# jematy/SAHS-Deformable-Nerf

Hardware: AMD Instinct MI355X
Metric: rendered rays/sec (coarse64+fine128, 8x256 MLP) (higher is better)
Workload: dtype f32

## Files before the change

include/sahs_nerf.h:

```cpp
#ifndef SAHS_NERF_H
#define SAHS_NERF_H
#include <stddef.h>
#include <stdint.h>
#ifdef __cplusplus
extern "C" {
#endif

#define SAHS_ABI_VERSION 1
#define SAHS_F32 0
#define SAHS_BF16 1
#define SAHS_BF16X3 3

int sahs_abi_version(void);
const char *sahs_last_error(void);

long sahs_param_count(void);
long sahs_packed_words(int precision);
long sahs_frame_words(void);

int sahs_pack_weights(const float *flat_params, void *packed, int precision, void *stream);

int sahs_fold_conditioning(const float *flat_params, const float *audio, const float *pose, int pose_ld, float *frame,
                           void *stream);

int sahs_get_ray_bundle(int H, int W, float fx, float fy, float cx, float cy, const float *c2w, int ld, float *ro, float *rd,
                        void *stream);

int sahs_ray_uniforms(uint64_t seed, int stream_id, long ray0, long N, int S, float *out, void *stream);

int sahs_stratified_depths(long N, int S, const float *rays, int ray_stride, int lindisp, const float *t_rand, float *z,
                           void *stream);

int sahs_field_forward(const void *packed, const float *frame, int level, long N, int S, const float *rays, int ray_stride,
                       const float *z, float *raw, float *dbg, int precision, void *stream);

int sahs_composite_forward(long N, int S, const float *raw, const float *z, const float *rays, int ray_stride,
                           const float *noise, const float *bg, int white_background, float *rgb, float *disp, float *acc,
                           float *weights, float *depth, void *stream);

int sahs_resample(long N, int S, int nf, const float *z, const float *weights, const float *u, float *z_samples,
                  float *z_out, int64_t *inds, void *stream);

int sahs_sample_pdf(long N, int nb, int ns, const float *bins, const float *weights, const float *u, float *samples,
                    int64_t *inds, void *stream);

int sahs_render_rays(const void *packed, const float *frame, int precision, long N, const float *rays, int ray_stride, int Sc,
                     int nf, int lindisp, int white_background, const float *bg, const float *t_rand, const float *noise_c,
                     const float *u, const float *noise_f, float *z_c, float *z_f, float *raw, float *weights, float *rgb_c,
                     float *disp_c, float *acc_c, float *rgb_f, float *disp_f, float *acc_f, float *w_bg, float *depth_f,
                     void *stream);

long sahs_act_words_per_sample(void);
long sahs_field_backward_workspace_words(long P);
int sahs_field_forward_save(const void *packed, const float *frame, int level, long N, int S, const float *rays, int ray_stride,
                            const float *z, float *raw, float *act_out, void *stream);
int sahs_field_backward(const float *flat_params, const float *frame, int level, long P, const float *act_in, const float *d_raw,
                        float *grad_flat, float *grad_cond, float *workspace, void *stream);
int sahs_backward_gemm_precision(int precision);
int sahs_composite_backward(long N, int S, const float *raw, const float *z, const float *rays, int ray_stride, const float *noise,
                            const float *bg, int white_background, const float *d_rgb, const float *d_disp, const float *d_acc,
                            const float *d_depth, const float *d_wlast, const float *d_weights, float *d_raw, void *stream);
#define SAHS_LOSS_STATS_WORDS 64
int sahs_stage1_loss_forward(long N, const float *map_coarse, const float *map_fine, const float *target, int target_ld, const float *mask,
                             const float *class_weights, float *stats, void *stream);
int sahs_composite_backward_loss(long N, int S, const float *raw, const float *z, const float *rays, int ray_stride, const float *noise,
                                 const float *bg, int white_background, const float *d_rgb, const float *d_disp, const float *d_acc,
                                 const float *d_depth, const float *d_wlast, const float *loss_map, const float *loss_target, int target_ld,
                                 const float *loss_mask, const float *loss_stats, const float *loss_gscale, float *d_raw, void *stream);
int sahs_conditioning_backward(const float *flat_params, const float *audio, const float *grad_cond, float *grad_flat,
                               float *grad_audio, void *stream);

#define SAHS_MODEL_AUDIO 0
#define SAHS_MODEL_NERFACE 1
#define SAHS_MODEL_NERFACE_STATIC 2
long sahs_model_param_count(int model);
long sahs_model_packed_words(int model, int precision);
long sahs_model_frame_words(int model);
int sahs_model_pack_weights(int model, const float *flat_params, void *packed, int precision, void *stream);
int sahs_model_fold_conditioning(int model, const float *flat_params, const float *driving, const float *pose, int pose_ld, float *frame,
                                 void *stream);
int sahs_model_field_forward(int model, const void *packed, const float *frame, int level, long N, int S, const float *rays,
                             int ray_stride, const float *z, float *raw, float *dbg, int precision, void *stream);
int sahs_model_render_rays(int model, const void *packed, const float *frame, int precision, long N, const float *rays, int ray_stride,
                           int Sc, int nf, int lindisp, int white_background, const float *bg, const float *t_rand, const float *noise_c,
                           const float *u, const float *noise_f, float *z_c, float *z_f, float *raw, float *weights, float *rgb_c,
                           float *disp_c, float *acc_c, float *rgb_f, float *disp_f, float *acc_f, float *w_bg, float *depth_f,
                           void *stream);

long sahs_model_act_words_per_sample(int model);
long sahs_model_field_backward_workspace_words(int model, long P);
int sahs_model_field_forward_save(int model, const void *packed, const float *frame, int level, long N, int S, const float *rays,
                                  int ray_stride, const float *z, float *raw, float *act_out, void *stream);
int sahs_model_field_backward(int model, const float *flat_params, const float *frame, int level, long P, const float *act_in,
                              const float *d_raw, float *grad_flat, float *grad_cond, float *workspace, void *stream);

long sahs_model_executed_macs_per_sample(int model, int precision);
long sahs_model_executed_macs_part(int model, int precision, int part);

#define SAHS_ROW_COLUMNS 36
#define SAHS_ROW_RGB_C 0
#define SAHS_ROW_DISP_C 15
#define SAHS_ROW_ACC_C 16
#define SAHS_ROW_RGB_F 17
#define SAHS_ROW_DISP_F 32
#define SAHS_ROW_ACC_F 33
#define SAHS_ROW_W_BG 34
#define SAHS_ROW_DEPTH_F 35
int sahs_composite_forward_rows(long N, int S, const float *raw, const float *z, const float *rays, int ray_stride, const float *noise,
                                const float *bg, int white_background, float *weights, float *rows, int row_ld, int fine_pass, void *stream);
int sahs_resample_merge(long N, int S, int nf, const float *z, const float *weights, const float *u, float *z_samples, float *z_out,
                        int32_t *src, void *stream);

int sahs_model_field_forward_split(int model, const void *packed, const float *frame, int precision, int level, int mode, long N, int S, const float *rays,
                                   int ray_stride, const float *z, float *raw, float *xw, int xw_row, int xw_col0, const int32_t *src,
                                   void *stream);

long sahs_model_act_words_part(int model, int part);
int sahs_model_field_forward_split_save(int model, const void *packed, const float *frame, int level, int mode, long N, int S, const float *rays,
                                        int ray_stride, const float *z, float *raw, float *xw, int xw_row, int xw_col0, const int32_t *src,
                                        float *act_out, void *stream);
int sahs_model_field_backward_split(int model, const float *flat_params, const float *frame, int level, int part, long P, const float *act_in,
                                    const float *d_raw, const float *xw_grad_in, float *xw_grad_out, float *grad_flat, float *grad_cond,
                                    float *workspace, void *stream);
int sahs_route_xw_grad(long N, int Sc, int nf, const int32_t *src, const float *g_fine, float *g_coarse, float *g_new, void *stream);

int sahs_bf16_exact_leaky(int enable);

long sahs_model_bits_words_part(int model, int part);
int sahs_model_field_forward_split_save_bits(int model, const void *packed, const float *frame, int level, int mode, long N, int S, const float *rays,
                                             int ray_stride, const float *z, float *raw, float *xw, int xw_row, int xw_col0, const int32_t *src,
                                             float *act_out, uint32_t *bits_out, void *stream);
int sahs_model_field_forward_save_bits(int model, const void *packed, const float *frame, int level, long N, int S, const float *rays,
                                       int ray_stride, const float *z, float *raw, float *act_out, uint32_t *bits_out, void *stream);
int sahs_model_field_forward_split_save_bits_x3(int model, const void *packed, const float *frame, int level, int mode, long N, int S, const float *rays,
                                                int ray_stride, const float *z, float *raw, float *xw, int xw_row, int xw_col0, const int32_t *src,
                                                float *act_out, uint32_t *bits_out, void *stream);
int sahs_model_field_forward_save_bits_x3(int model, const void *packed, const float *frame, int level, long N, int S, const float *rays,
                                          int ray_stride, const float *z, float *raw, float *act_out, uint32_t *bits_out, void *stream);
long sahs_model_field_backward_fused_workspace_words(int model, int part, long P);
int sahs_model_field_backward_fused(int model, const float *flat_params, const float *frame, int level, int part, long P, const float *act_in,
                                    const uint32_t *bits_in, const float *d_raw, const float *xw_grad_in, float *xw_grad_out, float *grad_flat,
                                    float *grad_cond, float *workspace, void *stream);

int sahs_model_render_rays_rows(int model, const void *packed, const float *frame, int precision, long N, const float *rays,
                                int ray_stride, int Sc, int nf, int lindisp, int white_background, const float *bg, const float *t_rand,
                                const float *noise_c, const float *u, const float *noise_f, float *z_c, float *z_f, float *raw,
                                float *weights, float *rows, int row_ld, float *xw, int32_t *src, float *z_new, void *stream);

size_t sahs_model_render_sparse_workspace_bytes(int model, long samples);
int sahs_model_render_rays_rows_sparse(int model, const void *packed, const float *frame, int precision, long N, const float *rays,
                                       int ray_stride, int Sc, int nf, int lindisp, int white_background, const float *bg, const float *t_rand,
                                       const float *noise_c, const float *u, const float *noise_f, float *z_c, float *z_f, float *raw,
                                       float *weights, float *rows, int row_ld, float *xw, int32_t *src, float *z_new, void *ws, size_t ws_bytes,
                                       void *stream);

int sahs_adam_step(float *params, const float *grad, float *exp_avg, float *exp_avg_sq, long n, float lr, float beta1, float beta2,
                   float eps, long step, float grad_scale, void *stream);

long sahs_spade_modulate_workspace_words(long planes);
int sahs_spade_modulate(long planes, long hw, const float *x, const float *gamma, const float *beta, float eps, float slope, float *out,
                        float *stats, void *stream);

int sahs_probe_arm(int capacity);
int sahs_probe_disarm(void);
int sahs_probe_count(void);
int sahs_probe_dropped(void);
int sahs_probe_read(int i, int *kind, long *samples, float *ms);

#ifdef __cplusplus
}
#endif
#endif
```

sahs-deformable-nerf_amd/_lib.py:

```python
import ctypes
import os

_HERE = os.path.dirname(os.path.abspath(__file__))
LIB_PATH = os.environ.get("SAHS_NERF_LIB") or os.path.join(_HERE, "libsahs_nerf.so")
SAHS_F32, SAHS_BF16, SAHS_BF16X3 = 0, 1, 3

_P = ctypes.c_void_p
_I = ctypes.c_int
_L = ctypes.c_long
_F = ctypes.c_float

SIGNATURES = {
    "sahs_abi_version": (_I, []),
    "sahs_last_error": (ctypes.c_char_p, []),
    "sahs_param_count": (_L, []),
    "sahs_packed_words": (_L, [_I]),
    "sahs_frame_words": (_L, []),
    "sahs_pack_weights": (_I, [_P, _P, _I, _P]),
    "sahs_fold_conditioning": (_I, [_P, _P, _P, _I, _P, _P]),
    "sahs_get_ray_bundle": (_I, [_I, _I, _F, _F, _F, _F, _P, _I, _P, _P, _P]),
    "sahs_ray_uniforms": (_I, [ctypes.c_uint64, _I, _L, _L, _I, _P, _P]),
    "sahs_stratified_depths": (_I, [_L, _I, _P, _I, _I, _P, _P, _P]),
    "sahs_field_forward": (_I, [_P, _P, _I, _L, _I, _P, _I, _P, _P, _P, _I, _P]),
    "sahs_composite_forward": (_I, [_L, _I, _P, _P, _P, _I, _P, _P, _I, _P, _P, _P, _P, _P, _P]),
    "sahs_resample": (_I, [_L, _I, _I, _P, _P, _P, _P, _P, _P, _P]),
    "sahs_sample_pdf": (_I, [_L, _I, _I, _P, _P, _P, _P, _P, _P]),
    "sahs_render_rays": (_I, [_P, _P, _I, _L, _P, _I, _I, _I, _I, _I] + [_P] * 18),
    "sahs_act_words_per_sample": (_L, []),
    "sahs_field_backward_workspace_words": (_L, [_L]),
    "sahs_field_forward_save": (_I, [_P, _P, _I, _L, _I, _P, _I, _P, _P, _P, _P]),
    "sahs_field_backward": (_I, [_P, _P, _I, _L, _P, _P, _P, _P, _P, _P]),
    "sahs_composite_backward": (_I, [_L, _I, _P, _P, _P, _I, _P, _P, _I, _P, _P, _P, _P, _P, _P, _P, _P]),
    "sahs_conditioning_backward": (_I, [_P, _P, _P, _P, _P, _P]),
    "sahs_model_param_count": (_L, [_I]),
    "sahs_model_packed_words": (_L, [_I, _I]),
    "sahs_model_frame_words": (_L, [_I]),
    "sahs_model_pack_weights": (_I, [_I, _P, _P, _I, _P]),
    "sahs_model_fold_conditioning": (_I, [_I, _P, _P, _P, _I, _P, _P]),
    "sahs_model_field_forward": (_I, [_I, _P, _P, _I, _L, _I, _P, _I, _P, _P, _P, _I, _P]),
    "sahs_model_render_rays": (_I, [_I, _P, _P, _I, _L, _P, _I, _I, _I, _I, _I] + [_P] * 18),
    "sahs_composite_forward_rows": (_I, [_L, _I, _P, _P, _P, _I, _P, _P, _I, _P, _P, _I, _I, _P]),
    "sahs_model_executed_macs_per_sample": (_L, [_I, _I]),
    "sahs_model_executed_macs_part": (_L, [_I, _I, _I]),
    "sahs_model_render_rays_rows": (_I, [_I, _P, _P, _I, _L, _P, _I, _I, _I, _I, _I] + [_P] * 10 + [_I, _P, _P, _P, _P]),
    "sahs_model_render_sparse_workspace_bytes": (ctypes.c_size_t, [_I, _L]),
    "sahs_model_render_rays_rows_sparse": (_I, [_I, _P, _P, _I, _L, _P, _I, _I, _I, _I, _I] + [_P] * 10 + [_I, _P, _P, _P, _P, ctypes.c_size_t, _P]),
    "sahs_resample_merge": (_I, [_L, _I, _I, _P, _P, _P, _P, _P, _P, _P]),
    "sahs_model_act_words_part": (_L, [_I, _I]),
    "sahs_model_field_forward_split_save": (_I, [_I, _P, _P, _I, _I, _L, _I, _P, _I, _P, _P, _P, _I, _I, _P, _P, _P]),
    "sahs_model_field_backward_split": (_I, [_I, _P, _P, _I, _I, _L, _P, _P, _P, _P, _P, _P, _P, _P]),
    "sahs_route_xw_grad": (_I, [_L, _I, _I, _P, _P, _P, _P, _P]),
    "sahs_bf16_exact_leaky": (_I, [_I]),
    "sahs_model_bits_words_part": (_L, [_I, _I]),
    "sahs_model_field_forward_split_save_bits": (_I, [_I, _P, _P, _I, _I, _L, _I, _P, _I, _P, _P, _P, _I, _I, _P, _P, _P, _P]),
    "sahs_model_field_forward_save_bits": (_I, [_I, _P, _P, _I, _L, _I, _P, _I, _P, _P, _P, _P, _P]),
    "sahs_model_field_forward_split_save_bits_x3": (_I, [_I, _P, _P, _I, _I, _L, _I, _P, _I, _P, _P, _P, _I, _I, _P, _P, _P, _P]),
    "sahs_model_field_forward_save_bits_x3": (_I, [_I, _P, _P, _I, _L, _I, _P, _I, _P, _P, _P, _P, _P]),
    "sahs_model_field_backward_fused_workspace_words": (_L, [_I, _I, _L]),
    "sahs_model_field_backward_fused": (_I, [_I, _P, _P, _I, _I, _L, _P, _P, _P, _P, _P, _P, _P, _P, _P]),
    "sahs_stage1_loss_forward": (_I, [_L, _P, _P, _P, _I, _P, _P, _P, _P]),
    "sahs_composite_backward_loss": (_I, [_L, _I, _P, _P, _P, _I, _P, _P, _I] + [_P] * 5 + [_P, _P, _I, _P, _P, _P, _P, _P]),
    "sahs_model_field_forward_split": (_I, [_I, _P, _P, _I, _I, _I, _L, _I, _P, _I, _P, _P, _P, _I, _I, _P, _P]),
    "sahs_model_act_words_per_sample": (_L, [_I]),
    "sahs_model_field_backward_workspace_words": (_L, [_I, _L]),
    "sahs_model_field_forward_save": (_I, [_I, _P, _P, _I, _L, _I, _P, _I, _P, _P, _P, _P]),
    "sahs_model_field_backward": (_I, [_I, _P, _P, _I, _L, _P, _P, _P, _P, _P, _P]),
    "sahs_backward_gemm_precision": (_I, [_I]),
    "sahs_adam_step": (_I, [_P, _P, _P, _P, _L, _F, _F, _F, _F, _L, _F, _P]),
    "sahs_spade_modulate_workspace_words": (_L, [_L]),
    "sahs_spade_modulate": (_I, [_L, _L, _P, _P, _P, _F, _F, _P, _P, _P]),
    "sahs_probe_arm": (_I, [_I]),
    "sahs_probe_disarm": (_I, []),
    "sahs_probe_count": (_I, []),
    "sahs_probe_dropped": (_I, []),
    "sahs_probe_read": (_I, [_I, ctypes.POINTER(_I), ctypes.POINTER(_L), ctypes.POINTER(_F)]),
}

_lib = None


class SahsError(RuntimeError):
    pass


def lib():
    global _lib
    if _lib is None:
        if not os.path.exists(LIB_PATH):
            raise SahsError("%s not found: the HIP extension is not built (run `python sahs-deformable-nerf_amd/build.py`); "
                            "there is no CPU fallback" % LIB_PATH)
        L = ctypes.CDLL(LIB_PATH)
        for name, (res, args) in SIGNATURES.items():
            fn = getattr(L, name)
            fn.restype, fn.argtypes = res, args
        if L.sahs_abi_version() != 1:
            raise SahsError("libsahs_nerf.so ABI version %d, expected 1" % L.sahs_abi_version())
        _lib = L
    return _lib


def check(code, what):
    if code != 0:
        raise SahsError("%s failed (%d): %s" % (what, code, lib().sahs_last_error().decode()))
```

sahs-deformable-nerf_amd/build.py:

```python
import os
import re
import subprocess
import sys

HERE = os.path.dirname(os.path.abspath(__file__))
CSRC = os.path.join(HERE, "csrc")
LIB = os.path.join(HERE, "libsahs_nerf.so")
SOURCES = ["capi.hip", "pack.hip", "render_ops.hip", "spade_ops.hip", "optim.hip", "field_f32.hip", "field_bf16w.hip", "field_bf16x3.hip", "field_bwd.hip", "field_bwd_gemm.hip", "field_bwd_chain.hip", "field_bwd_chain_f32.hip", "train_bwd.hip"]
MODEL_SOURCES = ["pack.hip", "field_f32.hip", "field_bwd.hip", "field_bwd_chain.hip", "field_bwd_chain_f32.hip"]
X3_SOURCES = ["field_bf16x3.hip"]
MODEL1_SOURCES = ["field_bf16w.hip"]
FIELD_FLAGS = ["-fno-honor-nans", "-mno-amdgpu-ieee"]
NO_SCRATCH = {"gemm_dma_kernel": 0, "_ZN4sahs24field_forward_f32_kernelILb0E": 0, "field_forward_bf16w_kernel": 0,
              "field_radiance_bf16x3_kernel": 0, "field_deform_bf16x3_kernel": 0, "gemm_tn_split_kernel": 0, "gemm_tn_jobs_kernel": 0,
              "field_backward_chain_rad_kernel": 0, "field_backward_chain_def_kernel": 0, "_ZN4sahs24field_forward_f32_kernelILb1E": 96,
              "gemm_tn_jobs_f32_kernel": 0, "gemm_tn_jobs256_f32_kernel": 0, "adam_step_kernel": 0,
              "field_backward_chain_rad_f32_kernel": 0, "field_backward_chain_def_f32_kernel": 0,
              "_ZN7sahs_nf3bwc31field_backward_chain_rad_kernel": 0, "_ZN7sahs_nf3bwc31field_backward_chain_def_kernel": 0,
              "_ZN7sahs_ns3bwc31field_backward_chain_rad_kernel": 0, "_ZN7sahs_nf3bwf35field_backward_chain_rad_f32_kernel": 0,
              "_ZN7sahs_nf3bwf35field_backward_chain_def_f32_kernel": 0, "_ZN7sahs_ns3bwf35field_backward_chain_rad_f32_kernel": 0}
HAND_SCHEDULED = [("field_bf16w.hip", 0, "field_forward_bf16w_kernel"), ("field_bf16w.hip", 1, "field_forward_bf16w_kernel"),
                  ("field_bf16w.hip", 2, "field_forward_bf16w_kernel"), ("field_bf16x3.hip", 0, "field_radiance_bf16x3_kernel"),
                  ("field_bf16x3.hip", 0, "field_deform_bf16x3_kernel"), ("field_bf16x3.hip", 1, "field_deform_bf16x3_kernel"),
                  ("field_bf16x3.hip", 1, "field_radiance_bf16x3_kernel"), ("field_bf16x3.hip", 2, "field_radiance_bf16x3_kernel"),
                  ("field_bwd_chain.hip", 0, "field_backward_chain_rad_kernel"), ("field_bwd_chain.hip", 0, "field_backward_chain_def_kernel"),
                  ("field_bwd_chain.hip", 1, "field_backward_chain_rad_kernel"), ("field_bwd_chain.hip", 1, "field_backward_chain_def_kernel"),
                  ("field_bwd_chain.hip", 2, "field_backward_chain_rad_kernel")]
PER_FILE_FLAGS = {"field_bwd_gemm.hip": ["-fno-slp-vectorize"], "field_bwd.hip": ["-fno-slp-vectorize"],
                  "field_bf16w.hip": ["-mllvm", "-amdgpu-mfma-vgpr-form=1"], "field_bf16x3.hip": ["-mllvm", "-amdgpu-mfma-vgpr-form=1"],
                  "field_bwd_chain.hip": ["-mllvm", "-amdgpu-mfma-vgpr-form=1"]}
FLAGS = ["--offload-arch=gfx950", "-O3", "-std=c++20", "-fPIC", "-ffp-contract=off", "-fno-math-errno", "-Wall", "-Wno-unused-function"]


def _stale():
    if not os.path.exists(LIB):
        return True
    t = os.path.getmtime(LIB)
    deps = [os.path.join(CSRC, f) for f in os.listdir(CSRC)] + [os.path.join(HERE, "..", "include", "sahs_nerf.h")]
    return any(os.path.getmtime(d) > t for d in deps)


def _resource_usage(remarks):
    out, cur = {}, None
    keys = {"TotalSGPRs": "sgpr", "VGPRs": "vgpr", "AGPRs": "agpr", "ScratchSize [bytes/lane]": "scratch", "Occupancy [waves/SIMD]": "occ",
            "LDS Size [bytes/block]": "lds"}
    for line in remarks.splitlines():
        if "remark:" not in line:
            continue
        body = line.split("remark:", 1)[1].replace("[-Rpass-analysis=kernel-resource-usage]", "").strip()
        if body.startswith("Function Name:"):
            cur = body.split(":", 1)[1].strip()
            out[cur] = dict(sgpr=0, vgpr=0, agpr=0, scratch=0, occ=0, lds=0)
        elif cur is not None and ":" in body:
            k, v = body.rsplit(":", 1)
            if k.strip() in keys:
                out[cur][keys[k.strip()]] = int(v)
    return out


def _compile_cmd(hipcc, src, model, defines):
    base = os.path.basename(src)
    extra = (FIELD_FLAGS if base.startswith("field_") else []) + (["-DSAHS_MODEL=%d" % model] if model else []) + \
            ([] if "SAHS_NOTHING" in defines else PER_FILE_FLAGS.get(src, []))
    return [hipcc] + FLAGS + extra + ["-D" + d for d in defines]


def build(force=False, verbose=False, defines=(), out=None, check_inflight=True):
    global LIB
    if out is None and defines:
        raise RuntimeError("libsahs_nerf.so is built without extra defines (SAHS_DIAG variants go to their own file: out=...)")
    if out is not None:
        LIB, force = out, True
    if not (force or _stale()):
        return LIB
    hipcc = os.environ.get("HIPCC", "/opt/rocm/bin/hipcc")
    objs = []
    bdir = os.path.join(HERE, "build")
    os.makedirs(bdir, exist_ok=True)
    tag = os.path.basename(LIB)
    procs = []
    for src, model in [(s, 0) for s in SOURCES] + [(s, m) for m in (1, 2) for s in MODEL_SOURCES] + [(s, m) for m in (1, 2) for s in MODEL1_SOURCES] + [(s, m) for m in (1, 2) for s in X3_SOURCES]:
        obj = os.path.join(bdir, (tag + "." if out else "") + os.path.basename(src).replace(".hip", ".m%d.o" % model if model else ".o"))
        objs.append(obj)
        cmd = _compile_cmd(hipcc, src, model, defines) + ["-Rpass-analysis=kernel-resource-usage", "-c", os.path.join(CSRC, src), "-o", obj]
        if verbose:
            print(" ".join(cmd))
        procs.append((src, subprocess.Popen(cmd, stderr=subprocess.PIPE, text=True)))
    isa = []
    if check_inflight:
        for src, model, pat in HAND_SCHEDULED:
            path = os.path.join(bdir, "%s.%s.m%d.s" % (tag, src.replace(".hip", ""), model))
            cmd = _compile_cmd(hipcc, src, model, defines) + ["--cuda-device-only", "-S", os.path.join(CSRC, src), "-o", path]
            isa.append((src, model, pat, path, subprocess.Popen(cmd, stderr=subprocess.DEVNULL)))
    usage = {}
    for src, p in procs:
        err = p.communicate()[1]
        diag = [l for l in err.splitlines() if "[-Rpass-analysis=kernel-resource-usage]" not in l and not l.lstrip().startswith(("|", "^")) and
                not (l[:1] == " " and l.strip()[:1].isdigit() and "|" in l)]
        if diag and (verbose or p.returncode != 0):
            print("\n".join(diag), file=sys.stderr)
        if p.returncode != 0:
            raise RuntimeError("hipcc failed on " + src)
        usage.update(_resource_usage(err))
    with open(os.path.join(bdir, tag + ".resource_usage.txt"), "w") as f:
        for k in sorted(usage):
            f.write("%-110s vgpr %3d agpr %3d sgpr %3d scratch %4d lds %6d occupancy %d\n" % (
                k, usage[k]["vgpr"], usage[k]["agpr"], usage[k]["sgpr"], usage[k]["scratch"], usage[k]["lds"], usage[k]["occ"]))
    bad = ["%s: %d bytes/lane of scratch" % (k, v["scratch"]) for k, v in usage.items() for name, cap in NO_SCRATCH.items()
           if name in k and v["scratch"] > cap]
    if bad and not defines:
        raise RuntimeError("kernels that rely on counted waits must not use scratch:\n  " + "\n  ".join(bad))
    if isa:
        sys.path.insert(0, os.path.join(HERE, "..", "tools"))
        import check_lds_inflight as chk
        report = []
        for src, model, pat, path, p in isa:
            if p.wait() != 0:
                raise RuntimeError("hipcc -S failed on %s (SAHS_MODEL=%d)" % (src, model))
            text = open(path).read()
            total, viol, dist = chk.check(text, pat)
            for n in re.findall(r"^(\S*%s\S*):" % re.escape(pat), text, re.M):
                want, meta = usage.get(n), re.search(r"\.amdhsa_kernel %s\b.*?\.end_amdhsa_kernel" % re.escape(n), text, re.S)
                nxt = re.search(r"\.amdhsa_next_free_vgpr (\d+)", meta.group(0)) if meta else None
                if want is not None and nxt is not None:
                    expect = want["vgpr"] if not want["agpr"] else (want["vgpr"] + 3) // 4 * 4 + want["agpr"]
                    if int(nxt.group(1)) != expect:
                        raise RuntimeError("in-flight check: the ISA of %s is not the object's (next_free_vgpr %s, object vgpr %d agpr %d)"
                                           % (n, nxt.group(1), want["vgpr"], want["agpr"]))
            report.append("%s (SAHS_MODEL=%d) %s: %d hand-issued ds_read_b128, %d violations, longest in-flight window %d instructions"
                          % (src, model, pat, total, len(viol), max(dist) if dist else 0))
            if viol or total == 0:
                raise RuntimeError("hand-issued LDS reads touched in flight (tools/check_lds_inflight.py) in %s SAHS_MODEL=%d:\n  %s"
                                   % (src, model, "\n  ".join("%s | %s" % (r, w) for _, r, w in viol[:8]) or "no reads found"))
        with open(os.path.join(bdir, tag + ".lds_inflight.txt"), "w") as f:
            f.write("\n".join(report) + "\n")
        if verbose:
            print("\n".join(report))
    cmd = [hipcc, "--offload-arch=gfx950", "-shared", "-fPIC", "-Wl,-z,defs", "-o", LIB] + objs
    subprocess.check_call(cmd)
    return LIB


if __name__ == "__main__":
    print(build(force="--force" in sys.argv, verbose=True))
```

sahs-deformable-nerf_amd/csrc/capi.hip:

```cpp
#include <hip/hip_runtime.h>
#include <cmath>
#include <cstdarg>
#include <cstdio>
#include <cstdlib>
#include <cstring>
#include <atomic>
#include <vector>
#include "../../include/sahs_nerf.h"
#include "sahs_common.hpp"
#include "sahs_launchers.hpp"

static thread_local char g_err[512] = "";

__attribute__((format(printf, 2, 3))) static int fail(int code, const char *fmt, ...)
{
    va_list ap;
    va_start(ap, fmt);
    vsnprintf(g_err, sizeof(g_err), fmt, ap);
    va_end(ap);
    return code;
}
static int hip_fail(const char *what, int e)
{
    snprintf(g_err, sizeof(g_err), "%s: HIP error %d (%s)", what, e, hipGetErrorString((hipError_t)e));
    return 100 + e;
}
#define REQUIRE(cond, name) do { if (!(cond)) return fail(1, "%s: invalid argument (capi.hip:%d)", name, __LINE__); } while (0)
#define ALIGNED16(p) ((reinterpret_cast<uintptr_t>(p) & 15u) == 0)

static int num_cus()
{
    static std::atomic<int> cache[sahs_once::MAX_DEVICES];
    int dev = 0;
    if (hipGetDevice(&dev) != hipSuccess || dev < 0 || dev >= sahs_once::MAX_DEVICES) return 256;
    int n = cache[dev].load(std::memory_order_relaxed);
    if (n == 0) {
        int v = 0;
        n = (hipDeviceGetAttribute(&v, hipDeviceAttributeMultiprocessorCount, dev) == hipSuccess && v > 0) ? v : 256;
        cache[dev].store(n, std::memory_order_relaxed);
    }
    return n;
}

struct Probe {
    bool armed = false;
    int cap = 0, n = 0, dropped = 0;
    std::vector<hipEvent_t> ev;
    std::vector<int> kind;
    std::vector<long> samples;
};
static thread_local Probe g_probe;
static inline int probe_kind(int model, int precision, int level, int part) { return model << 16 | level << 12 | part << 8 | precision; }
template <class F> static inline int probed(int kind, long samples, hipStream_t st, F &&launch)
{
    Probe &p = g_probe;
    if (!p.armed) return launch();
    if (p.n >= p.cap) { ++p.dropped; return launch(); }
    (void)hipEventRecord(p.ev[2 * p.n], st);
    const int e = launch();
    (void)hipEventRecord(p.ev[2 * p.n + 1], st);
    p.kind[p.n] = kind;
    p.samples[p.n] = samples;
    ++p.n;
    return e;
}


extern "C" {

int sahs_abi_version(void) { return SAHS_ABI_VERSION; }

int sahs_probe_arm(int capacity)
{
    Probe &p = g_probe;
    REQUIRE(capacity >= 1 && capacity <= 65536, "sahs_probe_arm(1 <= capacity <= 65536)");
    while ((int)p.ev.size() < 2 * capacity) {
        hipEvent_t e;
        const hipError_t r = hipEventCreate(&e);
        if (r != hipSuccess) return hip_fail("sahs_probe_arm", (int)r);
        p.ev.push_back(e);
    }
    p.kind.assign(capacity, 0);
    p.samples.assign(capacity, 0);
    p.cap = capacity;
    p.n = p.dropped = 0;
    p.armed = true;
    return 0;
}
int sahs_probe_disarm(void) { g_probe.armed = false; return 0; }
int sahs_probe_count(void) { return g_probe.n; }
int sahs_probe_dropped(void) { return g_probe.dropped; }
int sahs_probe_read(int i, int *kind, long *samples, float *ms)
{
    Probe &p = g_probe;
    REQUIRE(i >= 0 && i < p.n && kind && samples && ms, "sahs_probe_read");
    hipError_t r = hipEventSynchronize(p.ev[2 * i + 1]);
    if (r == hipSuccess) r = hipEventElapsedTime(ms, p.ev[2 * i], p.ev[2 * i + 1]);
    if (r != hipSuccess) return hip_fail("sahs_probe_read", (int)r);
    *kind = p.kind[i];
    *samples = p.samples[i];
    return 0;
}
const char *sahs_last_error(void) { return g_err; }

int sahs_get_ray_bundle(int H, int W, float fx, float fy, float cx, float cy, const float *c2w, int ld, float *ro, float *rd, void *stream)
{
    REQUIRE(H > 0 && W > 0 && c2w && ro && rd && ld >= 4, "sahs_get_ray_bundle");
    int e = sahs_ray_bundle_launch(H, W, fx, fy, cx, cy, c2w, ld, ro, rd, (hipStream_t)stream);
    return e ? hip_fail("sahs_get_ray_bundle", e) : 0;
}

int sahs_ray_uniforms(uint64_t seed, int stream_id, long ray0, long N, int S, float *out, void *stream)
{
    if (N == 0) return 0;
    REQUIRE(out && N >= 0 && S >= 1 && ray0 >= 0, "sahs_ray_uniforms");
    int e = sahs_ray_uniforms_launch(seed, stream_id, ray0, N, S, out, (hipStream_t)stream);
    return e ? hip_fail("sahs_ray_uniforms", e) : 0;
}

int sahs_stratified_depths(long N, int S, const float *rays, int ray_stride, int lindisp, const float *t_rand, float *z, void *stream)
{
    if (N == 0) return 0;
    REQUIRE(N >= 0 && S >= 1 && rays && z && ray_stride >= 8, "sahs_stratified_depths");
    int e = sahs_stratified_depths_launch(N, S, rays, ray_stride, lindisp, t_rand, z, (hipStream_t)stream);
    return e ? hip_fail("sahs_stratified_depths", e) : 0;
}

int sahs_composite_forward(long N, int S, const float *raw, const float *z, const float *rays, int ray_stride, const float *noise,
                           const float *bg, int white_background, float *rgb, float *disp, float *acc, float *weights, float *depth,
                           void *stream)
{
    if (N == 0) return 0;
    REQUIRE(raw && z && rays && rgb && disp && acc && weights && depth && ray_stride >= 6, "sahs_composite_forward");
    REQUIRE(N >= 0 && S >= 1 && S <= 256 && ALIGNED16(raw), "sahs_composite_forward(shape: 1 <= S <= 256)");
    int e = sahs_composite_forward_launch(N, S, raw, z, rays, ray_stride, noise, bg, white_background, rgb, disp, acc, weights, depth,
                                          nullptr, 15, 1, (hipStream_t)stream);
    return e ? hip_fail("sahs_composite_forward", e) : 0;
}

int sahs_resample(long N, int S, int nf, const float *z, const float *weights, const float *u, float *z_samples, float *z_out,
                  int64_t *inds, void *stream)
{
    if (N == 0) return 0;
    REQUIRE(z && weights && z_out, "sahs_resample");
    REQUIRE(N >= 0 && S >= 3 && S <= 256 && nf >= 1 && nf <= 256, "sahs_resample(shape: 3 <= S <= 256, 1 <= nf <= 256)");
    int e = sahs_resample_launch(N, S, nf, 1, z, weights, u, z_samples, z_out, (long long *)inds, nullptr, (hipStream_t)stream);
    return e ? hip_fail("sahs_resample", e) : 0;
}

int sahs_resample_merge(long N, int S, int nf, const float *z, const float *weights, const float *u, float *z_samples, float *z_out,
                        int32_t *src, void *stream)
{
    if (N == 0) return 0;
    REQUIRE(z && weights && z_out && z_samples && src, "sahs_resample_merge");
    REQUIRE(N >= 0 && S >= 3 && S <= 256 && nf >= 1 && nf <= 256, "sahs_resample_merge(shape: 3 <= S <= 256, 1 <= nf <= 256)");
    int e = sahs_resample_launch(N, S, nf, 1, z, weights, u, z_samples, z_out, nullptr, src, (hipStream_t)stream);
    return e ? hip_fail("sahs_resample_merge", e) : 0;
}

int sahs_sample_pdf(long N, int nb, int ns, const float *bins, const float *weights, const float *u, float *samples, int64_t *inds,
                    void *stream)
{
    if (N == 0) return 0;
    REQUIRE(bins && weights && samples, "sahs_sample_pdf");
    REQUIRE(N >= 0 && nb >= 2 && nb < 256 && ns >= 1 && ns <= 256, "sahs_sample_pdf(shape: 2 <= nb < 256, 1 <= ns <= 256)");
    int e = sahs_resample_launch(N, nb + 1, ns, 0, bins, weights, u, samples, nullptr, (long long *)inds, nullptr, (hipStream_t)stream);
    return e ? hip_fail("sahs_sample_pdf", e) : 0;
}

int sahs_composite_backward(long N, int S, const float *raw, const float *z, const float *rays, int ray_stride, const float *noise,
                            const float *bg, int white_background, const float *d_rgb, const float *d_disp, const float *d_acc,
                            const float *d_depth, const float *d_wlast, const float *d_weights, float *d_raw, void *stream)
{
    REQUIRE(raw && z && rays && d_raw && ray_stride >= 6 && ALIGNED16(raw) && ALIGNED16(d_raw), "sahs_composite_backward");
    REQUIRE(N >= 0 && S >= 1 && S <= 256, "sahs_composite_backward(shape: 1 <= S <= 256)");
    if (N == 0) return 0;
    int e = sahs_composite_backward_launch(N, S, raw, z, rays, ray_stride, noise, bg, white_background, d_rgb, d_disp, d_acc, d_depth, d_wlast,
                                           d_weights, d_raw, nullptr, nullptr, 0, nullptr, nullptr, nullptr, (hipStream_t)stream);
    return e ? hip_fail("sahs_composite_backward", e) : 0;
}

int sahs_stage1_loss_forward(long N, const float *map_coarse, const float *map_fine, const float *target, int target_ld, const float *mask,
                             const float *class_weights, float *stats, void *stream)
{
    REQUIRE((map_coarse || map_fine) && target && mask && class_weights && stats && target_ld >= 3 && N >= 1, "sahs_stage1_loss_forward");
    int e = sahs_stage1_loss_forward_launch(N, map_coarse, map_fine, target, target_ld, mask, class_weights, stats, (hipStream_t)stream);
    return e ? hip_fail("sahs_stage1_loss_forward", e) : 0;
}

int sahs_composite_backward_loss(long N, int S, const float *raw, const float *z, const float *rays, int ray_stride, const float *noise,
                                 const float *bg, int white_background, const float *d_rgb, const float *d_disp, const float *d_acc,
                                 const float *d_depth, const float *d_wlast, const float *loss_map, const float *loss_target, int target_ld,
                                 const float *loss_mask, const float *loss_stats, const float *loss_gscale, float *d_raw, void *stream)
{
    REQUIRE(raw && z && rays && d_raw && ray_stride >= 6 && ALIGNED16(raw) && ALIGNED16(d_raw), "sahs_composite_backward_loss");
    REQUIRE(loss_map && loss_target && loss_mask && loss_stats && target_ld >= 3, "sahs_composite_backward_loss(loss operands)");
    REQUIRE(N >= 0 && S >= 1 && S <= 256, "sahs_composite_backward_loss(shape: 1 <= S <= 256)");
    if (N == 0) return 0;
    int e = sahs_composite_backward_launch(N, S, raw, z, rays, ray_stride, noise, bg, white_background, d_rgb, d_disp, d_acc, d_depth, d_wlast,
                                           nullptr, d_raw, loss_map, loss_target, target_ld, loss_mask, loss_stats, loss_gscale,
                                           (hipStream_t)stream);
    return e ? hip_fail("sahs_composite_backward_loss", e) : 0;
}

int sahs_conditioning_backward(const float *flat_params, const float *audio, const float *grad_cond, float *grad_flat, float *grad_audio,
                               void *stream)
{
    REQUIRE(flat_params && audio && grad_cond && grad_flat, "sahs_conditioning_backward");
    int e = sahs_conditioning_backward_launch(flat_params, audio, grad_cond, grad_flat, grad_audio, (hipStream_t)stream);
    return e ? hip_fail("sahs_conditioning_backward", e) : 0;
}

int sahs_route_xw_grad(long N, int Sc, int nf, const int32_t *src, const float *g_fine, float *g_coarse, float *g_new, void *stream)
{
    if (N == 0) return 0;
    REQUIRE(src && g_fine && g_coarse && g_new && N >= 0 && Sc >= 1 && nf >= 1 && ALIGNED16(g_fine) && ALIGNED16(g_coarse) && ALIGNED16(g_new),
            "sahs_route_xw_grad");
    int e = sahs_route_xw_grad_launch(N, Sc, nf, src, g_fine, g_coarse, g_new, (hipStream_t)stream);
    return e ? hip_fail("sahs_route_xw_grad", e) : 0;
}

static double decimal_double(float x)
{
    char buf[32];
    for (int digits = 1; digits <= 9; ++digits) {
        snprintf(buf, sizeof(buf), "%.*g", digits, (double)x);
        if (strtof(buf, nullptr) == x) return strtod(buf, nullptr);
    }
    return (double)x;
}

int sahs_adam_step(float *params, const float *grad, float *exp_avg, float *exp_avg_sq, long n, float lr, float beta1, float beta2, float eps,
                   long step, float grad_scale, void *stream)
{
    if (n == 0) return 0;
    REQUIRE(params && grad && exp_avg && exp_avg_sq && n > 0 && step >= 1, "sahs_adam_step");
    REQUIRE(std::isfinite(lr) && lr > 0.0f && std::isfinite(eps) && eps > 0.0f && std::isfinite(grad_scale), "sahs_adam_step(lr > 0, eps > 0, finite)");
    REQUIRE(beta1 >= 0.0f && beta1 < 1.0f && beta2 >= 0.0f && beta2 < 1.0f, "sahs_adam_step(0 <= beta < 1)");
    const uintptr_t p = reinterpret_cast<uintptr_t>(params), g = reinterpret_cast<uintptr_t>(grad), m = reinterpret_cast<uintptr_t>(exp_avg),
                    v = reinterpret_cast<uintptr_t>(exp_avg_sq), bytes = (uintptr_t)n * sizeof(float);
    REQUIRE(((p | g | m | v) & 3u) == 0, "sahs_adam_step(4-byte aligned buffers)");
    auto overlap = [bytes](uintptr_t a, uintptr_t b) { return a < b + bytes && b < a + bytes; };
    REQUIRE(!overlap(p, m) && !overlap(p, v) && !overlap(m, v), "sahs_adam_step(params, exp_avg, exp_avg_sq must not overlap)");
    const double b1 = decimal_double(beta1), b2 = decimal_double(beta2);
    const double bc1 = 1.0 - std::pow(b1, (double)step), bc2 = 1.0 - std::pow(b2, (double)step);
    int e = sahs_adam_step_launch(params, grad, exp_avg, exp_avg_sq, n, (float)(1.0 - b1), (float)b2, (float)(1.0 - b2),
                                  (float)(decimal_double(lr) / bc1), (float)std::sqrt(bc2), (float)decimal_double(eps), grad_scale,
                                  (hipStream_t)stream);
    return e ? hip_fail("sahs_adam_step", e) : 0;
}

long sahs_spade_modulate_workspace_words(long planes) { return planes > 0 ? sahs_spade_stats_words(planes) : 0; }

int sahs_spade_modulate(long planes, long hw, const float *x, const float *gamma, const float *beta, float eps, float slope, float *out,
                        float *stats, void *stream)
{
    if (planes == 0 || hw == 0) return 0;
    REQUIRE(planes > 0 && planes <= 2147483647L && hw > 0 && x && gamma && beta && out && stats && eps > 0.0f, "sahs_spade_modulate");
    int e = sahs_spade_modulate_launch(planes, hw, x, gamma, beta, eps, slope, out, stats, (hipStream_t)stream);
    return e ? hip_fail("sahs_spade_modulate", e) : 0;
}

int sahs_composite_forward_rows(long N, int S, const float *raw, const float *z, const float *rays, int ray_stride, const float *noise,
                                const float *bg, int white_background, float *weights, float *rows, int row_ld, int fine_pass, void *stream)
{
    if (N == 0) return 0;
    REQUIRE(raw && z && rays && weights && rows && ray_stride >= 6 && row_ld >= SAHS_ROW_COLUMNS, "sahs_composite_forward_rows");
    REQUIRE(N >= 0 && S >= 1 && S <= 256 && ALIGNED16(raw), "sahs_composite_forward_rows(shape: 1 <= S <= 256)");
    int e = fine_pass ? sahs_composite_forward_launch(N, S, raw, z, rays, ray_stride, noise, bg, white_background, rows + SAHS_ROW_RGB_F,
                                                      rows + SAHS_ROW_DISP_F, rows + SAHS_ROW_ACC_F, weights, rows + SAHS_ROW_DEPTH_F,
                                                      rows + SAHS_ROW_W_BG, row_ld, row_ld, (hipStream_t)stream)
                      : sahs_composite_forward_launch(N, S, raw, z, rays, ray_stride, noise, bg, white_background, rows + SAHS_ROW_RGB_C,
                                                      rows + SAHS_ROW_DISP_C, rows + SAHS_ROW_ACC_C, weights, nullptr, nullptr, row_ld,
                                                      row_ld, (hipStream_t)stream);
    return e ? hip_fail("sahs_composite_forward_rows", e) : 0;
}

enum Pack { PK_NONE, PK_F32, PK_BF16, PK_X3 };
typedef int (*pack_fn)(const float *, float *, hipStream_t);
struct ModelFns {
    bool deformation_nets;
    long (*param_count)(void);
    long (*frame_words)(void);
    long (*act_words)(void);
    long (*packed_words[4])(void);
    pack_fn pack[4];
    long (*executed_macs)(int, int);
    int (*act_part_words)(int);
    int (*act_part_col0)(int);
    int (*bits_part_words)(int);
    int (*fold)(const float *, const float *, const float *, int, float *, hipStream_t);
    int (*bwd_gemm_precision_state)(int);
    int (*bf16w_exact_leaky_state)(int);
    decltype(&sahs_field_forward_f32_launch) f32;
    decltype(&sahs_field_forward_f32_split_launch) f32_split;
    decltype(&sahs_field_forward_f32_split_bits_launch) f32_split_bits;
    decltype(&sahs_field_forward_f32_sparse_launch) f32_sparse;
    decltype(&sahs_field_f32_sparse_ws_bytes) f32_sparse_ws_bytes;
    long (*bwd_ws_words)(long);
    decltype(&sahs_field_backward_launch) bwd;
    decltype(&sahs_field_backward_split_launch) bwd_split;
    long (*fused_ws_words)(int, long);
    decltype(&sahs_field_backward_fused_launch) bwd_fused;
    decltype(&sahs_field_forward_bf16w_launch) bf16w;
    decltype(&sahs_field_forward_bf16w_split_launch) bf16w_split;
    decltype(&sahs_field_deform_bf16x3_launch) deform_x3;
    decltype(&sahs_field_deform_bf16x3_save_launch) deform_x3_save;
    decltype(&sahs_field_radiance_bf16x3_launch) radiance_x3;
    decltype(&sahs_field_radiance_bf16x3_save_launch) radiance_x3_save;
    decltype(&sahs_field_forward_bf16x3_launch) x3;
    decltype(&sahs_field_forward_bf16x3_save_launch) x3_save;
};
#define SAHS_MODEL_ROW(sfx, deform)                                                                                                    \
    deform, sahs_layout_param_count##sfx, sahs_layout_frame_words##sfx, sahs_layout_act_words##sfx,                                 \
        {nullptr, sahs_layout_packed_words_f32##sfx, sahs_layout_packed_words_bf16##sfx, sahs_layout_packed_words_bf16x3##sfx},      \
        {nullptr, sahs_pack_weights_f32_launch##sfx, sahs_pack_weights_bf16_launch##sfx, sahs_pack_weights_bf16x3_launch##sfx},      \
        sahs_layout_executed_macs##sfx, sahs_layout_act_part_words##sfx, sahs_layout_act_part_col0##sfx, sahs_layout_bits_part_words##sfx, \
        sahs_fold_conditioning_launch##sfx, sahs_bwd_gemm_precision_state##sfx, sahs_bf16w_exact_leaky_state##sfx,                  \
        sahs_field_forward_f32_launch##sfx, sahs_field_forward_f32_split_launch##sfx, sahs_field_forward_f32_split_bits_launch##sfx, \
        sahs_field_forward_f32_sparse_launch##sfx, sahs_field_f32_sparse_ws_bytes##sfx,                                              \
        sahs_field_backward_ws_words##sfx, sahs_field_backward_launch##sfx, sahs_field_backward_split_launch##sfx,                  \
        sahs_field_backward_fused_ws_words##sfx, sahs_field_backward_fused_launch##sfx
static const ModelFns kModels[3] = {
    {SAHS_MODEL_ROW(, true), sahs_field_forward_bf16w_launch, sahs_field_forward_bf16w_split_launch, sahs_field_deform_bf16x3_launch,
     sahs_field_deform_bf16x3_save_launch, sahs_field_radiance_bf16x3_launch, sahs_field_radiance_bf16x3_save_launch, nullptr, nullptr},
    {SAHS_MODEL_ROW(_nf, true), nullptr, sahs_field_forward_bf16w_split_launch_nf, sahs_field_deform_bf16x3_launch_nf,
     sahs_field_deform_bf16x3_save_launch_nf, sahs_field_radiance_bf16x3_launch_nf, sahs_field_radiance_bf16x3_save_launch_nf, nullptr, nullptr},
    {SAHS_MODEL_ROW(_ns, false), sahs_field_forward_bf16w_launch_ns, nullptr, nullptr, nullptr, nullptr, nullptr,
     sahs_field_forward_bf16x3_launch_ns, sahs_field_forward_bf16x3_save_launch_ns},
};
#undef SAHS_MODEL_ROW

enum Kernel { K_NONE, K_F32, K_BF16, K_X3 };
struct Pipe {
    Pack seg[3];
    Kernel whole;
    Kernel split;
    Kernel chain;
    int def_prec, def_x, rad_prec, rad_x;
};
static const Pipe kPipes[3][4] = {
    {
        {{PK_F32}, K_F32, K_F32, K_NONE, SAHS_F32, 1, SAHS_F32, 1},
        {{PK_BF16}, K_BF16, K_BF16, K_NONE, SAHS_BF16, 1, SAHS_BF16, 1},
        {{}, K_NONE, K_NONE, K_NONE, SAHS_BF16, 1, SAHS_BF16, 1},
        {{PK_X3, PK_F32}, K_NONE, K_NONE, K_X3, SAHS_BF16, 3, SAHS_BF16, 3},
    },
    {
        {{PK_F32}, K_F32, K_F32, K_NONE, SAHS_F32, 1, SAHS_F32, 1},
        {{PK_BF16, PK_F32, PK_X3}, K_NONE, K_NONE, K_BF16, SAHS_BF16, 3, SAHS_BF16, 1},
        {{}, K_NONE, K_NONE, K_NONE, SAHS_BF16, 1, SAHS_BF16, 1},
        {{PK_X3, PK_F32}, K_NONE, K_NONE, K_X3, SAHS_BF16, 3, SAHS_BF16, 3},
    },
    {
        {{PK_F32}, K_F32, K_NONE, K_NONE, SAHS_F32, 1, SAHS_F32, 1},
        {{PK_BF16}, K_BF16, K_NONE, K_NONE, SAHS_BF16, 1, SAHS_BF16, 1},
        {{}, K_NONE, K_NONE, K_NONE, SAHS_BF16, 1, SAHS_BF16, 1},
        {{PK_X3}, K_X3, K_NONE, K_NONE, SAHS_BF16, 3, SAHS_BF16, 3},
    },
};
static const Pipe *pipe_of(int model, int precision) { return precision >= 0 && precision <= 3 ? &kPipes[model][precision] : nullptr; }
static long packed_layout(int model, const Pipe *p, long off[4])
{
    long end = -1;
    for (int i = 0; p && i < 3 && p->seg[i] != PK_NONE; ++i) {
        off[p->seg[i]] = end < 0 ? 0 : (end + 3) / 4 * 4;
        end = off[p->seg[i]] + kModels[model].packed_words[p->seg[i]]();
    }
    return end;
}
static bool x3_deform_on_f32()
{
    static const bool v = getenv("SAHS_X3_DEFORM") != nullptr && strcmp(getenv("SAHS_X3_DEFORM"), "f32") == 0;
    return v;
}
static long act_col0(int model, int part) { return kModels[model].act_part_col0(part == 3 ? 0 : part); }
#define REQUIRE_MODEL(m, name) do { if ((m) < 0 || (m) > 2) return fail(3, "%s: unknown model %d", name, (int)(m)); } while (0)

long sahs_param_count(void) { return sahs_model_param_count(SAHS_MODEL_AUDIO); }
long sahs_packed_words(int precision) { return sahs_model_packed_words(SAHS_MODEL_AUDIO, precision); }
long sahs_frame_words(void) { return sahs_model_frame_words(SAHS_MODEL_AUDIO); }
long sahs_act_words_per_sample(void) { return sahs_model_act_words_per_sample(SAHS_MODEL_AUDIO); }
long sahs_field_backward_workspace_words(long P) { return sahs_model_field_backward_workspace_words(SAHS_MODEL_AUDIO, P); }

long sahs_model_param_count(int model) { return (model < 0 || model > 2) ? -1 : kModels[model].param_count(); }
long sahs_model_frame_words(int model) { return (model < 0 || model > 2) ? -1 : kModels[model].frame_words(); }
long sahs_model_act_words_per_sample(int model) { return (model < 0 || model > 2) ? -1 : kModels[model].act_words(); }
long sahs_model_field_backward_workspace_words(int model, long P) { return (model < 0 || model > 2) ? -1 : kModels[model].bwd_ws_words(P); }
long sahs_model_packed_words(int model, int precision)
{
    long off[4];
    return (model < 0 || model > 2) ? -1 : packed_layout(model, pipe_of(model, precision), off);
}
long sahs_model_executed_macs_part(int model, int precision, int part)
{
    if (model < 0 || model > 2 || precision < SAHS_F32 || precision > SAHS_BF16X3 || part < 0 || part > 2) return -1;
    const ModelFns &m = kModels[model];
    const Pipe &p = kPipes[model][precision];
    const long def = p.chain != K_NONE && x3_deform_on_f32() ? m.executed_macs(SAHS_F32, 1) : p.def_x * m.executed_macs(p.def_prec, 1);
    const long rad = p.rad_x * m.executed_macs(p.rad_prec, 2);
    return (part != 2 ? def : 0) + (part != 1 ? rad : 0);
}
long sahs_model_executed_macs_per_sample(int model, int precision) { return sahs_model_executed_macs_part(model, precision, 0); }
long sahs_model_act_words_part(int model, int part)
{
    return (model < 0 || model > 2 || part < 0 || part > 3) ? -1 : kModels[model].act_part_words(part == 3 ? 0 : part);
}
long sahs_model_bits_words_part(int model, int part)
{
    return (model < 0 || model > 2 || part < 0 || part > 3) ? 0 : kModels[model].bits_part_words(part == 3 ? 0 : part);
}
long sahs_model_field_backward_fused_workspace_words(int model, int part, long P)
{
    return (model < 0 || model > 2 || part < 1 || part > 3 || P < 0) ? -1 : kModels[model].fused_ws_words(part, P);
}

int sahs_backward_gemm_precision(int precision)
{
    if (precision < 0) return kModels[SAHS_MODEL_AUDIO].bwd_gemm_precision_state(-1) ? SAHS_BF16X3 : SAHS_F32;
    if (precision != SAHS_F32 && precision != SAHS_BF16X3) return -1;
    for (const ModelFns &m : kModels) m.bwd_gemm_precision_state(precision == SAHS_BF16X3 ? 3 : 0);
    return precision;
}

int sahs_bf16_exact_leaky(int enable)
{
    if (enable < 0) return kModels[SAHS_MODEL_AUDIO].bf16w_exact_leaky_state(-1);
    int r = 0;
    for (int i = 2; i >= 0; --i) r = kModels[i].bf16w_exact_leaky_state(enable);
    return r;
}

static int pack_weights(const char *who, int model, const float *flat_params, void *packed, int precision, void *stream)
{
    REQUIRE(flat_params && packed && ALIGNED16(packed), who);
    long off[4];
    if (packed_layout(model, pipe_of(model, precision), off) < 0) return fail(2, "%s: precision %d is not built for this model", who, precision);
    int e = 0;
    for (Pack s : kPipes[model][precision].seg)
        if (s != PK_NONE && !e) e = kModels[model].pack[s](flat_params, (float *)packed + off[s], (hipStream_t)stream);
    return e ? hip_fail(who, e) : 0;
}
int sahs_pack_weights(const float *flat_params, void *packed, int precision, void *stream)
{
    return pack_weights("sahs_pack_weights", SAHS_MODEL_AUDIO, flat_params, packed, precision, stream);
}
int sahs_model_pack_weights(int model, const float *flat_params, void *packed, int precision, void *stream)
{
    REQUIRE_MODEL(model, "sahs_model_pack_weights");
    return pack_weights("sahs_model_pack_weights", model, flat_params, packed, precision, stream);
}

static int fold_conditioning(const char *who, int model, const float *flat_params, const float *driving, const float *pose, int pose_ld,
                             float *frame, void *stream)
{
    REQUIRE(flat_params && driving && pose && frame && pose_ld >= 4 && ALIGNED16(frame), who);
    int e = kModels[model].fold(flat_params, driving, pose, pose_ld, frame, (hipStream_t)stream);
    return e ? hip_fail(who, e) : 0;
}
int sahs_fold_conditioning(const float *flat_params, const float *audio, const float *pose, int pose_ld, float *frame, void *stream)
{
    return fold_conditioning("sahs_fold_conditioning", SAHS_MODEL_AUDIO, flat_params, audio, pose, pose_ld, frame, stream);
}
int sahs_model_fold_conditioning(int model, const float *flat_params, const float *driving, const float *pose, int pose_ld, float *frame,
                                 void *stream)
{
    REQUIRE_MODEL(model, "sahs_model_fold_conditioning");
    return fold_conditioning("sahs_model_fold_conditioning", model, flat_params, driving, pose, pose_ld, frame, stream);
}

static int field_forward(const char *who, int model, const void *packed, const float *frame, int level, long N, int S, const float *rays,
                         int ray_stride, const float *z, float *raw, float *dbg, int precision, void *stream)
{
    if (N == 0) return 0;
    REQUIRE(packed && frame && rays && z && raw, who);
    REQUIRE((level == 0 || level == 1) && N >= 0 && S >= 1 && ray_stride >= 8, who);
    REQUIRE(ALIGNED16(packed) && ALIGNED16(frame) && ALIGNED16(raw) && (!dbg || ALIGNED16(dbg)), who);
    const Pipe *p = pipe_of(model, precision);
    long off[4];
    if (packed_layout(model, p, off) < 0) return fail(2, "%s: precision %d is not built for this model", who, precision);
    if (p->whole == K_NONE)
        return fail(2, "%s: precision %d of this model runs through sahs_model_field_forward_split / sahs_model_render_rays_rows (it needs the "
                       "xw workspace)", who, precision);
    const ModelFns &m = kModels[model];
    const float *pk = (const float *)packed;
    hipStream_t st = (hipStream_t)stream;
    int e = probed(probe_kind(model, precision, level, 0), N * S, st, [&] {
        if (p->whole == K_F32) return m.f32(pk, frame, level, N * S, S, rays, ray_stride, z, raw, dbg, nullptr, num_cus(), st);
        if (p->whole == K_BF16) return m.bf16w(pk, frame, level, N * S, S, rays, ray_stride, z, raw, dbg, num_cus(), st);
        return m.x3(pk, frame, level, N * S, S, rays, ray_stride, z, raw, num_cus(), st);
    });
    return e ? hip_fail(who, e) : 0;
}
int sahs_field_forward(const void *packed, const float *frame, int level, long N, int S, const float *rays, int ray_stride,
                       const float *z, float *raw, float *dbg, int precision, void *stream)
{
    return field_forward("sahs_field_forward", SAHS_MODEL_AUDIO, packed, frame, level, N, S, rays, ray_stride, z, raw, dbg, precision, stream);
}
int sahs_model_field_forward(int model, const void *packed, const float *frame, int level, long N, int S, const float *rays, int ray_stride,
                             const float *z, float *raw, float *dbg, int precision, void *stream)
{
    REQUIRE_MODEL(model, "sahs_model_field_forward");
    return field_forward("sahs_model_field_forward", model, packed, frame, level, N, S, rays, ray_stride, z, raw, dbg, precision, stream);
}

static int render_rays_chain(const char *who, int model, const void *packed, const float *frame, int precision, long N,
                             const float *rays, int ray_stride, int Sc, int nf, int lindisp, int white_background, const float *bg,
                             const float *t_rand, const float *noise_c, const float *u, const float *noise_f, float *z_c, float *z_f,
                             float *raw, float *weights, float *rgb_c, float *disp_c, float *acc_c, float *rgb_f, float *disp_f,
                             float *acc_f, float *w_bg, float *depth_f, void *stream, int rgb_ld = 15, int sc_ld = 1)
{
    if (N == 0) return 0;
    REQUIRE(packed && frame && rays && z_c && raw && weights && rgb_c && disp_c && acc_c && w_bg && depth_f, who);
    REQUIRE(nf == 0 || (z_f && rgb_f && disp_f && acc_f), who);
    hipStream_t st = (hipStream_t)stream;
    int e;
    if ((e = sahs_stratified_depths(N, Sc, rays, ray_stride, lindisp, t_rand, z_c, stream))) return e;
    if ((e = field_forward(who, model, packed, frame, 0, N, Sc, rays, ray_stride, z_c, raw, nullptr, precision, stream))) return e;
    REQUIRE(Sc <= 256, who);
    e = sahs_composite_forward_launch(N, Sc, raw, z_c, rays, ray_stride, noise_c, bg, white_background, rgb_c, disp_c, acc_c, weights,
                                      nf == 0 ? depth_f : nullptr, nf == 0 ? w_bg : nullptr, rgb_ld, sc_ld, st);
    if (e) return hip_fail(who, e);
    if (nf > 0) {
        const int Sf = Sc + nf;
        REQUIRE(Sf <= 256, who);
        if ((e = sahs_resample(N, Sc, nf, z_c, weights, u, nullptr, z_f, nullptr, stream))) return e;
        if ((e = field_forward(who, model, packed, frame, 1, N, Sf, rays, ray_stride, z_f, raw, nullptr, precision, stream))) return e;
        e = sahs_composite_forward_launch(N, Sf, raw, z_f, rays, ray_stride, noise_f, bg, white_background, rgb_f, disp_f, acc_f,
                                          weights, depth_f, w_bg, rgb_ld, sc_ld, st);
        if (e) return hip_fail(who, e);
    }
    return 0;
}

int sahs_render_rays(const void *packed, const float *frame, int precision, long N, const float *rays, int ray_stride, int Sc, int nf,
                     int lindisp, int white_background, const float *bg, const float *t_rand, const float *noise_c, const float *u,
                     const float *noise_f, float *z_c, float *z_f, float *raw, float *weights, float *rgb_c, float *disp_c,
                     float *acc_c, float *rgb_f, float *disp_f, float *acc_f, float *w_bg, float *depth_f, void *stream)
{
    return render_rays_chain("sahs_render_rays", SAHS_MODEL_AUDIO, packed, frame, precision, N, rays, ray_stride, Sc, nf, lindisp,
                             white_background, bg, t_rand, noise_c, u, noise_f, z_c, z_f, raw, weights, rgb_c, disp_c, acc_c, rgb_f, disp_f,
                             acc_f, w_bg, depth_f, stream);
}
int sahs_model_render_rays(int model, const void *packed, const float *frame, int precision, long N, const float *rays, int ray_stride,
                           int Sc, int nf, int lindisp, int white_background, const float *bg, const float *t_rand, const float *noise_c,
                           const float *u, const float *noise_f, float *z_c, float *z_f, float *raw, float *weights, float *rgb_c,
                           float *disp_c, float *acc_c, float *rgb_f, float *disp_f, float *acc_f, float *w_bg, float *depth_f, void *stream)
{
    REQUIRE_MODEL(model, "sahs_model_render_rays");
    return render_rays_chain("sahs_model_render_rays", model, packed, frame, precision, N, rays, ray_stride, Sc, nf, lindisp, white_background,
                             bg, t_rand, noise_c, u, noise_f, z_c, z_f, raw, weights, rgb_c, disp_c, acc_c, rgb_f, disp_f, acc_f, w_bg, depth_f,
                             stream);
}

int sahs_model_field_forward_split(int model, const void *packed, const float *frame, int precision, int level, int mode, long N, int S,
                                   const float *rays, int ray_stride, const float *z, float *raw, float *xw, int xw_row, int xw_col0,
                                   const int32_t *src, void *stream)
{
    const char *who = "sahs_model_field_forward_split";
    REQUIRE_MODEL(model, who);
    if (N == 0) return 0;
    const ModelFns &m = kModels[model];
    if (!m.deformation_nets) return fail(4, "%s: this model has no deformation nets", who);
    REQUIRE(packed && frame && rays && xw && (level == 0 || level == 1) && N >= 0 && S >= 1 && ray_stride >= 8 && mode >= 0 && mode <= 2, who);
    const Pipe *p = pipe_of(model, precision);
    const bool chain = p && p->chain != K_NONE;
    REQUIRE((mode == 1 || raw) && (mode == 2 || z) && (mode != 2 || src || chain), who);
    REQUIRE(xw_col0 >= 0 && xw_row >= xw_col0 + (mode == 2 ? 0 : S) && ALIGNED16(xw) && ALIGNED16(packed) && ALIGNED16(frame) && (!raw || ALIGNED16(raw)),
            who);
    const float *pk = (const float *)packed;
    const long P = N * S;
    hipStream_t st = (hipStream_t)stream;
    int e = 0;
    if (chain) {
        REQUIRE(mode != 0 || xw_col0 == 0, who);
        long off[4];
        packed_layout(model, p, off);
        if (mode != 2 && !x3_deform_on_f32())
            e = probed(probe_kind(model, SAHS_BF16X3, level, 1), P, st, [&] {
                return m.deform_x3(pk + off[PK_X3], frame, level, P, S, rays, ray_stride, z, xw, xw_row, xw_col0, num_cus(), st);
            });
        else if (mode != 2)
            e = probed(probe_kind(model, SAHS_F32, level, 1), P, st, [&] {
                return m.f32_split(pk + off[PK_F32], frame, level, 1, P, S, rays, ray_stride, z, nullptr, xw, xw_row, xw_col0, nullptr, nullptr,
                                   num_cus(), st);
            });
        if (!e && mode != 1)
            e = probed(probe_kind(model, precision, level, 2), P, st, [&] {
                const int *sp = mode == 2 ? src : nullptr;
                return p->chain == K_BF16
                           ? m.bf16w_split(pk + off[PK_BF16], frame, level, 2, P, S, rays, ray_stride, nullptr, raw, xw, xw_row, 0, sp, num_cus(), st)
                           : m.radiance_x3(pk + off[PK_X3], frame, level, P, S, rays, ray_stride, raw, xw, xw_row, sp, num_cus(), st);
            });
        return e ? hip_fail(who, e) : 0;
    }
    if (!p || p->split == K_NONE) return fail(4, "%s: precision %d is not built for this model", who, precision);
    e = probed(probe_kind(model, precision, level, mode), P, st, [&] {
        return p->split == K_BF16
                   ? m.bf16w_split(pk, frame, level, mode, P, S, rays, ray_stride, z, raw, xw, xw_row, xw_col0, src, num_cus(), st)
                   : m.f32_split(pk, frame, level, mode, P, S, rays, ray_stride, z, raw, xw, xw_row, xw_col0, src, nullptr, num_cus(), st);
    });
    return e ? hip_fail(who, e) : 0;
}


struct SaveForm {
    const char *who;
    bool split, x3, bits;
};
static int field_forward_save(const SaveForm &f, int model, const void *packed, const float *frame, int level, int mode, long N, int S,
                              const float *rays, int ray_stride, const float *z, float *raw, float *xw, int xw_row, int xw_col0,
                              const int32_t *src, float *act_out, uint32_t *bits_out, void *stream)
{
    const char *who = f.who;
    REQUIRE_MODEL(model, who);
    const ModelFns &m = kModels[model];
    if (f.split && !f.bits && N == 0) return 0;
    if (f.split && !m.deformation_nets)
        return fail(4, "%s: this model has no deformation nets (its saving forward: sahs_model_field_forward_save%s)", who,
                    f.x3 ? "_bits_x3" : (f.bits ? "_bits" : ""));
    if (!f.split && f.x3 && !m.x3_save)
        return fail(4, "%s: this model saves through the split chain on this pipe (sahs_model_field_forward_split_save_bits_x3)", who);
    if (f.split && N == 0) return 0;
    REQUIRE(packed && frame && rays && act_out && (!f.bits || bits_out) && (f.split ? xw != nullptr : z && raw), who);
    REQUIRE((level == 0 || level == 1) && N >= 0 && S >= 1 && ray_stride >= 8, who);
    if (f.split) {
        REQUIRE(f.x3 ? (mode == 1 || mode == 2) : (mode >= 0 && mode <= 2), who);
        REQUIRE((mode == 1 || raw) && (mode == 2 || z) && (mode != 2 || src), who);
        REQUIRE(xw_col0 >= 0 && xw_row >= xw_col0 + (mode == 2 ? 0 : S) && ALIGNED16(xw), who);
    }
    REQUIRE(ALIGNED16(packed) && ALIGNED16(frame) && (!raw || ALIGNED16(raw)) && ALIGNED16(act_out) && (!f.bits || ALIGNED16(bits_out)), who);
    const long P = N * S;
    REQUIRE(!f.bits || P <= 4000000L, who);
    if (!f.split && f.bits && P == 0) return 0;
    const float *pk = (const float *)packed;
    float *base = act_out - act_col0(model, mode) * P;
    hipStream_t st = (hipStream_t)stream;
    int e;
    if (f.x3)
        e = probed(probe_kind(model, SAHS_BF16X3, level, mode), P, st, [&] {
            if (!f.split) return m.x3_save(pk, frame, level, P, S, rays, ray_stride, z, raw, act_out, bits_out, num_cus(), st);
            if (mode == 1) return m.deform_x3_save(pk, frame, level, P, S, rays, ray_stride, z, xw, xw_row, xw_col0, base, bits_out, num_cus(), st);
            return m.radiance_x3_save(pk, frame, level, P, S, rays, ray_stride, raw, xw, xw_row, src, base, bits_out, num_cus(), st);
        });
    else if (f.bits)
        e = m.f32_split_bits(pk, frame, level, mode, P, S, rays, ray_stride, z, raw, xw, xw_row, xw_col0, src, base, bits_out, num_cus(), st);
    else if (f.split)
        e = m.f32_split(pk, frame, level, mode, P, S, rays, ray_stride, z, raw, xw, xw_row, xw_col0, src, base, num_cus(), st);
    else
        e = m.f32(pk, frame, level, P, S, rays, ray_stride, z, raw, nullptr, act_out, num_cus(), st);
    return e ? hip_fail(who, e) : 0;
}

int sahs_field_forward_save(const void *packed, const float *frame, int level, long N, int S, const float *rays, int ray_stride,
                            const float *z, float *raw, float *act_out, void *stream)
{
    return field_forward_save({"sahs_field_forward_save", false, false, false}, SAHS_MODEL_AUDIO, packed, frame, level, 0, N, S, rays,
                              ray_stride, z, raw, nullptr, 0, 0, nullptr, act_out, nullptr, stream);
}
int sahs_model_field_forward_save(int model, const void *packed, const float *frame, int level, long N, int S, const float *rays,
                                  int ray_stride, const float *z, float *raw, float *act_out, void *stream)
{
    return field_forward_save({"sahs_model_field_forward_save", false, false, false}, model, packed, frame, level, 0, N, S, rays, ray_stride,
                              z, raw, nullptr, 0, 0, nullptr, act_out, nullptr, stream);
}
int sahs_model_field_forward_save_bits(int model, const void *packed, const float *frame, int level, long N, int S, const float *rays, int ray_stride,
                                       const float *z, float *raw, float *act_out, uint32_t *bits_out, void *stream)
{
    return field_forward_save({"sahs_model_field_forward_save_bits", false, false, true}, model, packed, frame, level, 0, N, S, rays,
                              ray_stride, z, raw, nullptr, 0, 0, nullptr, act_out, bits_out, stream);
}
int sahs_model_field_forward_save_bits_x3(int model, const void *packed, const float *frame, int level, long N, int S, const float *rays, int ray_stride,
                                          const float *z, float *raw, float *act_out, uint32_t *bits_out, void *stream)
{
    return field_forward_save({"sahs_model_field_forward_save_bits_x3", false, true, true}, model, packed, frame, level, 0, N, S, rays,
                              ray_stride, z, raw, nullptr, 0, 0, nullptr, act_out, bits_out, stream);
}
int sahs_model_field_forward_split_save(int model, const void *packed, const float *frame, int level, int mode, long N, int S, const float *rays,
                                        int ray_stride, const float *z, float *raw, float *xw, int xw_row, int xw_col0, const int32_t *src,
                                        float *act_out, void *stream)
{
    return field_forward_save({"sahs_model_field_forward_split_save", true, false, false}, model, packed, frame, level, mode, N, S, rays,
                              ray_stride, z, raw, xw, xw_row, xw_col0, src, act_out, nullptr, stream);
}
int sahs_model_field_forward_split_save_bits(int model, const void *packed, const float *frame, int level, int mode, long N, int S, const float *rays,
                                             int ray_stride, const float *z, float *raw, float *xw, int xw_row, int xw_col0, const int32_t *src,
                                             float *act_out, uint32_t *bits_out, void *stream)
{
    return field_forward_save({"sahs_model_field_forward_split_save_bits", true, false, true}, model, packed, frame, level, mode, N, S, rays,
                              ray_stride, z, raw, xw, xw_row, xw_col0, src, act_out, bits_out, stream);
}
int sahs_model_field_forward_split_save_bits_x3(int model, const void *packed, const float *frame, int level, int mode, long N, int S, const float *rays,
                                                int ray_stride, const float *z, float *raw, float *xw, int xw_row, int xw_col0, const int32_t *src,
                                                float *act_out, uint32_t *bits_out, void *stream)
{
    return field_forward_save({"sahs_model_field_forward_split_save_bits_x3", true, true, true}, model, packed, frame, level, mode, N, S, rays,
                              ray_stride, z, raw, xw, xw_row, xw_col0, src, act_out, bits_out, stream);
}

static int field_backward(const char *who, int model, const float *flat_params, const float *frame, int level, long P, const float *act_in,
                          const float *d_raw, float *grad_flat, float *grad_cond, float *workspace, void *stream)
{
    REQUIRE(flat_params && frame && act_in && d_raw && grad_flat && grad_cond && workspace, who);
    REQUIRE((level == 0 || level == 1) && P >= 0 && P <= 4000000L, who);
    int e = kModels[model].bwd(flat_params, frame, level, P, act_in, d_raw, grad_flat, grad_cond, workspace, (hipStream_t)stream);
    return e ? hip_fail(who, e) : 0;
}
int sahs_field_backward(const float *flat_params, const float *frame, int level, long P, const float *act_in, const float *d_raw,
                        float *grad_flat, float *grad_cond, float *workspace, void *stream)
{
    return field_backward("sahs_field_backward", SAHS_MODEL_AUDIO, flat_params, frame, level, P, act_in, d_raw, grad_flat, grad_cond,
                          workspace, stream);
}
int sahs_model_field_backward(int model, const float *flat_params, const float *frame, int level, long P, const float *act_in,
                              const float *d_raw, float *grad_flat, float *grad_cond, float *workspace, void *stream)
{
    REQUIRE_MODEL(model, "sahs_model_field_backward");
    return field_backward("sahs_model_field_backward", model, flat_params, frame, level, P, act_in, d_raw, grad_flat, grad_cond, workspace,
                          stream);
}

int sahs_model_field_backward_split(int model, const float *flat_params, const float *frame, int level, int part, long P, const float *act_in,
                                    const float *d_raw, const float *xw_grad_in, float *xw_grad_out, float *grad_flat, float *grad_cond,
                                    float *workspace, void *stream)
{
    const char *who = "sahs_model_field_backward_split";
    REQUIRE_MODEL(model, who);
    if (part == 0) part = 3;
    REQUIRE(flat_params && frame && act_in && grad_flat && grad_cond && workspace && part >= 1 && part <= 3, who);
    REQUIRE((level == 0 || level == 1) && P >= 0 && P <= 4000000L, who);
    REQUIRE(((part & 2) ? d_raw != nullptr : xw_grad_in != nullptr) && (part != 2 || xw_grad_out != nullptr), who);
    const ModelFns &m = kModels[model];
    if (!m.deformation_nets && part != 3) return fail(4, "%s: this model has no deformation nets", who);
    int e = m.bwd_split(flat_params, frame, level, part, P, act_in - act_col0(model, part) * P, d_raw, xw_grad_in, xw_grad_out, grad_flat,
                        grad_cond, workspace, (hipStream_t)stream);
    return e ? hip_fail(who, e) : 0;
}

int sahs_model_field_backward_fused(int model, const float *flat_params, const float *frame, int level, int part, long P, const float *act_in,
                                    const uint32_t *bits_in, const float *d_raw, const float *xw_grad_in, float *xw_grad_out, float *grad_flat,
                                    float *grad_cond, float *workspace, void *stream)
{
    const char *who = "sahs_model_field_backward_fused";
    REQUIRE_MODEL(model, who);
    const ModelFns &m = kModels[model];
    if (!m.deformation_nets && part != 3) return fail(4, "%s: this model has no deformation nets", who);
    REQUIRE(flat_params && frame && act_in && bits_in && grad_flat && grad_cond && workspace && part >= 1 && part <= 3, who);
    REQUIRE((level == 0 || level == 1) && P >= 0 && P <= 4000000L, who);
    REQUIRE(((part & 2) ? d_raw != nullptr : xw_grad_in != nullptr) && (part != 2 || xw_grad_out != nullptr), who);
    REQUIRE(ALIGNED16(act_in) && ALIGNED16(bits_in) && ALIGNED16(workspace) && (!d_raw || ALIGNED16(d_raw)) && (!xw_grad_in || ALIGNED16(xw_grad_in)) &&
            (!xw_grad_out || ALIGNED16(xw_grad_out)), who);
    if (P == 0) return 0;
    int e = m.bwd_fused(flat_params, frame, level, part, P, act_in - act_col0(model, part) * P, bits_in, d_raw, xw_grad_in, xw_grad_out,
                        grad_flat, grad_cond, workspace, num_cus(), (hipStream_t)stream);
    return e ? hip_fail(who, e) : 0;
}

int sahs_model_render_rays_rows(int model, const void *packed, const float *frame, int precision, long N, const float *rays,
                                int ray_stride, int Sc, int nf, int lindisp, int white_background, const float *bg, const float *t_rand,
                                const float *noise_c, const float *u, const float *noise_f, float *z_c, float *z_f, float *raw,
                                float *weights, float *rows, int row_ld, float *xw, int32_t *src, float *z_new, void *stream)
{
    const char *who = "sahs_model_render_rays_rows";
    REQUIRE_MODEL(model, who);
    if (N == 0) return 0;
    REQUIRE(rows && row_ld >= SAHS_ROW_COLUMNS, who);
    const Pipe *p = pipe_of(model, precision);
    const bool deform = kModels[model].deformation_nets;
    if (deform && p && p->chain != K_NONE)
        REQUIRE(xw && src && z_new && nf > 0, who);
    if (xw && src && z_new && nf > 0 && deform && p && (p->split != K_NONE || p->chain != K_NONE)) {
        REQUIRE(packed && frame && rays && z_c && z_f && raw && weights && Sc + nf <= 256, who);
        const int Sf = Sc + nf;
        hipStream_t st = (hipStream_t)stream;
        int e;
        if ((e = sahs_stratified_depths(N, Sc, rays, ray_stride, lindisp, t_rand, z_c, stream))) return e;
        if ((e = sahs_model_field_forward_split(model, packed, frame, precision, 0, 0, N, Sc, rays, ray_stride, z_c, raw, xw, Sf, 0, nullptr, stream))) return e;
        e = sahs_composite_forward_launch(N, Sc, raw, z_c, rays, ray_stride, noise_c, bg, white_background, rows + SAHS_ROW_RGB_C, rows + SAHS_ROW_DISP_C,
                                          rows + SAHS_ROW_ACC_C, weights, nullptr, nullptr, row_ld, row_ld, st);
        if (e) return hip_fail(who, e);
        if ((e = sahs_resample_merge(N, Sc, nf, z_c, weights, u, z_new, z_f, src, stream))) return e;
        if ((e = sahs_model_field_forward_split(model, packed, frame, precision, 1, 1, N, nf, rays, ray_stride, z_new, nullptr, xw, Sf, Sc, nullptr, stream))) return e;
        if ((e = sahs_model_field_forward_split(model, packed, frame, precision, 1, 2, N, Sf, rays, ray_stride, nullptr, raw, xw, Sf, 0, src, stream))) return e;
        e = sahs_composite_forward_launch(N, Sf, raw, z_f, rays, ray_stride, noise_f, bg, white_background, rows + SAHS_ROW_RGB_F, rows + SAHS_ROW_DISP_F,
                                          rows + SAHS_ROW_ACC_F, weights, rows + SAHS_ROW_DEPTH_F, rows + SAHS_ROW_W_BG, row_ld, row_ld, st);
        return e ? hip_fail(who, e) : 0;
    }
    return render_rays_chain(who, model, packed, frame, precision, N, rays, ray_stride, Sc, nf, lindisp, white_background, bg, t_rand, noise_c,
                             u, noise_f, z_c, z_f, raw, weights, rows + SAHS_ROW_RGB_C, rows + SAHS_ROW_DISP_C, rows + SAHS_ROW_ACC_C,
                             rows + SAHS_ROW_RGB_F, rows + SAHS_ROW_DISP_F, rows + SAHS_ROW_ACC_F, rows + SAHS_ROW_W_BG, rows + SAHS_ROW_DEPTH_F,
                             stream, row_ld, row_ld);
}

static long sparse_capacity(int model, size_t ws_bytes)
{
    const ModelFns &m = kModels[model];
    const long head = m.f32_sparse_ws_bytes(0), rec = m.f32_sparse_ws_bytes(1) - head;
    if ((long)ws_bytes < head) return 0;
    long cap = ((long)ws_bytes - head) / rec / 128 * 128;
    return cap > (1L << 30) ? (1L << 30) : cap;
}
static int field_forward_sparse(const char *who, int model, const float *pk, const float *frame, int level, int stage, int part, long N, int S,
                                const float *rays, int ray_stride, const float *z, float *raw, float *xw, int xw_row, const int32_t *src,
                                const float *noise, int has_bg, void *ws, long cap, hipStream_t st)
{
    const ModelFns &m = kModels[model];
    const long per = cap / S;
    if (per < 1) return fail(5, "%s: the sparse-branch workspace holds %ld records, one ray has %d samples", who, cap, S);
    const long nslab = (N + per - 1) / per, step = (N + nslab - 1) / nslab;
    int e = probed(probe_kind(model, SAHS_F32, level, part), N * S, st, [&] {
        for (long r0 = 0; r0 < N; r0 += step) {
            const long n = N - r0 < step ? N - r0 : step, s0 = r0 * S;
            hipError_t he = hipMemsetAsync(ws, 0, 8, st);
            if (he != hipSuccess) return (int)he;
            int le = m.f32_sparse(pk, frame, level, stage, n * S, S, rays + r0 * ray_stride, ray_stride, z ? z + s0 : nullptr, raw + s0 * 16,
                                  xw ? xw + r0 * xw_row * 8 : nullptr, xw_row, 0, src ? src + s0 : nullptr, noise ? noise + s0 : nullptr, has_bg, ws,
                                  cap, num_cus(), st);
            if (le) return le;
            le = m.f32_sparse(pk, frame, level, 2, n * S, S, rays + r0 * ray_stride, ray_stride, nullptr, raw + s0 * 16, nullptr, 0, 0, nullptr, nullptr,
                              has_bg, ws, cap, num_cus(), st);
            if (le) return le;
        }
        return 0;
    });
    if (e == -4) return fail(5, "%s: the sparse-branch launcher refused its record workspace (%ld slots for slabs of %ld samples)", who, cap, step * S);
    if (e < 0) return fail(4, "%s: the sparse-branch launcher has no stage %d for this model", who, stage);
    return e ? hip_fail(who, e) : 0;
}

size_t sahs_model_render_sparse_workspace_bytes(int model, long samples)
{
    if (model < 0 || model > 2 || samples < 0 || samples > (1L << 30)) return 0;
    return (size_t)kModels[model].f32_sparse_ws_bytes((samples + 127) / 128 * 128);
}

int sahs_model_render_rays_rows_sparse(int model, const void *packed, const float *frame, int precision, long N, const float *rays,
                                       int ray_stride, int Sc, int nf, int lindisp, int white_background, const float *bg, const float *t_rand,
                                       const float *noise_c, const float *u, const float *noise_f, float *z_c, float *z_f, float *raw,
                                       float *weights, float *rows, int row_ld, float *xw, int32_t *src, float *z_new, void *ws, size_t ws_bytes,
                                       void *stream)
{
    const char *who = "sahs_model_render_rays_rows_sparse";
    REQUIRE_MODEL(model, who);
    if (precision != SAHS_F32)
        return sahs_model_render_rays_rows(model, packed, frame, precision, N, rays, ray_stride, Sc, nf, lindisp, white_background, bg, t_rand, noise_c,
                                           u, noise_f, z_c, z_f, raw, weights, rows, row_ld, xw, src, z_new, stream);
    if (N == 0) return 0;
    REQUIRE(rows && row_ld >= SAHS_ROW_COLUMNS, who);
    REQUIRE(packed && frame && rays && z_c && raw && weights && N >= 0 && Sc >= 1 && nf >= 0 && Sc + nf <= 256 && ray_stride >= 8, who);
    REQUIRE(nf == 0 || z_f, who);
    REQUIRE(ws && ALIGNED16(ws) && ALIGNED16(packed) && ALIGNED16(frame) && ALIGNED16(raw) && (!xw || ALIGNED16(xw)), who);
    const long cap = sparse_capacity(model, ws_bytes);
    if (cap < 128)
        return fail(5, "%s: a sparse-branch workspace of %zu bytes holds less than one tile of 128 records (sahs_model_render_sparse_workspace_bytes)",
                    who, ws_bytes);
    const bool shared = xw && src && z_new && nf > 0 && kModels[model].deformation_nets;
    const float *pk = (const float *)packed;
    const int Sf = Sc + nf, has_bg = bg != nullptr;
    hipStream_t st = (hipStream_t)stream;
    int e;
    if ((e = sahs_stratified_depths(N, Sc, rays, ray_stride, lindisp, t_rand, z_c, stream))) return e;
    if ((e = field_forward_sparse(who, model, pk, frame, 0, 0, 0, N, Sc, rays, ray_stride, z_c, raw, shared ? xw : nullptr, Sf, nullptr, noise_c, has_bg, ws,
                                  cap, st)))
        return e;
    e = sahs_composite_forward_launch(N, Sc, raw, z_c, rays, ray_stride, noise_c, bg, white_background, rows + SAHS_ROW_RGB_C, rows + SAHS_ROW_DISP_C,
                                      rows + SAHS_ROW_ACC_C, weights, nf == 0 ? rows + SAHS_ROW_DEPTH_F : nullptr, nf == 0 ? rows + SAHS_ROW_W_BG : nullptr,
                                      row_ld, row_ld, st);
    if (e) return hip_fail(who, e);
    if (nf == 0) return 0;
    if (shared) {
        if ((e = sahs_resample_merge(N, Sc, nf, z_c, weights, u, z_new, z_f, src, stream))) return e;
        if ((e = sahs_model_field_forward_split(model, packed, frame, precision, 1, 1, N, nf, rays, ray_stride, z_new, nullptr, xw, Sf, Sc, nullptr, stream))) return e;
        if ((e = field_forward_sparse(who, model, pk, frame, 1, 1, 2, N, Sf, rays, ray_stride, nullptr, raw, xw, Sf, src, noise_f, has_bg, ws, cap, st))) return e;
    } else {
        if ((e = sahs_resample(N, Sc, nf, z_c, weights, u, nullptr, z_f, nullptr, stream))) return e;
        if ((e = field_forward_sparse(who, model, pk, frame, 1, 0, 0, N, Sf, rays, ray_stride, z_f, raw, nullptr, 0, nullptr, noise_f, has_bg, ws, cap, st))) return e;
    }
    e = sahs_composite_forward_launch(N, Sf, raw, z_f, rays, ray_stride, noise_f, bg, white_background, rows + SAHS_ROW_RGB_F, rows + SAHS_ROW_DISP_F,
                                      rows + SAHS_ROW_ACC_F, weights, rows + SAHS_ROW_DEPTH_F, rows + SAHS_ROW_W_BG, row_ld, row_ld, st);
    return e ? hip_fail(who, e) : 0;
}

}
```

sahs-deformable-nerf_amd/csrc/field_f32.hip:

```cpp
#include <hip/hip_runtime.h>
#include "sahs_common.hpp"
#include "sahs_launchers.hpp"
#include "sahs_layout.hpp"
#include "f32_pipe.hpp"

namespace SAHS_NS {


struct RevArg { float p, lo; };
__device__ __forceinline__ RevArg rev_arg(float x)
{
    const float C_HI = 0.15915494f;
    const float C_LO = 6.4206382e-09f;
    RevArg r;
    r.p = x * C_HI;
    r.lo = fmaf(x, C_LO, fmaf(x, C_HI, -r.p));
    return r;
}
__device__ __forceinline__ float sin_octave(RevArg u, float scale, int fn)
{
    const float P = u.p * scale, Lo = u.lo * scale;
    const float f = (P - rintf(P)) + Lo;
    const float qf = rintf(4.0f * f);
    const float th = fmaf(qf, -0.25f, f) * 6.2831855f;
    const float z = th * th;
    const float sp = fmaf(th * z, fmaf(fmaf(-1.9515295891e-4f, z, 8.3321608736e-3f), z, -1.6666654611e-1f), th);
    const float cp = fmaf(z * z, fmaf(fmaf(2.443315711809948e-5f, z, -1.388731625493765e-3f), z, 4.166664568298827e-2f), fmaf(z, -0.5f, 1.0f));
    const int m = ((int)qf + fn) & 3;
    const float v = (m & 1) ? cp : sp;
    return (m & 2) ? -v : v;
}

template <int D, int L, int NB, int INC = 1>
__device__ __forceinline__ void pe_blocks(const float *v, int q, f32x4 *out)
{
    constexpr int D0 = INC ? D : 0;
    constexpr int W = D0 + 2 * D * L;
    const float v0 = v[0], v1 = v[D > 1 ? 1 : 0], v2 = v[D > 2 ? 2 : 0];
    const RevArg u0 = rev_arg(v0), u1 = rev_arg(v1), u2 = rev_arg(v2);
#pragma unroll
    for (int b = 0; b < NB; ++b)
#pragma unroll
        for (int r = 0; r < 4; ++r) {
            const int f = 16 * b + 4 * q + r;
            float val = 0.0f;
            if (f < D0) {
                val = (f == 0) ? v0 : ((f == 1) ? v1 : v2);
            } else if (f < W) {
                const int g = f - D0;
                const int k = g / (2 * D), rem = g % (2 * D);
                const int fn = rem / D, ax = rem % D;
                RevArg a;
                a.p = (ax == 0) ? u0.p : ((ax == 1) ? u1.p : u2.p);
                a.lo = (ax == 0) ? u0.lo : ((ax == 1) ? u1.lo : u2.lo);
                val = sin_octave(a, (float)(1 << k), fn);
            }
            out[b][r] = val;
        }
}

__device__ __forceinline__ void grid_blocks(const float *__restrict__ grid, float x, float y, float z, int q, f32x4 *out)
{
    const float R1 = (float)(G_RES - 1);
    const float ix = ((x + 1.0f) / 2.0f) * R1, iy = ((y + 1.0f) / 2.0f) * R1, iz = ((z + 1.0f) / 2.0f) * R1;
    const float fx = floorf(ix), fy = floorf(iy), fz = floorf(iz);
    const float x1 = fx + 1.0f, y1 = fy + 1.0f, z1 = fz + 1.0f;
    const float wx[2] = {x1 - ix, ix - fx}, wy[2] = {y1 - iy, iy - fy}, wz[2] = {z1 - iz, iz - fz};
    const bool ok = fx >= -1.0f && fx <= (float)G_RES && fy >= -1.0f && fy <= (float)G_RES && fz >= -1.0f && fz <= (float)G_RES;
    const int xi = ok ? (int)fx : -2, yi = ok ? (int)fy : -2, zi = ok ? (int)fz : -2;
    out[0] = f32x4{0.0f, 0.0f, 0.0f, 0.0f};
    out[1] = f32x4{0.0f, 0.0f, 0.0f, 0.0f};
#pragma unroll
    for (int n = 0; n < 8; ++n) {
        const int cx = xi + (n & 1), cy = yi + ((n >> 1) & 1), cz = zi + (n >> 2);
        const bool inb = cx >= 0 && cx < G_RES && cy >= 0 && cy < G_RES && cz >= 0 && cz < G_RES;
        const float wt = (wx[n & 1] * wy[(n >> 1) & 1]) * wz[n >> 2];
        const long vox = inb ? (((long)cz * G_RES + cy) * G_RES + cx) : 0;
        const f32x4 *g = reinterpret_cast<const f32x4 *>(grid + vox * D_GRID) + q;
        const f32x4 g0 = g[0], g1 = g[4];
        const float we = inb ? wt : 0.0f;
#pragma unroll
        for (int r = 0; r < 4; ++r) { out[0][r] = out[0][r] + g0[r] * we; out[1][r] = out[1][r] + g1[r] * we; }
    }
}

#define CHF(id) (kProg.layer[id].G * kProg.layer[id].KB * 256)

enum { FIELD_ALL = 0, FIELD_DEFORM = 1, FIELD_RADIANCE = 2, FIELD_ALL_TRUNK = 3, FIELD_RADIANCE_TRUNK = 4, FIELD_BRANCH = 5 };
struct SparseArgs {
    const float *noise;
    unsigned int *count;
    f32x4 *hdr;
    f32x4 *feat;
    unsigned int cap;
    int has_bg;
};
constexpr long SPARSE_HEAD_BYTES = 256, SPARSE_RECORD_BYTES = 16 + 16 * 16 * 4;
#if defined(SAHS_DIAG) && defined(SAHS_F32_ENC2)
constexpr bool DIAG_ENC2 = true;
#else
constexpr bool DIAG_ENC2 = false;
#endif
#if defined(SAHS_DIAG) && defined(SAHS_F32_NOENC)
constexpr bool DIAG_NOENC = true;
#else
constexpr bool DIAG_NOENC = false;
#endif
#if defined(SAHS_DIAG) && defined(SAHS_F32_NOLOADS_TRUNK)
constexpr bool DIAG_NOLOADS_TRUNK = true;
#else
constexpr bool DIAG_NOLOADS_TRUNK = false;
#endif
#if defined(SAHS_DIAG) && defined(SAHS_F32_NOLOADS_BRANCH)
constexpr bool DIAG_NOLOADS_BRANCH = true;
#else
constexpr bool DIAG_NOLOADS_BRANCH = false;
#endif
#if defined(SAHS_DIAG) && defined(SAHS_F32_NOAPPEND)
constexpr bool DIAG_NOAPPEND = true;
#else
constexpr bool DIAG_NOAPPEND = false;
#endif
template <int NB>
__device__ __forceinline__ void diag_blocks(const float *v, int q, f32x4 *out)
{
#pragma unroll
    for (int b = 0; b < NB; ++b) out[b] = f32x4{v[0], v[1], v[0] * (float)(q + b), v[1] + (float)b};
}
template <bool SAVE, int MODE>
__global__ void __launch_bounds__(F32_THREADS, 2)
field_forward_f32_kernel(const float *__restrict__ packed, const float *__restrict__ frame, int level, long P, int S,
                         const float *__restrict__ rays, int ray_stride, const float *__restrict__ zvals,
                         float *__restrict__ raw, float *__restrict__ dbg, float *__restrict__ actbuf,
                         float *__restrict__ xw, int xw_row, int xw_col0, const int *__restrict__ src, uint32_t *__restrict__ bits, SparseArgs sp)
{
#if SAHS_MODEL == 2
    static_assert(MODE == FIELD_ALL || MODE == FIELD_ALL_TRUNK || MODE == FIELD_BRANCH, "this model has no deformation nets to split off");
#endif
    constexpr bool TRUNK = MODE == FIELD_ALL_TRUNK || MODE == FIELD_RADIANCE_TRUNK;
    constexpr bool BRANCH = MODE == FIELD_BRANCH;
    constexpr bool XW_IN = MODE == FIELD_RADIANCE || MODE == FIELD_RADIANCE_TRUNK;
    static_assert(!(SAVE && (TRUNK || BRANCH)), "the sparse branches are an inference path");
    extern __shared__ __attribute__((aligned(16))) float lds[];
    Ctx cx;
    cx.stream = packed + PACK_STREAM_OFF + (long)level * STREAM_FLOATS;
    cx.lds = lds;
    cx.buf = 1;
    cx.lane = threadIdx.x & 63;
    cx.q = cx.lane >> 4;
    cx.wave = __builtin_amdgcn_readfirstlane(threadIdx.x >> 6);
    constexpr const Layer *Ly = kProg.layer;
    constexpr int L_START = BRANCH ? L_D0B : (XW_IN ? L_T0 : L_FIRST);
    cx.wrap_to = (uint32_t)Ly[L_START].stream_off;
    cx.wrap_at = (MODE == FIELD_DEFORM) ? (uint32_t)Ly[L_T0].stream_off : (TRUNK ? (uint32_t)Ly[L_D0B].stream_off : (uint32_t)STREAM_FLOATS);
    cx.off = cx.wrap_to;
    const float *grid = packed + PACK_GRID_OFF;

    {
        const float *bsrc = frame + FRAME_BIAS_OFF + level * BIAS_FLOATS;
        for (int i = threadIdx.x; i < BIAS_FLOATS; i += F32_THREADS) lds[LDS_BIAS_OFF + i] = bsrc[i];
        cx.begin_chunk(CHF(L_START));
#pragma unroll
        for (int pc = 0; pc < (CHF(L_START) + PIECE_FLOATS - 1) / PIECE_FLOATS; ++pc) cx.issue_piece(pc);
        cx.end_chunk();
    }

    if constexpr (BRANCH) {
        const unsigned int n = *sp.count;
        P = n < sp.cap ? n : sp.cap;
    }
    const long ntiles = (P + F32_PTS_PER_WG - 1) / F32_PTS_PER_WG;
    constexpr bool XW_AHEAD = MODE == FIELD_RADIANCE_TRUNK && !DIAG_NOLOADS_TRUNK;
    f32x4 nx_a = f32x4{0.0f, 0.0f, 0.0f, 0.0f};
    float nx_w1 = 0.0f;
    int nx_src = 0;
    for (long tile = blockIdx.x; tile < ntiles; tile += gridDim.x) {
        cx.refresh();
        int q_tile = cx.q;
        if constexpr (TRUNK) { asm volatile("" : "+s"(cx.off)); asm volatile("" : "+v"(q_tile)); }
        const int q = q_tile;
        const long p_raw = tile * F32_PTS_PER_WG + cx.wave * F32_PTS_PER_WAVE + (cx.lane & 15);
        const long p = p_raw < P ? p_raw : P - 1;
        float *stash = lds + LDS_STASH_OFF + (cx.wave * F32_PTS_PER_WAVE + (cx.lane & 15)) * STASH_FLOATS;
        const bool dump = MODE == FIELD_ALL && dbg != nullptr && q == 0 && p_raw < P;
        float *dsl = dbg + p * DBG_STRIDE;
        const bool sv_on = SAVE && p_raw < P;
        long Psv = P;
        if constexpr (SAVE) asm volatile("" : "+s"(Psv));
#define SVP(c, w) (actbuf + (long)(c) * Psv + p * (long)(w) + 4 * q)
#define SV(c, w) SVP(c, w)
        const bool sb_on = sv_on && bits != nullptr;
        uint32_t *const bits_r = bits + (MODE == FIELD_ALL ? (long)sbits::BD_WORDS * Psv : 0L);
        const uint32_t sb_lane = (uint32_t)(p * 4 + q);
#define SBD(b, w) (sb_on ? bits + (long)(b) * Psv + sb_lane * (uint32_t)((w) >= 128 ? (w) / 128 : 1) : nullptr)
#define SBR(b, w) (sb_on ? bits_r + (long)(b) * Psv + sb_lane * (uint32_t)((w) >= 128 ? (w) / 128 : 1) : nullptr)
        float x[3] = {0.0f, 0.0f, 0.0f};
        long smp = p;
        if constexpr ((TRUNK && DIAG_NOLOADS_TRUNK) || (BRANCH && DIAG_NOLOADS_BRANCH)) {
            const float t = (float)(p & 1023) * (1.0f / 1024.0f);
            x[0] = t - 0.5f; x[1] = 0.25f - t; x[2] = 0.8f - t;
            if (q == 0 && (XW_IN || BRANCH)) { stash[0] = x[0]; stash[1] = x[1]; stash[2] = x[2]; stash[3] = t; stash[4] = -t; }
        } else if constexpr (BRANCH) {
            const f32x4 a = sp.hdr[p];
            smp = __float_as_int(a[3]);
            if (q == 0) { stash[0] = a[0]; stash[1] = a[1]; stash[2] = a[2]; }
        } else if constexpr (!XW_IN) {
            const float *rp = rays + (p / S) * ray_stride;
            const float z = zvals[p];
#pragma unroll
            for (int i = 0; i < 3; ++i) x[i] = rp[i] + rp[3 + i] * z;
        } else if constexpr (XW_AHEAD) {
            if (q == 0) {
                if (tile == (long)blockIdx.x) {
                    const float *row = xw + ((p / S) * (long)xw_row + src[p]) * 8;
                    nx_a = *reinterpret_cast<const f32x4 *>(row);
                    nx_w1 = row[4];
                }
                stash[0] = nx_a[0]; stash[1] = nx_a[1]; stash[2] = nx_a[2]; stash[3] = nx_a[3]; stash[4] = nx_w1;
            }
        } else if (q == 0) {
            const float *row = xw + ((p / S) * (long)xw_row + src[p]) * 8;
            const f32x4 a = *reinterpret_cast<const f32x4 *>(row);
            stash[0] = a[0]; stash[1] = a[1]; stash[2] = a[2]; stash[3] = a[3]; stash[4] = row[4];
            if (sv_on) { float *d = SVP(act::XW, 16); d[0] = a[0]; d[1] = a[1]; d[2] = a[2]; }
        }
        const bool has_next = XW_AHEAD && tile + gridDim.x < ntiles;
        const long pn_raw = p_raw + (long)gridDim.x * F32_PTS_PER_WG;
        const long p_next = pn_raw < P ? pn_raw : P - 1;
        if constexpr (XW_AHEAD) {
            if (has_next && q == 0) nx_src = src[p_next];
        }
        if constexpr (!XW_IN && !BRANCH) {
#if SAHS_MODEL == 2
        if (q == 0) {
            stash[0] = x[0]; stash[1] = x[1]; stash[2] = x[2]; stash[3] = 0.0f; stash[4] = 0.0f;
            if (sv_on) { float *d = SVP(act::XW, 16); d[0] = x[0]; d[1] = x[1]; d[2] = x[2]; }
        }
#else
        f32x4 pe_x[KB_XYZ];
        {
            if constexpr (TRUNK && DIAG_NOENC) diag_blocks<KB_XYZ>(x, q, pe_x);
            else pe_blocks<3, L_XYZ, KB_XYZ>(x, q, pe_x);
            if (sv_on) {
#pragma unroll
                for (int b = 0; b < KB_XYZ; ++b) *reinterpret_cast<f32x4 *>(SVP(act::E, 16 * KB_XYZ) + 16 * b) = pe_x[b];
            }
        }
        {
            f32x4 h[8], hn[8];
            dense_sv<SAVE, KB_XYZ, 0, 8, CHF(L_W1)>(cx, pe_x, nullptr, h, Ly[L_W0].bias_off, false, 0.0f, SV(act::WH, 128), SBD(sbits::BD_WH + 4 * (0), 128));
            constexpr int W_ROLLED = (CHF(L_W4B) == CHF(L_W2)) ? 3 : 2;
#pragma unroll 1
            for (int l = 0; l < W_ROLLED; ++l) {
                dense_sv<SAVE, 8, 0, 8, CHF(L_W2)>(cx, h, nullptr, hn, Ly[L_W1].bias_off + 128 * l, false, 0.0f, SV(act::WH + 128 * (l + 1), 128), SBD(sbits::BD_WH + 4 * ((l + 1)), 128));
#pragma unroll
                for (int i = 0; i < 8; ++i) h[i] = hn[i];
            }
            if (W_ROLLED == 2) {
                dense_sv<SAVE, 8, 0, 8, CHF(L_W4B)>(cx, h, nullptr, hn, Ly[L_W3].bias_off, false, 0.0f, SV(act::WH + 128 * 3, 128), SBD(sbits::BD_WH + 4 * (3), 128));
#pragma unroll
                for (int i = 0; i < 8; ++i) h[i] = hn[i];
            }
            dense<KB_XYZ, 0, 8, CHF(L_W4A)>(cx, pe_x, nullptr, hn, Ly[L_W4B].bias_off, false, 1.0f);
            dense_sv<SAVE, 8, 0, 8, CHF(L_W5)>(cx, h, nullptr, hn, 0, true, 0.0f, SV(act::WH + 4 * 128, 128), SBD(sbits::BD_WH + 4 * (4), 128));
            dense_sv<SAVE, 8, 0, 8, CHF(L_WF)>(cx, hn, nullptr, h, Ly[L_W5].bias_off, false, 0.0f, SV(act::WH + 5 * 128, 128), SBD(sbits::BD_WH + 4 * (5), 128));
            f32x4 o[1];
            dense<8, 0, 1, CHF(L_H0)>(cx, h, nullptr, o, Ly[L_WF].bias_off, false, 1.0f);
            if (q == 0) {
#pragma unroll
                for (int i = 0; i < 3; ++i) {
                    const float dxv = tanhf(o[0][i]);
                    stash[i] = x[i] + dxv;
                    if (sv_on) { SVP(act::DX, 16)[i] = dxv; SVP(act::XW, 16)[i] = x[i] + dxv; }
                }
            }
        }
        {
            f32x4 h[4], hn[4];
            dense_sv<SAVE, KB_XYZ, 0, 4, CHF(L_H1)>(cx, pe_x, nullptr, h, Ly[L_H0].bias_off, false, 0.0f, SV(act::HH, 64), SBD(sbits::BD_HH + 4 * (0), 64));
            constexpr int H_ROLLED = (CHF(L_H4B) == CHF(L_H2)) ? 3 : 2;
#pragma unroll 1
            for (int l = 0; l < H_ROLLED; ++l) {
                dense_sv<SAVE, 4, 0, 4, CHF(L_H2)>(cx, h, nullptr, hn, Ly[L_H1].bias_off + 64 * l, false, 0.0f, SV(act::HH + 64 * (l + 1), 64), SBD(sbits::BD_HH + 4 * ((l + 1)), 64));
#pragma unroll
                for (int i = 0; i < 4; ++i) h[i] = hn[i];
            }
            if (H_ROLLED == 2) {
                dense_sv<SAVE, 4, 0, 4, CHF(L_H4B)>(cx, h, nullptr, hn, Ly[L_H3].bias_off, false, 0.0f, SV(act::HH + 64 * 3, 64), SBD(sbits::BD_HH + 4 * (3), 64));
#pragma unroll
                for (int i = 0; i < 4; ++i) h[i] = hn[i];
            }
            dense<KB_XYZ, 0, 4, CHF(L_H4A)>(cx, pe_x, nullptr, hn, Ly[L_H4B].bias_off, false, 1.0f);
            dense_sv<SAVE, 4, 0, 4, CHF(L_H5)>(cx, h, nullptr, hn, 0, true, 0.0f, SV(act::HH + 4 * 64, 64), SBD(sbits::BD_HH + 4 * (4), 64));
            dense_sv<SAVE, 4, 0, 4, CHF(L_HF)>(cx, hn, nullptr, h, Ly[L_H5].bias_off, false, 0.0f, SV(act::HH + 5 * 64, 64), SBD(sbits::BD_HH + 4 * (5), 64));
            f32x4 o[1];
            dense<4, 0, 1, (MODE == FIELD_DEFORM ? CHF(L_FIRST) : CHF(L_T0))>(cx, h, nullptr, o, Ly[L_HF].bias_off, false, 1.0f);
            if (q == 0) {
                stash[3] = o[0][0]; stash[4] = (AMB_DIM > 1) ? o[0][1] : 0.0f;
                if (sv_on) { SVP(act::AW, 16)[0] = o[0][0]; SVP(act::AW, 16)[1] = stash[4]; }
            }
        }
#endif
        if (xw != nullptr && q == 0 && p_raw < P) {
            float *row = xw + ((p / S) * (long)xw_row + xw_col0 + (p % S)) * 8;
            *reinterpret_cast<f32x4 *>(row) = f32x4{stash[0], stash[1], stash[2], stash[3]};
            row[4] = stash[4];
        }
        }
        if constexpr (MODE == FIELD_DEFORM) continue;
        __builtin_amdgcn_wave_barrier();
        if (dump) { dsl[0] = stash[0] - x[0]; dsl[1] = stash[1] - x[1]; dsl[2] = stash[2] - x[2]; dsl[3] = stash[3]; dsl[4] = stash[4]; }

        f32x4 fin[1];
        f32x4 feat[16];
        if constexpr (BRANCH && DIAG_NOLOADS_BRANCH) {
            fin[0] = f32x4{x[0], x[1], x[2], x[0]};
#pragma unroll
            for (int b = 0; b < 16; ++b) feat[b] = f32x4{x[0] * (float)b, x[1], x[2] + (float)q, x[0]};
        } else if constexpr (BRANCH) {
            fin[0] = *reinterpret_cast<const f32x4 *>(raw + smp * D_RAW + 4 * q);
            const f32x4 *rec = sp.feat + (p >> 4) * (16 * 64) + q * 16 + (p & 15);
#pragma unroll
            for (int b = 0; b < 16; ++b) feat[b] = rec[b * 64];
        } else {
            f32x4 h[16];
            if constexpr (TRUNK) {
                constexpr bool ENC_ONCE = MODE == FIELD_RADIANCE_TRUNK && !DIAG_ENC2;
                f32x4 in_tr[KB_XYZ + KB_AMB];
                auto build_enc = [&]() {
                    const float xw[3] = {stash[0], stash[1], stash[2]}, amb[2] = {stash[3], stash[4]};
                    if constexpr (DIAG_NOENC) {
                        diag_blocks<KB_XYZ>(xw, q, in_tr);
                        diag_blocks<KB_AMB>(amb, q, in_tr + KB_XYZ);
                    } else {
                        pe_blocks<3, L_XYZ, KB_XYZ>(xw, q, in_tr);
#if SAHS_MODEL != 2
                        pe_blocks<AMB_DIM, L_AMB, KB_AMB, AMB_INC>(amb, q, in_tr + KB_XYZ);
#else
                        (void)amb;
#endif
                    }
                };
                build_enc();
                dense<KB_XYZ, KB_AMB, 16, CHF(L_T1)>(cx, in_tr, in_tr + KB_XYZ, h, Ly[L_T0].bias_off, false, 0.01f);
                dense<16, 0, 16, CHF(L_T2)>(cx, h, nullptr, feat, Ly[L_T1].bias_off, false, 0.01f);
#pragma unroll
                for (int i = 0; i < 16; ++i) h[i] = feat[i];
                dense<16, 0, 16, CHF(L_T3B)>(cx, h, nullptr, feat, Ly[L_T2].bias_off, false, 0.01f);
#pragma unroll
                for (int i = 0; i < 16; ++i) h[i] = feat[i];
                if constexpr (XW_AHEAD) {
                    if (has_next && q == 0) {
                        const float *row = xw + ((p_next / S) * (long)xw_row + nx_src) * 8;
                        nx_a = *reinterpret_cast<const f32x4 *>(row);
                        nx_w1 = row[4];
                    }
                }
                if constexpr (!ENC_ONCE) build_enc();
                dense<KB_XYZ, KB_AMB, 16, CHF(L_T3A)>(cx, in_tr, in_tr + KB_XYZ, feat, Ly[L_T3B].bias_off, false, 1.0f);
            } else {
            {
                f32x4 in_tr[KB_XYZ + KB_AMB];
                const float xw[3] = {stash[0], stash[1], stash[2]}, amb[2] = {stash[3], stash[4]};
                pe_blocks<3, L_XYZ, KB_XYZ>(xw, q, in_tr);
#if SAHS_MODEL != 2
                pe_blocks<AMB_DIM, L_AMB, KB_AMB, AMB_INC>(amb, q, in_tr + KB_XYZ);
#else
                (void)amb;
#endif
                if (sv_on) {
#pragma unroll
                    for (int b = 0; b < KB_XYZ + KB_AMB; ++b)
                        *reinterpret_cast<f32x4 *>(b < KB_XYZ ? SVP(act::PEX, 16 * KB_XYZ) + 16 * b : SVP(act::PEW, 16 * KB_AMB) + 16 * (b - KB_XYZ)) = in_tr[b];
                }
                dense_sv<SAVE, KB_XYZ, KB_AMB, 16, CHF(L_T1)>(cx, in_tr, in_tr + KB_XYZ, h, Ly[L_T0].bias_off, false, 0.01f, SV(act::T, 256), SBR(sbits::BR_T + 8 * (0), 256));
            }
            if (dump) dsl[5] = h[0][0];
            dense_sv<SAVE, 16, 0, 16, CHF(L_T2)>(cx, h, nullptr, feat, Ly[L_T1].bias_off, false, 0.01f, SV(act::T + 256, 256), SBR(sbits::BR_T + 8 * (1), 256));
            if (dump) dsl[6] = feat[0][0];
#pragma unroll
            for (int i = 0; i < 16; ++i) h[i] = feat[i];
            dense_sv<SAVE, 16, 0, 16, CHF(L_T3B)>(cx, h, nullptr, feat, Ly[L_T2].bias_off, false, 0.01f, SV(act::T + 512, 256), SBR(sbits::BR_T + 8 * (2), 256));
            if (dump) dsl[7] = feat[0][0];
#pragma unroll
            for (int i = 0; i < 16; ++i) h[i] = feat[i];
            {
                f32x4 in_tr[KB_XYZ + KB_AMB];
                const float xw[3] = {stash[0], stash[1], stash[2]}, amb[2] = {stash[3], stash[4]};
                pe_blocks<3, L_XYZ, KB_XYZ>(xw, q, in_tr);
#if SAHS_MODEL != 2
                pe_blocks<AMB_DIM, L_AMB, KB_AMB, AMB_INC>(amb, q, in_tr + KB_XYZ);
#else
                (void)amb;
#endif
                dense<KB_XYZ, KB_AMB, 16, CHF(L_T3A)>(cx, in_tr, in_tr + KB_XYZ, feat, Ly[L_T3B].bias_off, false, 1.0f);
            }
            }
#if SAHS_MODEL == 0
            dense_sv<SAVE, 16, 0, 16, CHF(L_T4)>(cx, h, nullptr, feat, 0, true, 0.01f, SV(act::T + 768, 256), SBR(sbits::BR_T + 8 * (3), 256));
#else
            dense_sv<SAVE, 16, 0, 16, CHF(L_FEAT)>(cx, h, nullptr, feat, 0, true, 0.01f, SV(act::T + 768, 256), SBR(sbits::BR_T + 8 * (3), 256));
#endif
            if (dump) dsl[8] = feat[0][0];
#pragma unroll
            for (int i = 0; i < 16; ++i) h[i] = feat[i];
#if SAHS_MODEL == 0
#pragma unroll 1
            for (int l = 4; l <= 7; ++l) {
                dense_sv<SAVE, 16, 0, 16, CHF(L_T5)>(cx, h, nullptr, feat, Ly[L_T4].bias_off + 256 * (l - 4), false, 0.01f, SV(act::T + 256 * l, 256), SBR(sbits::BR_T + 8 * (l), 256));
                if (dump) dsl[5 + l] = feat[0][0];
#pragma unroll
                for (int i = 0; i < 16; ++i) h[i] = feat[i];
            }
#endif
            dense_sv<SAVE, 16, 0, 16, CHF(L_ALPHA)>(cx, h, nullptr, feat, Ly[L_FEAT].bias_off, false, 1.0f, SV(act::FEAT, 256));
            if (dump) dsl[13] = feat[0][0];
        }
        if constexpr (!BRANCH) dense<16, 0, 1, (TRUNK ? CHF(L_START) : CHF(L_D0B))>(cx, feat, nullptr, fin, Ly[L_ALPHA].bias_off, false, 1.0f);
        if constexpr (TRUNK) {
            if (p_raw < P) *reinterpret_cast<f32x4 *>(raw + p * D_RAW + 4 * q) = fin[0];
            const long ray = p / S;
            const bool last = (p - ray * S) == S - 1;
            const float sg = fin[0][3] + (sp.noise != nullptr ? sp.noise[p] : 0.0f);
            const bool live = q == 3 && p_raw < P && (last ? sp.has_bg == 0 : sg > 0.0f);
            const uint32_t mask = (uint32_t)(__ballot(live) >> 48);
            if (!DIAG_NOAPPEND && mask != 0u) {
                uint32_t base = 0u;
                if (cx.lane == 0) base = atomicAdd(sp.count, (unsigned int)__popc(mask));
                base = (uint32_t)__builtin_amdgcn_readfirstlane((int)base);
                const int j = cx.lane & 15;
                const uint32_t slot = base + (uint32_t)__popc(mask & ((1u << j) - 1u));
                if (((mask >> j) & 1u) && slot < sp.cap) {
                    f32x4 *rec = sp.feat + (long)(slot >> 4) * (16 * 64) + q * 16 + (slot & 15u);
#pragma unroll
                    for (int b = 0; b < 16; ++b) rec[b * 64] = feat[b];
                    if (q == 0) sp.hdr[slot] = f32x4{stash[0], stash[1], stash[2], __int_as_float((int)p)};
                }
            }
            continue;
        }
        if (dbg != nullptr && p_raw < P) *reinterpret_cast<f32x4 *>(dsl + 24 + 4 * q) = fin[0];
        {
            f32x4 in_d[4];
            {
                if constexpr (BRANCH && DIAG_NOLOADS_BRANCH) {
                    pe_blocks<3, 4, 2>(x, q, in_d);
                    diag_blocks<2>(x, q, in_d + 2);
                } else if constexpr (BRANCH && DIAG_NOENC) {
                    const float *rp = rays + (smp / S) * ray_stride;
                    const float rd[3] = {rp[3], rp[4], rp[5]};
                    diag_blocks<2>(rd, q, in_d);
                    grid_blocks(grid, stash[0], stash[1], stash[2], q, in_d + 2);
                } else {
                const float *rp = rays + (smp / S) * ray_stride;
                const float rd[3] = {rp[3], rp[4], rp[5]};
                pe_blocks<3, 4, 2>(rd, q, in_d);
                grid_blocks(grid, stash[0], stash[1], stash[2], q, in_d + 2);
                }
                if (sv_on) {
#pragma unroll
                    for (int b = 0; b < 4; ++b) *reinterpret_cast<f32x4 *>(b < 2 ? SVP(act::DIR, 32) + 16 * b : SVP(act::GRID, 32) + 16 * (b - 2)) = in_d[b];
                }
            }
            if (dbg != nullptr && p_raw < P) {
                float *d = dbg + P * DBG_STRIDE + p * 32;
                *reinterpret_cast<f32x4 *>(d + 4 * q) = in_d[2];
                *reinterpret_cast<f32x4 *>(d + 16 + 4 * q) = in_d[3];
            }
            f32x4 c[8], cn[8];
            dense<2, 2, 8, CHF(L_D0A)>(cx, in_d, in_d + 2, c, Ly[L_D0B].bias_off, false, 1.0f);
            dense_sv<SAVE, 16, 0, 8, CHF(L_D1)>(cx, feat, nullptr, c, 0, true, 0.01f, SV(act::C, 128), SBR(sbits::BR_C + 4 * (0), 128));
            if (dump) dsl[14] = c[0][0];
#pragma unroll 1
            for (int l = 0; l < 2; ++l) {
                dense_sv<SAVE, 8, 0, 8, CHF(L_D2)>(cx, c, nullptr, cn, Ly[L_D1].bias_off + 128 * l, false, 0.01f, SV(act::C + 128 * (l + 1), 128), SBR(sbits::BR_C + 4 * ((l + 1)), 128));
#pragma unroll
                for (int i = 0; i < 8; ++i) c[i] = cn[i];
            }
            dense_sv<SAVE, 8, 0, 8, CHF(L_RGB)>(cx, c, nullptr, cn, Ly[L_D3].bias_off, false, 0.01f, SV(act::C + 384, 128), SBR(sbits::BR_C + 4 * (3), 128));
            if (dump) dsl[15] = cn[0][0];
            dense<8, 0, 1, CHF(L_S0)>(cx, cn, nullptr, fin, 0, true, 1.0f);
            if (dbg != nullptr && p_raw < P) *reinterpret_cast<f32x4 *>(dsl + 40 + 4 * q) = fin[0];
        }
        {
            f32x4 s[8], sn[8];
            dense_sv<SAVE, 16, 0, 8, CHF(L_S1)>(cx, feat, nullptr, s, Ly[L_S0].bias_off, false, 0.01f, SV(act::S, 128), SBR(sbits::BR_S + 4 * (0), 128));
            if (dump) dsl[16] = s[0][0];
#pragma unroll 1
            for (int l = 0; l < 2; ++l) {
                dense_sv<SAVE, 8, 0, 8, CHF(L_S2)>(cx, s, nullptr, sn, Ly[L_S1].bias_off + 128 * l, false, 0.01f, SV(act::S + 128 * (l + 1), 128), SBR(sbits::BR_S + 4 * ((l + 1)), 128));
#pragma unroll
                for (int i = 0; i < 8; ++i) s[i] = sn[i];
            }
            dense_sv<SAVE, 8, 0, 8, CHF(L_SEG)>(cx, s, nullptr, sn, Ly[L_S3].bias_off, false, 0.01f, SV(act::S + 384, 128), SBR(sbits::BR_S + 4 * (3), 128));
            if (dump) dsl[17] = sn[0][0];
            dense<8, 0, 1, CHF(L_START)>(cx, sn, nullptr, fin, 0, true, 1.0f);
        }
        if (p_raw < P) *reinterpret_cast<f32x4 *>(raw + smp * D_RAW + 4 * q) = fin[0];
    }
}

}

using namespace SAHS_NS;

template <bool SAVE, int MODE>
static int launch_field(const float *packed, const float *frame, int level, long P, int S, const float *rays, int ray_stride, const float *zvals,
                        float *raw, float *dbg, float *actbuf, float *xw, int xw_row, int xw_col0, const int *src, int num_cu, hipStream_t stream,
                        uint32_t *bits = nullptr, SparseArgs sp = SparseArgs{})
{
    const long ntiles = (P + F32_PTS_PER_WG - 1) / F32_PTS_PER_WG;
    const int grid = (int)(ntiles < num_cu ? ntiles : num_cu);
    const size_t lds_bytes = (size_t)LDS_TOTAL_FLOATS * sizeof(float);
    static sahs_once::Flags attr_set;
    hipError_t ae = sahs_once::per_device(attr_set, [&]() {
        return hipFuncSetAttribute(reinterpret_cast<const void *>(field_forward_f32_kernel<SAVE, MODE>), hipFuncAttributeMaxDynamicSharedMemorySize,
                                   (int)lds_bytes);
    });
    if (ae != hipSuccess) return (int)ae;
    field_forward_f32_kernel<SAVE, MODE><<<grid, F32_THREADS, lds_bytes, stream>>>(packed, frame, level, P, S, rays, ray_stride, zvals, raw, dbg, actbuf,
                                                                                   xw, xw_row, xw_col0, src, bits, sp);
    return (int)hipGetLastError();
}

extern "C" int SAHS_SYM(sahs_field_forward_f32_launch)(const float *packed, const float *frame, int level, long P, int S, const float *rays,
                                             int ray_stride, const float *zvals, float *raw, float *dbg, float *actbuf, int num_cu,
                                             hipStream_t stream)
{
    if (P <= 0) return 0;
    if (actbuf != nullptr)
        return launch_field<true, FIELD_ALL>(packed, frame, level, P, S, rays, ray_stride, zvals, raw, dbg, actbuf, nullptr, 0, 0, nullptr, num_cu, stream);
    return launch_field<false, FIELD_ALL>(packed, frame, level, P, S, rays, ray_stride, zvals, raw, dbg, nullptr, nullptr, 0, 0, nullptr, num_cu, stream);
}

extern "C" int SAHS_SYM(sahs_field_forward_f32_split_launch)(const float *packed, const float *frame, int level, int mode, long P, int S,
                                                   const float *rays, int ray_stride, const float *zvals, float *raw, float *xw, int xw_row,
                                                   int xw_col0, const int *src, float *actbuf, int num_cu, hipStream_t stream)
{
    return SAHS_SYM(sahs_field_forward_f32_split_bits_launch)(packed, frame, level, mode, P, S, rays, ray_stride, zvals, raw, xw, xw_row, xw_col0, src, actbuf,
                                                              nullptr, num_cu, stream);
}
extern "C" int SAHS_SYM(sahs_field_forward_f32_split_bits_launch)(const float *packed, const float *frame, int level, int mode, long P, int S,
                                                   const float *rays, int ray_stride, const float *zvals, float *raw, float *xw, int xw_row,
                                                   int xw_col0, const int *src, float *actbuf, uint32_t *bits, int num_cu, hipStream_t stream)
{
    if (P <= 0) return 0;
#if SAHS_MODEL == 2
    if (mode != FIELD_ALL || actbuf == nullptr) return -3;
    return launch_field<true, FIELD_ALL>(packed, frame, level, P, S, rays, ray_stride, zvals, raw, nullptr, actbuf, xw, xw_row, xw_col0, nullptr, num_cu, stream, bits);
#else
    if (actbuf != nullptr) {
        if (mode == FIELD_ALL)
            return launch_field<true, FIELD_ALL>(packed, frame, level, P, S, rays, ray_stride, zvals, raw, nullptr, actbuf, xw, xw_row, xw_col0, nullptr, num_cu, stream, bits);
        if (mode == FIELD_DEFORM)
            return launch_field<true, FIELD_DEFORM>(packed, frame, level, P, S, rays, ray_stride, zvals, nullptr, nullptr, actbuf, xw, xw_row, xw_col0, nullptr, num_cu, stream, bits);
        if (mode == FIELD_RADIANCE)
            return launch_field<true, FIELD_RADIANCE>(packed, frame, level, P, S, rays, ray_stride, nullptr, raw, nullptr, actbuf, xw, xw_row, 0, src, num_cu, stream, bits);
        return -2;
    }
    if (mode == FIELD_ALL)
        return launch_field<false, FIELD_ALL>(packed, frame, level, P, S, rays, ray_stride, zvals, raw, nullptr, nullptr, xw, xw_row, xw_col0, nullptr, num_cu, stream);
    if (mode == FIELD_DEFORM)
        return launch_field<false, FIELD_DEFORM>(packed, frame, level, P, S, rays, ray_stride, zvals, nullptr, nullptr, nullptr, xw, xw_row, xw_col0, nullptr, num_cu, stream);
    if (mode == FIELD_RADIANCE)
        return launch_field<false, FIELD_RADIANCE>(packed, frame, level, P, S, rays, ray_stride, nullptr, raw, nullptr, nullptr, xw, xw_row, 0, src, num_cu, stream);
    return -2;
#endif
}

extern "C" long SAHS_SYM(sahs_field_f32_sparse_ws_bytes)(long cap) { return SPARSE_HEAD_BYTES + cap * SPARSE_RECORD_BYTES; }
extern "C" int SAHS_SYM(sahs_field_forward_f32_sparse_launch)(const float *packed, const float *frame, int level, int stage, long P, int S,
                                                    const float *rays, int ray_stride, const float *zvals, float *raw, float *xw, int xw_row,
                                                    int xw_col0, const int *src, const float *noise, int has_bg, void *ws, long cap, int num_cu,
                                                    hipStream_t stream)
{
    if (P <= 0) return 0;
    if (ws == nullptr || cap < P || cap % F32_PTS_PER_WG != 0 || cap > (1L << 30)) return -4;
    char *base = static_cast<char *>(ws);
    SparseArgs sp{noise, reinterpret_cast<unsigned int *>(base), reinterpret_cast<f32x4 *>(base + SPARSE_HEAD_BYTES),
                  reinterpret_cast<f32x4 *>(base + SPARSE_HEAD_BYTES + cap * 16), (unsigned int)cap, has_bg};
    if (stage == 0)
        return launch_field<false, FIELD_ALL_TRUNK>(packed, frame, level, P, S, rays, ray_stride, zvals, raw, nullptr, nullptr, xw, xw_row, xw_col0, nullptr, num_cu, stream, nullptr, sp);
    if (stage == 2)
        return launch_field<false, FIELD_BRANCH>(packed, frame, level, P, S, rays, ray_stride, nullptr, raw, nullptr, nullptr, nullptr, 0, 0, nullptr, num_cu, stream, nullptr, sp);
#if SAHS_MODEL != 2
    if (stage == 1)
        return launch_field<false, FIELD_RADIANCE_TRUNK>(packed, frame, level, P, S, rays, ray_stride, nullptr, raw, nullptr, nullptr, xw, xw_row, 0, src, num_cu, stream, nullptr, sp);
#endif
    return -2;
}

extern "C" int SAHS_SYM(sahs_layout_act_part_words)(int part) { return part == 1 ? act::XW + 16 : (part == 2 ? act::STRIDE - act::XW : act::STRIDE); }
extern "C" int SAHS_SYM(sahs_layout_act_part_col0)(int part) { return part == 2 ? act::XW : 0; }
extern "C" int SAHS_SYM(sahs_layout_bits_part_words)(int part) { return part == 1 ? sbits::BD_WORDS : (part == 2 ? sbits::BR_WORDS : sbits::BD_WORDS + sbits::BR_WORDS); }
```

sahs-deformable-nerf_amd/csrc/sahs_launchers.hpp:

```cpp
#pragma once
#include <hip/hip_runtime.h>
#include <cstdint>

extern "C" {
int sahs_ray_bundle_launch(int H, int W, float fx, float fy, float cx, float cy, const float *c2w, int ld, float *ro, float *rd,
                           hipStream_t stream);
int sahs_stratified_depths_launch(long N, int S, const float *rays, int ray_stride, int lindisp, const float *t_rand, float *z,
                                  hipStream_t stream);
int sahs_composite_forward_launch(long N, int S, const float *raw, const float *z, const float *rays, int ray_stride, const float *noise,
                                  const float *bg, int white_bkgd, float *rgb_map, float *disp, float *acc_map, float *weights,
                                  float *depth, float *w_last, int rgb_ld, int sc_ld, hipStream_t stream);
int sahs_route_xw_grad_launch(long N, int Sc, int nf, const int *src, const float *g_fine, float *g_coarse, float *g_new, hipStream_t stream);
int sahs_resample_launch(long N, int S, int nf, int from_z, const float *z, const float *weights, const float *u, float *z_samples,
                         float *z_out, long long *inds, int *src, hipStream_t stream);
int sahs_ray_uniforms_launch(unsigned long long seed, int stream_id, long ray0, long N, int S, float *out, hipStream_t stream);
long sahs_spade_stats_words(long planes);
int sahs_spade_modulate_launch(long planes, long hw, const float *x, const float *gamma, const float *beta, float eps, float slope, float *out,
                               float *stats, hipStream_t stream);
int sahs_adam_step_launch(float *params, const float *grad, float *exp_avg, float *exp_avg_sq, long n, float w1, float beta2, float w2,
                          float step_size, float bc2_sqrt, float eps, float grad_scale, hipStream_t stream);
int sahs_composite_backward_launch(long N, int S, const float *raw, const float *z, const float *rays, int ray_stride, const float *noise,
                                   const float *bg, int white_bkgd, const float *d_rgb, const float *d_disp, const float *d_acc,
                                   const float *d_depth, const float *d_wlast, const float *d_weights, float *d_raw, const float *loss_map,
                                   const float *loss_target, int target_ld, const float *loss_mask, const float *loss_stats,
                                   const float *loss_gscale, hipStream_t stream);
int sahs_stage1_loss_forward_launch(long N, const float *map_c, const float *map_f, const float *target, int target_ld, const float *mask,
                                    const float *class_w, float *stats, hipStream_t stream);
int sahs_conditioning_backward_launch(const float *flat, const float *audio, const float *grad_cond, float *grad_flat, float *grad_audio,
                                      hipStream_t stream);

#define SAHS_DECLARE_MODEL(sfx)                                                                                                          \
                                                                                                                           \
    long sahs_layout_param_count##sfx(void);                                                                                            \
    long sahs_layout_packed_words_f32##sfx(void);                                                                                       \
    long sahs_layout_packed_words_bf16##sfx(void);                                                                                      \
    long sahs_layout_packed_words_bf16x3##sfx(void);                                                                                    \
    long sahs_layout_frame_words##sfx(void);                                                                                            \
    long sahs_layout_act_words##sfx(void);                                                                                              \
    long sahs_layout_executed_macs##sfx(int precision, int part);                                                                       \
    int sahs_pack_weights_f32_launch##sfx(const float *flat, float *packed, hipStream_t stream);                                       \
    int sahs_pack_weights_bf16_launch##sfx(const float *flat, float *packed, hipStream_t stream);                                      \
    int sahs_pack_weights_bf16x3_launch##sfx(const float *flat, float *packed, hipStream_t stream);                                    \
    int sahs_fold_conditioning_launch##sfx(const float *flat, const float *audio, const float *pose, int pose_ld, float *frame,        \
                                           hipStream_t stream);                                                                         \
                                                                                                                      \
    int sahs_layout_act_part_words##sfx(int part);                                                                                      \
    int sahs_layout_act_part_col0##sfx(int part);                                                                                       \
    int sahs_layout_bits_part_words##sfx(int part);                                                                                     \
    int sahs_field_forward_f32_launch##sfx(const float *packed, const float *frame, int level, long P, int S, const float *rays,       \
                                           int ray_stride, const float *zvals, float *raw, float *dbg, float *actbuf, int num_cu,       \
                                           hipStream_t stream);                                                                         \
    int sahs_field_forward_f32_split_launch##sfx(const float *packed, const float *frame, int level, int mode, long P, int S,          \
                                                 const float *rays, int ray_stride, const float *zvals, float *raw, float *xw,          \
                                                 int xw_row, int xw_col0, const int *src, float *actbuf, int num_cu,                    \
                                                 hipStream_t stream);                                                                   \
    int sahs_field_forward_f32_split_bits_launch##sfx(const float *packed, const float *frame, int level, int mode, long P, int S,     \
                                                      const float *rays, int ray_stride, const float *zvals, float *raw, float *xw,     \
                                                      int xw_row, int xw_col0, const int *src, float *actbuf, uint32_t *bits,           \
                                                      int num_cu, hipStream_t stream);                                                  \
    long sahs_field_f32_sparse_ws_bytes##sfx(long cap);                                                                                 \
    int sahs_field_forward_f32_sparse_launch##sfx(const float *packed, const float *frame, int level, int stage, long P, int S,        \
                                                  const float *rays, int ray_stride, const float *zvals, float *raw, float *xw,         \
                                                  int xw_row, int xw_col0, const int *src, const float *noise, int has_bg, void *ws,    \
                                                  long cap, int num_cu, hipStream_t stream);                                            \
                                                                                                                    \
    int sahs_bf16w_exact_leaky_state##sfx(int set);                                                                                     \
    int sahs_field_forward_bf16w_launch##sfx(const float *packed, const float *frame, int level, long P, int S, const float *rays,     \
                                             int ray_stride, const float *zvals, float *raw, float *dbg, int num_cu, hipStream_t stream); \
    int sahs_field_forward_bf16w_split_launch##sfx(const float *packed, const float *frame, int level, int mode, long P, int S,        \
                                                   const float *rays, int ray_stride, const float *zvals, float *raw, float *xw,        \
                                                   int xw_row, int xw_col0, const int *src, int num_cu, hipStream_t stream);            \
                                                                                                                   \
    int sahs_field_deform_bf16x3_launch##sfx(const float *packed, const float *frame, int level, long P, int S, const float *rays,     \
                                             int ray_stride, const float *zvals, float *xw, int xw_row, int xw_col0, int num_cu,        \
                                             hipStream_t stream);                                                                       \
    int sahs_field_deform_bf16x3_save_launch##sfx(const float *packed, const float *frame, int level, long P, int S,                  \
                                                  const float *rays, int ray_stride, const float *zvals, float *xw, int xw_row,         \
                                                  int xw_col0, float *actbuf, uint32_t *bits, int num_cu, hipStream_t stream);          \
    int sahs_field_radiance_bf16x3_launch##sfx(const float *packed, const float *frame, int level, long P, int S, const float *rays,   \
                                               int ray_stride, float *raw, const float *xw, int xw_row, const int *src, int num_cu,     \
                                               hipStream_t stream);                                                                     \
    int sahs_field_radiance_bf16x3_save_launch##sfx(const float *packed, const float *frame, int level, long P, int S,                \
                                                    const float *rays, int ray_stride, float *raw, const float *xw, int xw_row,         \
                                                    const int *src, float *actbuf, uint32_t *bits, int num_cu, hipStream_t stream);     \
    int sahs_field_forward_bf16x3_launch##sfx(const float *packed, const float *frame, int level, long P, int S, const float *rays,    \
                                              int ray_stride, const float *zvals, float *raw, int num_cu, hipStream_t stream);          \
    int sahs_field_forward_bf16x3_save_launch##sfx(const float *packed, const float *frame, int level, long P, int S,                  \
                                                   const float *rays, int ray_stride, const float *zvals, float *raw, float *actbuf,    \
                                                   uint32_t *bits, int num_cu, hipStream_t stream);                                     \
                                                                                                                      \
    int sahs_bwd_gemm_precision_state##sfx(int set);                                                                                    \
    long sahs_field_backward_ws_words##sfx(long P);                                                                                     \
    int sahs_field_backward_launch##sfx(const float *flat, const float *frame, int level, long P, const float *actbuf,                  \
                                        const float *d_raw, float *grad_flat, float *grad_cond, float *ws, hipStream_t stream);         \
    int sahs_field_backward_split_launch##sfx(const float *flat, const float *frame, int level, int part, long P, const float *actbuf,  \
                                              const float *d_raw, const float *xwg_in, float *xwg_out, float *grad_flat,                \
                                              float *grad_cond, float *ws, hipStream_t stream);                                         \
    long sahs_field_backward_fused_ws_words##sfx(int part, long P);                                                                     \
    int sahs_field_backward_fused_launch##sfx(const float *flat, const float *frame, int level, int part, long P, const float *actbuf,  \
                                              const uint32_t *bits, const float *d_raw, const float *xwg_in, float *xwg_out,            \
                                              float *grad_flat, float *grad_cond, float *ws, int num_cu, hipStream_t stream);           \
                                                  \
    long sahs_bwd_chain_stream_hw##sfx(int part);                                                                                       \
    int sahs_bwd_chain_pack_launch##sfx(const float *flat, void *stream_out, int level, int part, hipStream_t stream);                 \
    int sahs_bwd_chain_rad_launch##sfx(const void *bstream, long P, const float *d_raw, const uint32_t *bits, float *dact,             \
                                       float *dgridf, float *din_a, float *din_b, int num_cu, hipStream_t stream);                      \
    int sahs_bwd_chain_def_launch##sfx(const void *bstream, long P, const float *xwg, const float *actbuf, const uint32_t *bits,       \
                                       float *dact, float *g3, float *dw4, int num_cu, hipStream_t stream);                             \
                                                                   \
    long sahs_bwd_chain_f32_stream_floats##sfx(int part);                                                                               \
    int sahs_bwd_chain_f32_pack_launch##sfx(const float *flat, float *stream_out, int level, int part, hipStream_t stream);             \
    int sahs_bwd_chain_f32_rad_launch##sfx(const float *bstream, long P, const float *d_raw, const uint32_t *bits, float *dact,         \
                                           float *dgridf, float *din_a, float *din_b, int num_cu, hipStream_t stream);                  \
    int sahs_bwd_chain_f32_def_launch##sfx(const float *bstream, long P, const float *xwg, const float *actbuf, const uint32_t *bits,   \
                                           float *dact, float *g3, float *dw4, int num_cu, hipStream_t stream);
SAHS_DECLARE_MODEL()
SAHS_DECLARE_MODEL(_nf)
SAHS_DECLARE_MODEL(_ns)
#undef SAHS_DECLARE_MODEL
}
```

sahs-deformable-nerf_amd/ops.py:

```python
import ctypes
import os
import types

import torch

from . import _lib
from ._lib import SAHS_F32, SAHS_BF16, SAHS_BF16X3, check

PRECISIONS = {"fp32": SAHS_F32, "f32": SAHS_F32, "bf16": SAHS_BF16,
              "bf16x3": SAHS_BF16X3}


def is_mixed(arch, precision):
    return (precision == SAHS_BF16 and arch == "nerface") or (precision == SAHS_BF16X3 and arch in ("audio", "nerface"))


def _p(t):
    return None if t is None else ctypes.c_void_p(t.data_ptr())


def _stream():
    return ctypes.c_void_p(torch.cuda.current_stream().cuda_stream)


def _req(t, name, dtype=torch.float32):
    if t is None:
        return None
    if not isinstance(t, torch.Tensor) or not t.is_cuda:
        raise _lib.SahsError("%s must be a GPU tensor (the HIP path has no CPU fallback)" % name)
    if t.dtype != dtype:
        raise _lib.SahsError("%s must be %s, got %s" % (name, dtype, t.dtype))
    if t.device.index != torch.cuda.current_device():
        raise _lib.SahsError("%s lives on %s but the current device is cuda:%d: one process drives one GPU (call "
                             "torch.cuda.set_device first, as torchrun-style launchers do)" % (name, t.device, torch.cuda.current_device()))
    return t if t.is_contiguous() else t.contiguous()


ARCHS = ("audio", "nerface", "nerface_static")


def _fn(name, arch="audio"):
    if arch not in ARCHS:
        raise _lib.SahsError("unknown architecture %r" % (arch,))
    full = "sahs_model_" + name
    f = getattr(_lib.lib(), full)
    m = ARCHS.index(arch)
    return (lambda *a: f(m, *a)), full + "(%s)" % arch


def param_count(arch="audio"):
    return int(_fn("param_count", arch)[0]())


def executed_macs_per_sample(arch="audio", precision=SAHS_F32, part=0):
    return int(_fn("executed_macs_part", arch)[0](precision, part))


def pack_weights(flat, precision=SAHS_F32, arch="audio"):
    flat = _req(flat, "flat_params")
    if flat.numel() != param_count(arch):
        raise _lib.SahsError("flat_params has %d values, expected %d" % (flat.numel(), param_count(arch)))
    words = _fn("packed_words", arch)[0](precision)
    if words <= 0:
        raise _lib.SahsError("precision %r is not built for architecture %r" % (precision, arch))
    packed = torch.empty(words, dtype=torch.float32, device=flat.device)
    f, name = _fn("pack_weights", arch)
    check(f(_p(flat), _p(packed), precision, _stream()), name)
    return packed


def fold_conditioning(flat, audio, pose, arch="audio"):
    flat, audio = _req(flat, "flat_params"), _req(audio, "audio")
    pose = _req(pose, "pose")
    want = (16, 29) if arch == "audio" else (76,)
    if tuple(audio.shape) != want:
        raise _lib.SahsError("driving input must be %s for %r, got %s" % (want, arch, tuple(audio.shape)))
    if pose.dim() != 2 or pose.shape[0] < 3 or pose.shape[1] != 4:
        raise _lib.SahsError("pose must be (3|4, 4), got %s" % (tuple(pose.shape),))
    frame = torch.empty(_fn("frame_words", arch)[0](), dtype=torch.float32, device=flat.device)
    f, name = _fn("fold_conditioning", arch)
    check(f(_p(flat), _p(audio), _p(pose), 4, _p(frame), _stream()), name)
    return frame


def get_ray_bundle(height, width, intrinsics, c2w):
    c2w = _req(c2w, "tform_cam2world")
    fx, fy, cx, cy = [float(v) for v in intrinsics]
    ro = torch.empty(height, width, 3, dtype=torch.float32, device=c2w.device)
    rd = torch.empty_like(ro)
    check(_lib.lib().sahs_get_ray_bundle(int(height), int(width), fx, fy, cx, cy, _p(c2w), int(c2w.shape[-1]), _p(ro), _p(rd), _stream()),
          "sahs_get_ray_bundle")
    return ro, rd


def ray_uniforms(seed, stream_id, ray0, num_rays, num_samples, device):
    out = torch.empty(int(num_rays), int(num_samples), dtype=torch.float32, device=device)
    check(_lib.lib().sahs_ray_uniforms(int(seed) & (2 ** 64 - 1), int(stream_id), int(ray0), int(num_rays), int(num_samples), _p(out), _stream()),
          "sahs_ray_uniforms")
    return out


def stratified_depths(rays, num_samples, lindisp=False, t_rand=None):
    rays, t_rand = _req(rays, "rays"), _req(t_rand, "t_rand")
    N = rays.shape[0]
    z = torch.empty(N, num_samples, dtype=torch.float32, device=rays.device)
    check(_lib.lib().sahs_stratified_depths(N, int(num_samples), _p(rays), int(rays.shape[1]), int(bool(lindisp)), _p(t_rand), _p(z),
                                             _stream()), "sahs_stratified_depths")
    return z


def field_forward(packed, frame, level, rays, z, precision=SAHS_F32, debug=False, out=None, arch="audio"):
    packed, frame, rays, z = _req(packed, "packed"), _req(frame, "frame"), _req(rays, "rays"), _req(z, "z")
    N, S = z.shape
    if rays.shape[0] != N or rays.shape[1] < 8:
        raise _lib.SahsError("rays must be (N, >=8) with N == z.shape[0]")
    raw = out if out is not None else torch.empty(N, S, 16, dtype=torch.float32, device=z.device)
    dbg = torch.zeros(N * S * 88, dtype=torch.float32, device=z.device) if debug else None
    f, name = _fn("field_forward", arch)
    check(f(_p(packed), _p(frame), int(level), N, S, _p(rays), int(rays.shape[1]), _p(z), _p(raw), _p(dbg), precision, _stream()), name)
    if debug == "full":
        return raw, dbg[: N * S * 56].view(N * S, 56), dbg[N * S * 56:].view(N * S, 32)
    if debug:
        a = dbg[: N * S * 56].view(N * S, 56)
        return raw, a[:, 0:3].reshape(N, S, 3), a[:, 3:5].reshape(N, S, 2), dbg[N * S * 56:].view(N, S, 32)
    return raw


def composite_forward(raw, z, rays, noise=None, bg=None, white_background=False):
    raw, z, rays, noise, bg = _req(raw, "radiance_field"), _req(z, "depth_values"), _req(rays, "rays"), _req(noise, "noise"), _req(bg, "background_prior")
    N, S = z.shape
    dev = z.device
    rgb = torch.empty(N, 15, dtype=torch.float32, device=dev)
    disp, acc, depth = (torch.empty(N, dtype=torch.float32, device=dev) for _ in range(3))
    weights = torch.empty(N, S, dtype=torch.float32, device=dev)
    check(_lib.lib().sahs_composite_forward(N, S, _p(raw), _p(z), _p(rays), int(rays.shape[1]), _p(noise), _p(bg), int(bool(white_background)),
                                             _p(rgb), _p(disp), _p(acc), _p(weights), _p(depth), _stream()), "sahs_composite_forward")
    return rgb, disp, acc, weights, depth


def resample(z, weights, num_fine, u=None, want_aux=False):
    z, weights, u = _req(z, "z_vals"), _req(weights, "weights"), _req(u, "u")
    N, S = z.shape
    z_out = torch.empty(N, S + num_fine, dtype=torch.float32, device=z.device)
    zs = torch.empty(N, num_fine, dtype=torch.float32, device=z.device) if want_aux else None
    inds = torch.empty(N, num_fine, dtype=torch.int64, device=z.device) if want_aux else None
    check(_lib.lib().sahs_resample(N, S, int(num_fine), _p(z), _p(weights), _p(u), _p(zs), _p(z_out), _p(inds), _stream()), "sahs_resample")
    return (z_out, zs, inds) if want_aux else z_out


def resample_merge(z, weights, num_fine, u=None):
    z, weights, u = _req(z, "z_vals"), _req(weights, "weights"), _req(u, "u")
    N, S = z.shape
    z_out = torch.empty(N, S + num_fine, dtype=torch.float32, device=z.device)
    z_new = torch.empty(N, num_fine, dtype=torch.float32, device=z.device)
    src = torch.empty(N, S + num_fine, dtype=torch.int32, device=z.device)
    check(_lib.lib().sahs_resample_merge(N, S, int(num_fine), _p(z), _p(weights), _p(u), _p(z_new), _p(z_out), _p(src), _stream()), "sahs_resample_merge")
    return z_out, z_new, src


FIELD_ALL, FIELD_DEFORM, FIELD_RADIANCE = 0, 1, 2


def field_forward_split(packed, frame, level, mode, rays, xw, z=None, src=None, xw_col0=0, out=None, arch="audio", precision=SAHS_F32,
                        validate_src=False):
    packed, frame, rays, z = _req(packed, "packed"), _req(frame, "frame"), _req(rays, "rays"), _req(z, "z")
    src = _req(src, "src", torch.int32)
    xw = _req(xw, "xw")
    N = rays.shape[0]
    S = src.shape[1] if mode == FIELD_RADIANCE else z.shape[1]
    if xw.dim() != 3 or xw.shape[0] != N or xw.shape[2] != 8:
        raise _lib.SahsError("xw must be (N, row, 8)")
    if src is not None and (src.dim() != 2 or src.shape[0] != N):
        raise _lib.SahsError("src must be (N, S)")
    if validate_src and src is not None and src.numel() and not (0 <= int(src.min()) and int(src.max()) < xw.shape[1]):
        raise _lib.SahsError("src indexes outside xw's %d slots per ray" % xw.shape[1])
    raw = None
    if mode != FIELD_DEFORM:
        raw = out if out is not None else torch.empty(N, S, 16, dtype=torch.float32, device=rays.device)
    f, name = _fn("field_forward_split", arch)
    check(f(_p(packed), _p(frame), int(precision), int(level), int(mode), N, int(S), _p(rays), int(rays.shape[1]), _p(z), _p(raw), _p(xw), int(xw.shape[1]), int(xw_col0),
            _p(src), _stream()), name)
    return raw


def sample_pdf(bins, weights, num_samples, u=None, want_inds=False):
    bins, weights, u = _req(bins, "bins"), _req(weights, "weights"), _req(u, "u")
    N, nb = bins.shape
    if tuple(weights.shape) != (N, nb - 1):
        raise _lib.SahsError("weights must be (N, nb-1)")
    out = torch.empty(N, num_samples, dtype=torch.float32, device=bins.device)
    inds = torch.empty(N, num_samples, dtype=torch.int64, device=bins.device) if want_inds else None
    check(_lib.lib().sahs_sample_pdf(N, nb, int(num_samples), _p(bins), _p(weights), _p(u), _p(out), _p(inds), _stream()), "sahs_sample_pdf")
    return (out, inds) if want_inds else out


def _workspace_buffer(ws, dev, name, shape, dtype=torch.float32):
    t = ws.get(name)
    if t is None or tuple(t.shape) != tuple(shape) or t.device != dev:
        t = ws[name] = torch.empty(*shape, dtype=dtype, device=dev)
    return t


def _req_rows(rows, N):
    if not (isinstance(rows, torch.Tensor) and rows.is_cuda and rows.dtype == torch.float32 and rows.dim() == 2 and rows.shape[0] == N
            and rows.shape[1] >= ROW_COLUMNS and rows.stride(1) == 1):
        raise _lib.SahsError("rows must be a GPU fp32 (N, >=36) tensor with unit column stride")


def render_rays(packed, frame, rays, num_coarse, num_fine, precision=SAHS_F32, lindisp=False, white_background=False, bg=None,
                t_rand=None, noise_c=None, u=None, noise_f=None, workspace=None, arch="audio"):
    if is_mixed(arch, precision):
        rows = torch.empty(rays.shape[0], ROW_COLUMNS, dtype=torch.float32, device=rays.device)
        render_rays_rows(packed, frame, rays, num_coarse, num_fine, rows, precision=precision, lindisp=lindisp, white_background=white_background,
                         bg=bg, t_rand=t_rand, noise_c=noise_c, u=u, noise_f=noise_f, workspace=workspace, arch=arch)
        return tuple(c.contiguous() for c in (rows[:, 0:15], rows[:, 15], rows[:, 16], rows[:, 17:32], rows[:, 32], rows[:, 33], rows[:, 34], rows[:, 35]))
    packed, frame, rays = _req(packed, "packed"), _req(frame, "frame"), _req(rays, "rays")
    bg, t_rand, noise_c, u, noise_f = (_req(t, n) for t, n in ((bg, "background_prior"), (t_rand, "t_rand"), (noise_c, "noise_c"),
                                                               (u, "u"), (noise_f, "noise_f")))
    N = rays.shape[0]
    dev = rays.device
    Sf = num_coarse + num_fine
    ws = workspace if workspace is not None else {}
    buf = lambda name, *shape: _workspace_buffer(ws, dev, name, shape)
    z_c, z_f = buf("z_c", N, num_coarse), buf("z_f", N, Sf)
    raw, weights = buf("raw", N, Sf, 16), buf("weights", N, Sf)
    rgb_c, rgb_f = (torch.empty(N, 15, dtype=torch.float32, device=dev) for _ in range(2))
    disp_c, acc_c, disp_f, acc_f, w_bg, depth_f = (torch.empty(N, dtype=torch.float32, device=dev) for _ in range(6))
    f, name = _fn("render_rays", arch)
    check(f(_p(packed), _p(frame), precision, N, _p(rays), int(rays.shape[1]), int(num_coarse), int(num_fine),
            int(bool(lindisp)), int(bool(white_background)), _p(bg), _p(t_rand), _p(noise_c), _p(u), _p(noise_f),
            _p(z_c), _p(z_f), _p(raw), _p(weights), _p(rgb_c), _p(disp_c), _p(acc_c), _p(rgb_f), _p(disp_f),
            _p(acc_f), _p(w_bg), _p(depth_f), _stream()), name)
    if num_fine > 0:
        return rgb_c, disp_c, acc_c, rgb_f, disp_f, acc_f, w_bg, depth_f
    return rgb_c, disp_c, acc_c, None, None, None, w_bg, depth_f


_SPARSE_WORKSPACE_BYTES = 4 << 30
_SPARSE_BRANCHES = True


def sparse_branches(on=None, workspace_bytes=None):
    global _SPARSE_BRANCHES, _SPARSE_WORKSPACE_BYTES
    if on is not None:
        if not isinstance(on, (bool, int)) or on not in (0, 1, False, True):
            raise _lib.SahsError("sparse_branches: True or False, not %r" % (on,))
        _SPARSE_BRANCHES = bool(on)
    if workspace_bytes is not None:
        if not isinstance(workspace_bytes, int) or isinstance(workspace_bytes, bool) or workspace_bytes < 1:
            raise _lib.SahsError("sparse_branches: workspace_bytes must be a positive int, not %r" % (workspace_bytes,))
        _SPARSE_WORKSPACE_BYTES = workspace_bytes
    return _SPARSE_BRANCHES


def sparse_workspace_bytes():
    return _SPARSE_WORKSPACE_BYTES


def sparse_last_count(workspace):
    rec = workspace.get("sparse") if workspace else None
    if rec is None:
        raise _lib.SahsError("sparse_last_count: this workspace has not been through a sparse render")
    return int(rec[:4].view(torch.int32).item())


ROW_COLUMNS = 36


def composite_forward_rows(raw, z, rays, rows, fine_pass, noise=None, bg=None, white_background=False, weights=None):
    raw, z, rays, noise, bg = _req(raw, "radiance_field"), _req(z, "depth_values"), _req(rays, "rays"), _req(noise, "noise"), _req(bg, "background_prior")
    N, S = z.shape
    _req_rows(rows, N)
    if weights is None or tuple(weights.shape) != (N, S):
        weights = torch.empty(N, S, dtype=torch.float32, device=z.device)
    check(_lib.lib().sahs_composite_forward_rows(N, S, _p(raw), _p(z), _p(rays), int(rays.shape[1]), _p(noise), _p(bg), int(bool(white_background)),
                                                  _p(weights), _p(rows), int(rows.stride(0)), int(bool(fine_pass)), _stream()), "sahs_composite_forward_rows")
    return weights


def render_rays_rows(packed, frame, rays, num_coarse, num_fine, rows, precision=SAHS_F32, lindisp=False, white_background=False, bg=None,
                     t_rand=None, noise_c=None, u=None, noise_f=None, workspace=None, arch="audio", share_deformation=True):
    packed, frame, rays = _req(packed, "packed"), _req(frame, "frame"), _req(rays, "rays")
    bg, t_rand, noise_c, u, noise_f = (_req(t, n) for t, n in ((bg, "background_prior"), (t_rand, "t_rand"), (noise_c, "noise_c"),
                                                               (u, "u"), (noise_f, "noise_f")))
    N = rays.shape[0]
    _req_rows(rows, N)
    dev = rays.device
    Sf = num_coarse + num_fine
    ws = workspace if workspace is not None else {}
    buf = lambda name, *shape: _workspace_buffer(ws, dev, name, shape)
    z_c, z_f = buf("z_c", N, num_coarse), buf("z_f", N, Sf)
    raw, weights = buf("raw", N, Sf, 16), buf("weights", N, Sf)
    xw = src = z_new = None
    mixed = is_mixed(arch, precision)
    if mixed and not (share_deformation and num_fine > 0):
        raise _lib.SahsError("a mixed-precision model renders through the split chain (share_deformation=True, num_fine > 0)")
    if share_deformation and num_fine > 0 and arch != "nerface_static" and precision in (SAHS_F32, SAHS_BF16, SAHS_BF16X3):
        xw, z_new = buf("xw", N, Sf, 8), buf("z_new", N, num_fine)
        src = _workspace_buffer(ws, dev, "src", (N, Sf), torch.int32)
    extra = []
    if _SPARSE_BRANCHES and precision == SAHS_F32 and N > 0:
        want = min(int(_fn("render_sparse_workspace_bytes", arch)[0](min(N * Sf, 1 << 30))), _SPARSE_WORKSPACE_BYTES)
        extra = [_p(_workspace_buffer(ws, dev, "sparse", (want,), torch.uint8)), want]
    f, name = _fn("render_rays_rows_sparse" if extra else "render_rays_rows", arch)
    check(f(_p(packed), _p(frame), precision, N, _p(rays), int(rays.shape[1]), int(num_coarse), int(num_fine),
            int(bool(lindisp)), int(bool(white_background)), _p(bg), _p(t_rand), _p(noise_c), _p(u), _p(noise_f),
            _p(z_c), _p(z_f), _p(raw), _p(weights), _p(rows), int(rows.stride(0)), _p(xw), _p(src), _p(z_new), *extra, _stream()), name)
    return rows


def spade_modulate(x, gamma, beta, eps=1e-5, slope=1.0):
    x, gamma, beta = _req(x, "x"), _req(gamma, "gamma"), _req(beta, "beta")
    if x.dim() != 4 or gamma.shape != x.shape or beta.shape != x.shape:
        raise _lib.SahsError("spade_modulate: x, gamma, beta must be NCHW tensors of one shape, got %s %s %s" % (tuple(x.shape), tuple(gamma.shape), tuple(beta.shape)))
    planes, hw = x.shape[0] * x.shape[1], x.shape[2] * x.shape[3]
    out = torch.empty_like(x)
    stats = torch.empty(int(_lib.lib().sahs_spade_modulate_workspace_words(planes)), dtype=torch.float32, device=x.device)
    check(_lib.lib().sahs_spade_modulate(planes, hw, _p(x), _p(gamma), _p(beta), float(eps), float(slope), _p(out), _p(stats), _stream()), "sahs_spade_modulate")
    return out


def adam_step(params, grad, exp_avg, exp_avg_sq, lr, beta1=0.9, beta2=0.999, eps=1e-8, step=1, grad_scale=1.0):
    for t, name in ((params, "params"), (grad, "grad"), (exp_avg, "exp_avg"), (exp_avg_sq, "exp_avg_sq")):
        if _req(t, name) is not t:
            raise _lib.SahsError("adam_step: %s must be contiguous" % name)
        if t.numel() != params.numel():
            raise _lib.SahsError("adam_step: %s has %d values, params has %d" % (name, t.numel(), params.numel()))
    check(_lib.lib().sahs_adam_step(_p(params), _p(grad), _p(exp_avg), _p(exp_avg_sq), params.numel(), float(lr), float(beta1), float(beta2),
                                    float(eps), int(step), float(grad_scale), _stream()), "sahs_adam_step")
    return params


class LaunchProbe:

    def __init__(self, capacity=4096):
        self.capacity = int(capacity)

    def __enter__(self):
        check(_lib.lib().sahs_probe_arm(self.capacity), "sahs_probe_arm")
        return self

    def __exit__(self, *exc):
        _lib.lib().sahs_probe_disarm()
        return False

    @staticmethod
    def records():
        L = _lib.lib()
        if L.sahs_probe_dropped():
            raise _lib.SahsError("launch probe overflow: %d launches were not recorded" % L.sahs_probe_dropped())
        out = []
        kind, samples, ms = ctypes.c_int(), ctypes.c_long(), ctypes.c_float()
        for i in range(L.sahs_probe_count()):
            check(L.sahs_probe_read(i, ctypes.byref(kind), ctypes.byref(samples), ctypes.byref(ms)), "sahs_probe_read")
            k = kind.value
            out.append(dict(model=ARCHS[k >> 16], level=(k >> 12) & 15, part=(k >> 8) & 15, precision=k & 255, samples=samples.value, ms=ms.value))
        return out


def field_forward_save(packed, frame, level, rays, z, arch="audio", bits=None, precision=SAHS_F32):
    packed, frame, rays, z = _req(packed, "packed"), _req(frame, "frame"), _req(rays, "rays"), _req(z, "z")
    N, S = z.shape
    x3 = int(precision) == SAHS_BF16X3
    if int(precision) not in (SAHS_F32, SAHS_BF16X3) or (x3 and bits is None):
        raise _lib.SahsError("field_forward_save: fp32, or SAHS_BF16X3 with the sign bits (bits=alloc_sign_bits(...))")
    raw = torch.empty(N, S, 16, dtype=torch.float32, device=z.device)
    act = torch.empty(N * S, _fn("act_words_per_sample", arch)[0](), dtype=torch.float32, device=z.device)
    if bits is not None:
        bits = _req(bits, "bits", torch.int32)
        if tuple(bits.shape) != (N * S, int(_fn("bits_words_part", arch)[0](FIELD_ALL))):
            raise _lib.SahsError("field_forward_save: bits must come from alloc_sign_bits(N * S, FIELD_ALL, arch, device)")
    f, name = _fn("field_forward_save" + ("" if bits is None else "_bits_x3" if x3 else "_bits"), arch)
    out = [_p(act)] if bits is None else [_p(act), _p(bits)]
    check(f(_p(packed), _p(frame), int(level), N, S, _p(rays), int(rays.shape[1]), _p(z), _p(raw), *out, _stream()), name)
    return raw, act


def field_backward(flat, frame, level, act, d_raw, grad_flat, grad_cond, arch="audio"):
    flat, frame, act, d_raw = _req(flat, "flat_params"), _req(frame, "frame"), _req(act, "act"), _req(d_raw, "d_raw")
    P = act.shape[0]
    ws = torch.empty(_fn("field_backward_workspace_words", arch)[0](P), dtype=torch.float32, device=act.device)
    f, name = _fn("field_backward", arch)
    check(f(_p(flat), _p(frame), int(level), P, _p(act), _p(d_raw), _p(grad_flat), _p(grad_cond), _p(ws), _stream()), name)


def alloc_sign_bits(num_samples, mode, arch, device):
    words = int(_fn("bits_words_part", arch)[0](int(mode)))
    return torch.empty(int(num_samples), words, dtype=torch.int32, device=device) if words > 0 else None


def _whole_save_part(act, bits, part, arch, P):
    if int(part) != FIELD_RADIANCE:
        return _p(act), _p(bits)
    words, bwords = _fn("act_words_part", arch)[0], _fn("bits_words_part", arch)[0]
    offs = 4 * (int(words(FIELD_ALL)) - int(words(FIELD_RADIANCE))) * P, 4 * int(bwords(FIELD_DEFORM)) * P
    if offs[0] % 16 or offs[1] % 16:
        raise _lib.SahsError("the radiance part of a whole-network save of N*S = %d samples starts at byte %d (activations) / %d (sign bits): "
                             "not multiples of 16" % (P, offs[0], offs[1]))
    return ctypes.c_void_p(act.data_ptr() + offs[0]), None if bits is None else ctypes.c_void_p(bits.data_ptr() + offs[1])


def field_forward_split_save(packed, frame, level, mode, rays, xw, z=None, src=None, xw_col0=0, arch="audio", bits=None, precision=SAHS_F32, whole=None):
    packed, frame, rays, z = _req(packed, "packed"), _req(frame, "frame"), _req(rays, "rays"), _req(z, "z")
    src, xw = _req(src, "src", torch.int32), _req(xw, "xw")
    N = rays.shape[0]
    S = src.shape[1] if mode == FIELD_RADIANCE else z.shape[1]
    if xw.dim() != 3 or xw.shape[0] != N or xw.shape[2] != 8:
        raise _lib.SahsError("xw must be (N, row, 8)")
    raw = None if mode == FIELD_DEFORM else torch.empty(N, S, 16, dtype=torch.float32, device=rays.device)
    words, bwords = _fn("act_words_part", arch)[0], _fn("bits_words_part", arch)[0]
    if whole is not None:
        act, bits = _req(whole[0], "whole act"), _req(whole[1], "whole bits", torch.int32)
        if int(mode) not in (FIELD_DEFORM, FIELD_RADIANCE) or tuple(act.shape) != (N * S, int(words(FIELD_ALL))) or tuple(bits.shape) != (N * S, int(bwords(FIELD_ALL))):
            raise _lib.SahsError("field_forward_split_save(whole): buffers of a FIELD_ALL save of the same samples, filled by a FIELD_DEFORM or FIELD_RADIANCE launch")
        act_ptr, bits_ptr = _whole_save_part(act, bits, mode, arch, N * S)
    else:
        act = torch.empty(N * S, words(int(mode)), dtype=torch.float32, device=rays.device)
        if bits is not None:
            bits = _req(bits, "bits", torch.int32)
            if tuple(bits.shape) != (N * S, int(bwords(int(mode)))):
                raise _lib.SahsError("field_forward_split_save: bits must come from alloc_sign_bits(N * S, mode, arch, device)")
        elif int(precision) != SAHS_F32:
            raise _lib.SahsError("field_forward_split_save: a saving forward at a precision other than fp32 needs the sign bits (bits=alloc_sign_bits(...))")
        act_ptr, bits_ptr = _p(act), _p(bits)
    f, name = _fn("field_forward_split_save" + ("" if bits is None else "_bits_x3" if int(precision) == SAHS_BF16X3 else "_bits"), arch)
    out = [act_ptr] if bits is None else [act_ptr, bits_ptr]
    check(f(_p(packed), _p(frame), int(level), int(mode), N, int(S), _p(rays), int(rays.shape[1]), _p(z), _p(raw), _p(xw), int(xw.shape[1]), int(xw_col0),
            _p(src), *out, _stream()), name)
    return raw, act


def fused_backward(enable=None):
    global _FUSED_BACKWARD
    if enable is not None:
        _FUSED_BACKWARD = bool(enable)
    return _FUSED_BACKWARD


_FUSED_BACKWARD = os.environ.get("SAHS_BWD_FUSED", "1") != "0"


def training_forward_precision(precision=None):
    global _TRAIN_FORWARD
    if precision is not None:
        if precision not in ("fp32", "bf16x3"):
            raise _lib.SahsError("training_forward_precision: 'fp32' or 'bf16x3'")
        _TRAIN_FORWARD = precision
    return _TRAIN_FORWARD


_TRAIN_FORWARD = os.environ.get("SAHS_TRAIN_FORWARD", "fp32")
if _TRAIN_FORWARD not in ("fp32", "bf16x3"):
    raise _lib.SahsError("SAHS_TRAIN_FORWARD must be 'fp32' or 'bf16x3', not %r" % (_TRAIN_FORWARD,))


def field_backward_split(flat, frame, level, part, act, grad_flat, grad_cond, d_raw=None, xw_grad_in=None, arch="audio", full_act=False, bits=None):
    flat, frame, act = _req(flat, "flat_params"), _req(frame, "frame"), _req(act, "act")
    d_raw, xw_grad_in = _req(d_raw, "d_raw"), _req(xw_grad_in, "xw_grad_in")
    P = act.shape[0]
    in_whole = bool(full_act) and int(part) in (FIELD_DEFORM, FIELD_RADIANCE)
    if act.shape[1] != _fn("act_words_part", arch)[0](3 if in_whole else int(part)):
        raise _lib.SahsError("field_backward_split(full_act): the activations were not saved by a whole-network forward" if in_whole else
                             "field_backward_split: the activations were not saved by a forward of part %d" % part)
    if xw_grad_in is not None and xw_grad_in.numel() != P * 8:
        raise _lib.SahsError("field_backward_split: xw_grad_in must hold (P,8)")
    out = torch.empty(P, 8, dtype=torch.float32, device=act.device) if part == FIELD_RADIANCE else None
    fused = bits is not None and _FUSED_BACKWARD
    bits = _req(bits, "bits", torch.int32) if fused else None
    if fused:
        saved_mode = 0 if (full_act or int(part) == 3) else int(part)
        if tuple(bits.shape) != (P, int(_fn("bits_words_part", arch)[0](saved_mode))):
            raise _lib.SahsError("field_backward_split: bits were not written by the forward that saved these activations")
    act_ptr, bits_ptr = _whole_save_part(act, bits, part, arch, P) if in_whole else (_p(act), _p(bits))
    if fused:
        ws = torch.empty(int(_fn("field_backward_fused_workspace_words", arch)[0](int(part), P)), dtype=torch.float32, device=act.device)
        f, name = _fn("field_backward_fused", arch)
        check(f(_p(flat), _p(frame), int(level), int(part), P, act_ptr, bits_ptr, _p(d_raw), _p(xw_grad_in), _p(out), _p(grad_flat), _p(grad_cond), _p(ws),
                _stream()), name)
        return out
    ws = torch.empty(_fn("field_backward_workspace_words", arch)[0](P), dtype=torch.float32, device=act.device)
    f, name = _fn("field_backward_split", arch)
    check(f(_p(flat), _p(frame), int(level), int(part), P, act_ptr, _p(d_raw), _p(xw_grad_in), _p(out), _p(grad_flat), _p(grad_cond), _p(ws), _stream()), name)
    return out


_SIDE_STREAMS = {}


def _side_stream(dev):
    key = torch.device(dev).index if torch.device(dev).index is not None else torch.cuda.current_device()
    if key not in _SIDE_STREAMS:
        _SIDE_STREAMS[key] = torch.cuda.Stream(device=key)
    return _SIDE_STREAMS[key]


def route_xw_grad(src, g_fine, num_coarse):
    src, g_fine = _req(src, "src", torch.int32), _req(g_fine, "g_fine")
    N, Sf = src.shape
    nf = Sf - int(num_coarse)
    g_c = torch.empty(N * int(num_coarse), 8, dtype=torch.float32, device=src.device)
    g_n = torch.empty(N * nf, 8, dtype=torch.float32, device=src.device)
    check(_lib.lib().sahs_route_xw_grad(N, int(num_coarse), nf, _p(src), _p(g_fine), _p(g_c), _p(g_n), _stream()), "sahs_route_xw_grad")
    return g_c, g_n


def backward_gemm_precision(precision=None):
    names = {SAHS_F32: "fp32", SAHS_BF16X3: "bf16x3"}
    if precision is None:
        return names[_lib.lib().sahs_backward_gemm_precision(-1)]
    code = PRECISIONS[precision] if isinstance(precision, str) else int(precision)
    if _lib.lib().sahs_backward_gemm_precision(code) != code:
        raise _lib.SahsError("backward GEMM precision must be 'fp32' or 'bf16x3'")
    return names[code]


def bf16_exact_leaky(enable=None):
    return bool(_lib.lib().sahs_bf16_exact_leaky(-1 if enable is None else int(bool(enable))))


LOSS_STATS_WORDS = 64


def stage1_loss_forward(map_coarse, map_fine, target, mask, class_weights):
    mc, mf = _req(map_coarse, "map_coarse"), _req(map_fine, "map_fine")
    target, mask, cw = _req(target, "target"), _req(mask, "mask"), _req(class_weights, "class_weights")
    ref = mc if mc is not None else mf
    N = ref.shape[0]
    if any(t is not None and tuple(t.shape) != (N, 15) for t in (mc, mf)) or tuple(mask.shape) != (N, 12) or target.shape[0] != N or cw.numel() != 12:
        raise _lib.SahsError("stage1_loss_forward: maps (N,15), target (N,>=3), mask (N,12), class_weights (12,)")
    stats = torch.zeros(LOSS_STATS_WORDS, dtype=torch.float32, device=ref.device)
    check(_lib.lib().sahs_stage1_loss_forward(N, _p(mc), _p(mf), _p(target), int(target.shape[1]), _p(mask), _p(cw), _p(stats), _stream()),
          "sahs_stage1_loss_forward")
    return stats


def composite_backward(raw, z, rays, noise, bg, white_background, d_rgb, d_disp, d_acc, d_depth, d_wlast, d_weights=None, loss=None):
    raw, z, rays = _req(raw, "raw"), _req(z, "z"), _req(rays, "rays")
    N, S = z.shape
    d_raw = torch.empty(N, S, 16, dtype=torch.float32, device=z.device)
    gs = [_req(g, n) for g, n in ((d_rgb, "d_rgb"), (d_disp, "d_disp"), (d_acc, "d_acc"), (d_depth, "d_depth"), (d_wlast, "d_wlast"))]
    head = (N, S, _p(raw), _p(z), _p(rays), int(rays.shape[1]), _p(_req(noise, "noise")), _p(_req(bg, "bg")), int(bool(white_background)),
            *[_p(g) for g in gs])
    if loss is None:
        check(_lib.lib().sahs_composite_backward(*head, _p(_req(d_weights, "d_weights")), _p(d_raw), _stream()), "sahs_composite_backward")
        return d_raw
    if d_weights is not None:
        raise _lib.SahsError("composite_backward: d_weights and loss together are not supported")
    lm, lt, lk, st, gsc = (_req(t, n) for t, n in zip(loss, ("loss_map", "loss_target", "loss_mask", "loss_stats", "loss_gscale")))
    if tuple(lm.shape) != (N, 15) or tuple(lk.shape) != (N, 12) or lt.shape[0] != N or st.numel() < LOSS_STATS_WORDS:
        raise _lib.SahsError("composite_backward: loss operands (N,15), (N,>=3), (N,12), stats (64,)")
    check(_lib.lib().sahs_composite_backward_loss(*head, _p(lm), _p(lt), int(lt.shape[1]), _p(lk), _p(st), _p(gsc), _p(d_raw), _stream()),
          "sahs_composite_backward_loss")
    return d_raw


def _save_named(ctx, **tensors):
    ctx.saved_names = tuple(tensors)
    ctx.save_for_backward(*tensors.values())


def _load_named(ctx):
    return types.SimpleNamespace(**dict(zip(ctx.saved_names, ctx.saved_tensors)))


def _driving_grad(arch, flat, driving, grad_flat, grad_cond):
    if arch != "audio":
        return grad_cond[:76].clone()
    grad_drv = torch.zeros_like(driving)
    check(_lib.lib().sahs_conditioning_backward(_p(flat), _p(driving), _p(grad_cond), _p(grad_flat), _p(grad_drv), _stream()),
          "sahs_conditioning_backward")
    return grad_drv


class CompositeFn(torch.autograd.Function):

    @staticmethod
    def forward(ctx, raw, z, rays, noise, bg, white_background):
        outs = composite_forward(raw, z, rays, noise=noise, bg=bg, white_background=white_background)
        _save_named(ctx, raw=raw.detach(), z=z, rays=rays, noise=noise, bg=bg, w_last=outs[3][:, -1])
        ctx.white_background = bool(white_background)
        return outs

    @staticmethod
    def backward(ctx, g_rgb, g_disp, g_acc, g_w, g_depth):
        s = _load_named(ctx)
        c = lambda t: None if t is None else t.contiguous().float()
        d_raw = composite_backward(s.raw, s.z, s.rays, s.noise, s.bg, ctx.white_background, c(g_rgb), c(g_disp), c(g_acc), c(g_depth), None, c(g_w))
        if s.bg is not None and g_rgb is not None:
            d_raw[:, -1, :15] += s.w_last[:, None] * g_rgb
        return d_raw, None, None, None, None, None


class FieldFn(torch.autograd.Function):

    BLOCK = 2_000_000

    @staticmethod
    def forward(ctx, flat, driving, pose, rays, z, packed, level, arch):
        frame = fold_conditioning(flat.detach(), driving.detach(), pose, arch=arch)
        N = z.shape[0]
        rows = max(1, FieldFn.BLOCK // max(1, z.shape[1]))
        raws, acts = [], {}
        for s in range(0, N, rows):
            r, acts["act%d" % len(raws)] = field_forward_save(packed, frame, level, rays[s:s + rows].contiguous(), z[s:s + rows].contiguous(), arch)
            raws.append(r)
        _save_named(ctx, flat=flat.detach(), driving=driving.detach(), frame=frame, **acts)
        ctx.level, ctx.arch, ctx.block, ctx.num_blocks = level, arch, rows * z.shape[1], len(raws)
        return raws[0] if len(raws) == 1 else torch.cat(raws, dim=0)

    @staticmethod
    def backward(ctx, g_raw):
        s = _load_named(ctx)
        acts = [getattr(s, "act%d" % i) for i in range(ctx.num_blocks)]
        grad_flat = torch.zeros_like(s.flat)
        grad_cond = torch.zeros(128, dtype=torch.float32, device=s.flat.device)
        g = g_raw.contiguous().float().view(-1, 16)
        if sum(a.shape[0] for a in acts) != g.shape[0]:
            raise _lib.SahsError("FieldFn.backward: %d gradient rows for %d saved samples" % (g.shape[0], sum(a.shape[0] for a in acts)))
        for i, act in enumerate(acts):
            field_backward(s.flat, s.frame, ctx.level, act, g[i * ctx.block: i * ctx.block + act.shape[0]], grad_flat, grad_cond, ctx.arch)
        return grad_flat, _driving_grad(ctx.arch, s.flat, s.driving, grad_flat, grad_cond), None, None, None, None, None, None


class RenderRaysFn(torch.autograd.Function):

    BLOCK_RAYS = 4096
    SHARE_DEFORMATION = True

    @staticmethod
    def forward(ctx, flat, audio, pose, rays, bg, t_rand, noise_c, u, noise_f, packed, num_coarse, num_fine, lindisp, white_background,
                arch="audio", loss_target=None, loss_mask=None, loss_weights=None, packed_x3=None):
        frame = fold_conditioning(flat.detach(), audio.detach(), pose, arch=arch)
        N, dev, Sf = rays.shape[0], rays.device, num_coarse + num_fine
        kept = N <= RenderRaysFn.BLOCK_RAYS and num_fine > 0
        shared = kept and RenderRaysFn.SHARE_DEFORMATION and arch != "nerface_static"
        ctx.strategy = "shared" if shared else "whole" if kept else "recompute"
        ctx.arch, ctx.num_coarse, ctx.num_fine, ctx.white_background = arch, num_coarse, num_fine, bool(white_background)
        saved = dict(flat=flat.detach(), audio=audio.detach(), rays=rays, frame=frame, packed=packed, bg=bg, noise_c=noise_c, noise_f=noise_f,
                     map_c=None, map_f=None, loss_target=None, loss_mask=None, loss_stats=None)
        sign_bits = lambda samples, mode: alloc_sign_bits(samples, mode, arch, dev) if (shared or arch == "nerface_static") else None
        bits0 = sign_bits(N * num_coarse, FIELD_ALL) if kept else None
        pk, prec = (packed_x3, SAHS_BF16X3) if (packed_x3 is not None and bits0 is not None) else (packed, SAHS_F32)
        xw = torch.empty(N, Sf, 8, dtype=torch.float32, device=dev) if shared else None

        def level_pass(level, z, noise, z_new=None, src=None):
            nonlocal xw
            if not shared:
                bits = bits0 if level == 0 else sign_bits(z.numel(), FIELD_ALL)
                raw, act = field_forward_save(pk, frame, level, rays, z, arch, bits=bits, precision=prec)
                saved.update({"act%d" % level: act, "bits%d" % level: bits})
            elif level == 0 and prec == SAHS_F32:
                raw, act = field_forward_split_save(pk, frame, 0, FIELD_ALL, rays, xw, z=z, arch=arch, bits=bits0)
                saved.update(act0=act, bits0=bits0)
            elif level == 0:
                whole = (torch.empty(N * num_coarse, _fn("act_words_part", arch)[0](FIELD_ALL), dtype=torch.float32, device=dev), bits0)
                field_forward_split_save(pk, frame, 0, FIELD_DEFORM, rays, xw, z=z, arch=arch, precision=prec, whole=whole)
                raw, _ = field_forward_split_save(pk, frame, 0, FIELD_RADIANCE, rays, xw, arch=arch, precision=prec, whole=whole,
                                                  src=torch.arange(num_coarse, dtype=torch.int32, device=dev).repeat(N, 1))
                saved.update(act0=whole[0], bits0=bits0)
            else:
                bits_d, bits_r = sign_bits(N * num_fine, FIELD_DEFORM), sign_bits(N * Sf, FIELD_RADIANCE)
                _, act_d = field_forward_split_save(pk, frame, 1, FIELD_DEFORM, rays, xw, z=z_new, xw_col0=num_coarse, arch=arch, bits=bits_d, precision=prec)
                raw, act_r = field_forward_split_save(pk, frame, 1, FIELD_RADIANCE, rays, xw, src=src, arch=arch, bits=bits_r, precision=prec)
                saved.update(act_d=act_d, bits_d=bits_d, act_r=act_r, bits_r=bits_r, src=src)
                xw = None
            saved["raw%d" % level] = raw
            return composite_forward(raw, z, rays, noise, bg, white_background)

        if kept:
            z_c = stratified_depths(rays, num_coarse, lindisp, t_rand)
            rgb_c, disp_c, acc_c, w_c, _ = level_pass(0, z_c, noise_c)
            z_f, z_new, src = resample_merge(z_c, w_c, num_fine, u=u) if shared else (resample(z_c, w_c, num_fine, u), None, None)
            rgb_f, disp_f, acc_f, w_f, depth_f = level_pass(1, z_f, noise_f, z_new, src)
            saved.update(z_c=z_c, z_f=z_f)
            outs = (rgb_c, disp_c, acc_c, rgb_f, disp_f, acc_f, w_f[:, -1].contiguous(), depth_f)
        else:
            ws = {}
            outs = render_rays(packed, frame, rays, num_coarse, num_fine, precision=SAHS_F32, lindisp=lindisp, white_background=white_background,
                               bg=bg, t_rand=t_rand, noise_c=noise_c, u=u, noise_f=noise_f, workspace=ws, arch=arch)
            saved.update(z_c=ws["z_c"].clone(), z_f=ws["z_f"].clone() if num_fine > 0 else None)
        if loss_target is not None:
            tgt, msk = loss_target.detach().float().contiguous(), loss_mask.detach().float().contiguous()
            rgb_f = outs[3] if num_fine > 0 else None
            stats = stage1_loss_forward(outs[0], rgb_f, tgt, msk, loss_weights.detach().float().contiguous())
            saved.update(map_c=outs[0], map_f=rgb_f, loss_target=tgt, loss_mask=msk, loss_stats=stats)
            ctx.mark_non_differentiable(stats)
            outs = tuple(outs) + (stats[0].clone(), stats)
        _save_named(ctx, **saved)
        return outs

    @staticmethod
    def backward(ctx, g_rgb_c, g_disp_c, g_acc_c, g_rgb_f, g_disp_f, g_acc_f, g_wbg, g_depth_f, g_loss=None, g_stats=None):
        grads = ({1: (g_rgb_f, g_disp_f, g_acc_f, g_depth_f, g_wbg), 0: (g_rgb_c, g_disp_c, g_acc_c, None, None)} if ctx.num_fine > 0 else
                 {0: (g_rgb_c, g_disp_c, g_acc_c, g_depth_f, g_wbg)})
        bw = _RenderBackward(ctx, _load_named(ctx), grads, g_loss)
        if (ctx.strategy == "shared" and not (bw.s.bits0 is not None and _FUSED_BACKWARD) and bw.has_grad[0] and bw.has_grad[1]
                and not os.environ.get("SAHS_BWD_ONE_STREAM")):
            bw.two_streams()
        else:
            bw.one_stream()
        return (bw.grad_flat, _driving_grad(ctx.arch, bw.s.flat, bw.s.audio, bw.grad_flat, bw.grad_cond)) + (None,) * 17


class _RenderBackward:

    def __init__(self, ctx, s, grads, g_loss):
        self.s, self.grads, self.arch, self.strategy, self.num_coarse, self.white = s, grads, ctx.arch, ctx.strategy, ctx.num_coarse, ctx.white_background
        self.z, self.noise, self.loss_map = {0: s.z_c, 1: s.z_f}, {0: s.noise_c, 1: s.noise_f}, {0: s.map_c, 1: s.map_f}
        self.gscale = g_loss.detach().float().reshape(1).contiguous() if (s.loss_stats is not None and g_loss is not None) else None
        self.has_grad = {level: self.gscale is not None or any(g is not None for g in gs) for level, gs in grads.items()}
        self.grad_flat = torch.zeros_like(s.flat)
        self.grad_cond = torch.zeros(128, dtype=torch.float32, device=s.rays.device)

    def composite(self, level, raw, sl=slice(None)):
        s = self.s
        cut = lambda t: None if t is None else t[sl].contiguous()
        loss = None if self.gscale is None else (cut(self.loss_map[level]), cut(s.loss_target), cut(s.loss_mask), s.loss_stats, self.gscale)
        return composite_backward(raw, cut(self.z[level]), cut(s.rays), cut(self.noise[level]), cut(s.bg), self.white,
                                  *[None if g is None else g[sl].contiguous().float() for g in self.grads[level]], loss=loss).view(-1, 16)

    def whole_walk(self, level, act, bits, d_raw, xw_grad_in=None):
        s = self.s
        if self.strategy == "shared" or bits is not None:
            field_backward_split(s.flat, s.frame, level, 3, act, self.grad_flat, self.grad_cond, d_raw=d_raw, xw_grad_in=xw_grad_in, arch=self.arch, bits=bits)
        else:
            field_backward(s.flat, s.frame, level, act, d_raw, self.grad_flat, self.grad_cond, self.arch)

    def part_walk(self, level, part, d_raw=None, xw_grad_in=None, side=None):
        s = self.s
        act, bits = (s.act0, s.bits0) if level == 0 else (s.act_r, s.bits_r) if part == FIELD_RADIANCE else (s.act_d, s.bits_d)
        walk = lambda grad_cond: field_backward_split(s.flat, s.frame, level, part, act, self.grad_flat, grad_cond, d_raw=d_raw, xw_grad_in=xw_grad_in,
                                                      arch=self.arch, full_act=(level == 0), bits=bits)
        if side is None:
            return walk(self.grad_cond)
        main = torch.cuda.current_stream(s.rays.device)
        side[0].wait_stream(main)
        with torch.cuda.stream(side[0]):
            out = walk(side[1])
        for t in (s.flat, s.frame, act, bits, self.grad_flat, side[1], d_raw, xw_grad_in):
            if t is not None:
                t.record_stream(side[0])
        if out is not None:
            out.record_stream(main)
        return out

    def fine_walks(self, d_raw):
        g_f = self.part_walk(1, FIELD_RADIANCE, d_raw=d_raw)
        xwg_coarse, g_new = route_xw_grad(self.s.src, g_f, self.num_coarse)
        self.part_walk(1, FIELD_DEFORM, xw_grad_in=g_new)
        return xwg_coarse

    def one_stream(self):
        s, N = self.s, self.s.rays.shape[0]
        for start in range(0, N, RenderRaysFn.BLOCK_RAYS):
            sl = slice(start, min(N, start + RenderRaysFn.BLOCK_RAYS))
            xwg_coarse = None
            for level in self.grads:
                if not self.has_grad[level] and xwg_coarse is None:
                    continue
                if (self.strategy, level) == ("shared", 1):
                    xwg_coarse = self.fine_walks(self.composite(1, s.raw1, sl))
                    continue
                if self.strategy == "recompute":
                    (raw, act), bits = field_forward_save(s.packed, s.frame, level, s.rays[sl].contiguous(), self.z[level][sl].contiguous(), self.arch), None
                else:
                    raw, act, bits = getattr(s, "raw%d" % level), getattr(s, "act%d" % level), getattr(s, "bits%d" % level)
                d_raw = self.composite(level, raw, sl)
                self.whole_walk(level, act, bits, d_raw, xwg_coarse)
                del raw, act, d_raw

    def two_streams(self):
        s = self.s
        d_raw1, d_raw0 = self.composite(1, s.raw1), self.composite(0, s.raw0)
        side = (_side_stream(s.rays.device), torch.zeros_like(self.grad_cond))
        main = torch.cuda.current_stream(s.rays.device)
        g_c0 = self.part_walk(0, FIELD_RADIANCE, d_raw=d_raw0, side=side)
        g_f = self.part_walk(1, FIELD_RADIANCE, d_raw=d_raw1)
        xwg_coarse, g_new = route_xw_grad(s.src, g_f, self.num_coarse)
        main.wait_stream(side[0])
        xwg0 = g_c0 + xwg_coarse
        self.part_walk(0, FIELD_DEFORM, xw_grad_in=xwg0, side=side)
        self.part_walk(1, FIELD_DEFORM, xw_grad_in=g_new)
        main.wait_stream(side[0])
        self.grad_cond += side[1]
```

Measured before the change: 455,200.

## Fuse sparse branch into trunk kernel via per-workgroup ring buffers

Adds fused trunk+branch modes in which each persistent workgroup writes live samples' features into its own bounded ring buffer and runs the branch MLP tile as soon as a full tile has accumulated. This replaces the separate trunk and branch launches and the slab loop over a large record workspace. The default workspace now shrinks to the ring size, which avoids writing and re-reading feature records for all samples through global memory. The cost is a more complex kernel with per-tile branching, LDS counts, block-wide syncs and a permuted tile order, and the branch tiles may be unevenly balanced across workgroups.

After: 460,400 (median of 6 runs). 1.1% higher.

```diff
diff --git a/include/sahs_nerf.h b/include/sahs_nerf.h
--- a/include/sahs_nerf.h
+++ b/include/sahs_nerf.h
@@ -148,6 +148,7 @@
                                 float *weights, float *rows, int row_ld, float *xw, int32_t *src, float *z_new, void *stream);
 
 size_t sahs_model_render_sparse_workspace_bytes(int model, long samples);
+size_t sahs_model_render_sparse_fused_workspace_bytes(int model, long samples);
 int sahs_model_render_rays_rows_sparse(int model, const void *packed, const float *frame, int precision, long N, const float *rays,
                                        int ray_stride, int Sc, int nf, int lindisp, int white_background, const float *bg, const float *t_rand,
                                        const float *noise_c, const float *u, const float *noise_f, float *z_c, float *z_f, float *raw,
diff --git a/sahs-deformable-nerf_amd/_lib.py b/sahs-deformable-nerf_amd/_lib.py
--- a/sahs-deformable-nerf_amd/_lib.py
+++ b/sahs-deformable-nerf_amd/_lib.py
@@ -44,6 +44,7 @@
     "sahs_model_executed_macs_part": (_L, [_I, _I, _I]),
     "sahs_model_render_rays_rows": (_I, [_I, _P, _P, _I, _L, _P, _I, _I, _I, _I, _I] + [_P] * 10 + [_I, _P, _P, _P, _P]),
     "sahs_model_render_sparse_workspace_bytes": (ctypes.c_size_t, [_I, _L]),
+    "sahs_model_render_sparse_fused_workspace_bytes": (ctypes.c_size_t, [_I, _L]),
     "sahs_model_render_rays_rows_sparse": (_I, [_I, _P, _P, _I, _L, _P, _I, _I, _I, _I, _I] + [_P] * 10 + [_I, _P, _P, _P, _P, ctypes.c_size_t, _P]),
     "sahs_resample_merge": (_I, [_L, _I, _I, _P, _P, _P, _P, _P, _P, _P]),
     "sahs_model_act_words_part": (_L, [_I, _I]),
diff --git a/sahs-deformable-nerf_amd/build.py b/sahs-deformable-nerf_amd/build.py
--- a/sahs-deformable-nerf_amd/build.py
+++ b/sahs-deformable-nerf_amd/build.py
@@ -14,6 +14,7 @@
 NO_SCRATCH = {"gemm_dma_kernel": 0, "_ZN4sahs24field_forward_f32_kernelILb0E": 0, "field_forward_bf16w_kernel": 0,
               "field_radiance_bf16x3_kernel": 0, "field_deform_bf16x3_kernel": 0, "gemm_tn_split_kernel": 0, "gemm_tn_jobs_kernel": 0,
               "field_backward_chain_rad_kernel": 0, "field_backward_chain_def_kernel": 0, "_ZN4sahs24field_forward_f32_kernelILb1E": 96,
+              "field_forward_f32_kernelILb0ELi6E": 0, "field_forward_f32_kernelILb0ELi7E": 0,
               "gemm_tn_jobs_f32_kernel": 0, "gemm_tn_jobs256_f32_kernel": 0, "adam_step_kernel": 0,
               "field_backward_chain_rad_f32_kernel": 0, "field_backward_chain_def_f32_kernel": 0,
               "_ZN7sahs_nf3bwc31field_backward_chain_rad_kernel": 0, "_ZN7sahs_nf3bwc31field_backward_chain_def_kernel": 0,
diff --git a/sahs-deformable-nerf_amd/csrc/capi.hip b/sahs-deformable-nerf_amd/csrc/capi.hip
--- a/sahs-deformable-nerf_amd/csrc/capi.hip
+++ b/sahs-deformable-nerf_amd/csrc/capi.hip
@@ -297,6 +297,7 @@
     decltype(&sahs_field_forward_f32_split_bits_launch) f32_split_bits;
     decltype(&sahs_field_forward_f32_sparse_launch) f32_sparse;
     decltype(&sahs_field_f32_sparse_ws_bytes) f32_sparse_ws_bytes;
+    decltype(&sahs_field_f32_sparse_ring_slots) f32_sparse_ring_slots;
     long (*bwd_ws_words)(long);
     decltype(&sahs_field_backward_launch) bwd;
     decltype(&sahs_field_backward_split_launch) bwd_split;
@@ -318,7 +319,7 @@
         sahs_layout_executed_macs##sfx, sahs_layout_act_part_words##sfx, sahs_layout_act_part_col0##sfx, sahs_layout_bits_part_words##sfx, \
         sahs_fold_conditioning_launch##sfx, sahs_bwd_gemm_precision_state##sfx, sahs_bf16w_exact_leaky_state##sfx,                  \
         sahs_field_forward_f32_launch##sfx, sahs_field_forward_f32_split_launch##sfx, sahs_field_forward_f32_split_bits_launch##sfx, \
-        sahs_field_forward_f32_sparse_launch##sfx, sahs_field_f32_sparse_ws_bytes##sfx,                                              \
+        sahs_field_forward_f32_sparse_launch##sfx, sahs_field_f32_sparse_ws_bytes##sfx, sahs_field_f32_sparse_ring_slots##sfx,       \
         sahs_field_backward_ws_words##sfx, sahs_field_backward_launch##sfx, sahs_field_backward_split_launch##sfx,                  \
         sahs_field_backward_fused_ws_words##sfx, sahs_field_backward_fused_launch##sfx
 static const ModelFns kModels[3] = {
@@ -805,6 +806,16 @@
                                 const float *noise, int has_bg, void *ws, long cap, hipStream_t st)
 {
     const ModelFns &m = kModels[model];
+    if (N * S <= (1L << 30) && cap >= m.f32_sparse_ring_slots(N * S, num_cus())) {
+        int e = probed(probe_kind(model, SAHS_F32, level, part), N * S, st, [&] {
+            hipError_t he = hipMemsetAsync(ws, 0, 8, st);
+            if (he != hipSuccess) return (int)he;
+            return m.f32_sparse(pk, frame, level, stage + 3, N * S, S, rays, ray_stride, z, raw, xw, xw_row, 0, src, noise, has_bg, ws, cap, num_cus(), st);
+        });
+        if (e == -4) return fail(5, "%s: the sparse-branch launcher refused its record workspace (%ld slots for the rings of %ld samples)", who, cap, N * S);
+        if (e < 0) return fail(4, "%s: the sparse-branch launcher has no stage %d for this model", who, stage + 3);
+        return e ? hip_fail(who, e) : 0;
+    }
     const long per = cap / S;
     if (per < 1) return fail(5, "%s: the sparse-branch workspace holds %ld records, one ray has %d samples", who, cap, S);
     const long nslab = (N + per - 1) / per, step = (N + nslab - 1) / nslab;
@@ -826,6 +837,12 @@
     if (e == -4) return fail(5, "%s: the sparse-branch launcher refused its record workspace (%ld slots for slabs of %ld samples)", who, cap, step * S);
     if (e < 0) return fail(4, "%s: the sparse-branch launcher has no stage %d for this model", who, stage);
     return e ? hip_fail(who, e) : 0;
+}
+
+size_t sahs_model_render_sparse_fused_workspace_bytes(int model, long samples)
+{
+    if (model < 0 || model > 2 || samples < 0 || samples > (1L << 30)) return 0;
+    return (size_t)kModels[model].f32_sparse_ws_bytes(samples > 0 ? kModels[model].f32_sparse_ring_slots(samples, num_cus()) : 0);
 }
 
 size_t sahs_model_render_sparse_workspace_bytes(int model, long samples)
diff --git a/sahs-deformable-nerf_amd/csrc/field_f32.hip b/sahs-deformable-nerf_amd/csrc/field_f32.hip
--- a/sahs-deformable-nerf_amd/csrc/field_f32.hip
+++ b/sahs-deformable-nerf_amd/csrc/field_f32.hip
@@ -86,7 +86,17 @@
 
 #define CHF(id) (kProg.layer[id].G * kProg.layer[id].KB * 256)
 
-enum { FIELD_ALL = 0, FIELD_DEFORM = 1, FIELD_RADIANCE = 2, FIELD_ALL_TRUNK = 3, FIELD_RADIANCE_TRUNK = 4, FIELD_BRANCH = 5 };
+enum { FIELD_ALL = 0, FIELD_DEFORM = 1, FIELD_RADIANCE = 2, FIELD_ALL_TRUNK = 3, FIELD_RADIANCE_TRUNK = 4, FIELD_BRANCH = 5, FIELD_ALL_FUSED = 6,
+       FIELD_RADIANCE_FUSED = 7 };
+constexpr int SPARSE_RING = 512;
+static_assert(SPARSE_RING >= 255 + 128 && SPARSE_RING % 128 == 0, "a ring holds the carried count plus one tile");
+__host__ __device__ constexpr long sparse_ring_slots(long tiles) { return tiles * F32_PTS_PER_WG < SPARSE_RING ? tiles * F32_PTS_PER_WG : SPARSE_RING; }
+__host__ __device__ constexpr long sparse_ring_base(long ntiles, long grid, long g)
+{
+    const long tlo = ntiles / grid, rem = ntiles % grid;
+    return g * sparse_ring_slots(tlo) + (g < rem ? g : rem) * (sparse_ring_slots(tlo + 1) - sparse_ring_slots(tlo));
+}
+constexpr int LDS_RING_FLOATS = 16;
 struct SparseArgs {
     const float *noise;
     unsigned int *count;
@@ -135,12 +145,13 @@
                          float *__restrict__ xw, int xw_row, int xw_col0, const int *__restrict__ src, uint32_t *__restrict__ bits, SparseArgs sp)
 {
 #if SAHS_MODEL == 2
-    static_assert(MODE == FIELD_ALL || MODE == FIELD_ALL_TRUNK || MODE == FIELD_BRANCH, "this model has no deformation nets to split off");
+    static_assert(MODE == FIELD_ALL || MODE == FIELD_ALL_TRUNK || MODE == FIELD_BRANCH || MODE == FIELD_ALL_FUSED, "this model has no deformation nets to split off");
 #endif
     constexpr bool TRUNK = MODE == FIELD_ALL_TRUNK || MODE == FIELD_RADIANCE_TRUNK;
     constexpr bool BRANCH = MODE == FIELD_BRANCH;
-    constexpr bool XW_IN = MODE == FIELD_RADIANCE || MODE == FIELD_RADIANCE_TRUNK;
-    static_assert(!(SAVE && (TRUNK || BRANCH)), "the sparse branches are an inference path");
+    constexpr bool FUSED = MODE == FIELD_ALL_FUSED || MODE == FIELD_RADIANCE_FUSED;
+    constexpr bool XW_IN = MODE == FIELD_RADIANCE || MODE == FIELD_RADIANCE_TRUNK || MODE == FIELD_RADIANCE_FUSED;
+    static_assert(!(SAVE && (TRUNK || BRANCH || FUSED)), "the sparse branches are an inference path");
     extern __shared__ __attribute__((aligned(16))) float lds[];
     Ctx cx;
     cx.stream = packed + PACK_STREAM_OFF + (long)level * STREAM_FLOATS;
@@ -152,7 +163,7 @@
     constexpr const Layer *Ly = kProg.layer;
     constexpr int L_START = BRANCH ? L_D0B : (XW_IN ? L_T0 : L_FIRST);
     cx.wrap_to = (uint32_t)Ly[L_START].stream_off;
-    cx.wrap_at = (MODE == FIELD_DEFORM) ? (uint32_t)Ly[L_T0].stream_off : (TRUNK ? (uint32_t)Ly[L_D0B].stream_off : (uint32_t)STREAM_FLOATS);
+    cx.wrap_at = (MODE == FIELD_DEFORM) ? (uint32_t)Ly[L_T0].stream_off : ((TRUNK || FUSED) ? (uint32_t)Ly[L_D0B].stream_off : (uint32_t)STREAM_FLOATS);
     cx.off = cx.wrap_to;
     const float *grid = packed + PACK_GRID_OFF;
 
@@ -170,14 +181,45 @@
         P = n < sp.cap ? n : sp.cap;
     }
     const long ntiles = (P + F32_PTS_PER_WG - 1) / F32_PTS_PER_WG;
-    constexpr bool XW_AHEAD = MODE == FIELD_RADIANCE_TRUNK && !DIAG_NOLOADS_TRUNK;
+    constexpr bool XW_AHEAD = (MODE == FIELD_RADIANCE_TRUNK && !DIAG_NOLOADS_TRUNK) || MODE == FIELD_RADIANCE_FUSED;
     f32x4 nx_a = f32x4{0.0f, 0.0f, 0.0f, 0.0f};
     float nx_w1 = 0.0f;
     int nx_src = 0;
-    for (long tile = blockIdx.x; tile < ntiles; tile += gridDim.x) {
+    uint32_t r_cnt = 0u, r_head = 0u, r_total = 0u, r_cap = 0u, r_base = 0u;
+    uint32_t r_it = 0u, r_tiles = 0u;
+    if constexpr (FUSED) {
+        r_tiles = (uint32_t)__builtin_amdgcn_readfirstlane((int)(ntiles / gridDim.x + ((long)blockIdx.x < ntiles % gridDim.x ? 1 : 0)));
+        r_cap = (uint32_t)sparse_ring_slots(r_tiles);
+        r_base = (uint32_t)__builtin_amdgcn_readfirstlane((int)sparse_ring_base(ntiles, gridDim.x, blockIdx.x));
+    }
+    const uint32_t r_rows = FUSED ? (uint32_t)__builtin_amdgcn_readfirstlane((int)(ntiles / gridDim.x)) : 0u;
+    auto fused_tile = [&](uint32_t k) -> long {
+        const uint32_t col = k < r_rows ? (blockIdx.x + 61u * k) % gridDim.x : blockIdx.x;
+        return (long)k * gridDim.x + col;
+    };
+    for (long tile_it = blockIdx.x; FUSED || tile_it < ntiles; tile_it += gridDim.x, ++r_it) {
+        const long tile = FUSED ? fused_tile(r_it) : tile_it;
+        bool has_tile = true, do_branch = false;
+        uint32_t b_valid = 0u;
+        if constexpr (FUSED) {
+            has_tile = r_it < r_tiles;
+            do_branch = has_tile ? r_cnt >= (uint32_t)F32_PTS_PER_WG : r_cnt > 0u;
+            if (!has_tile && !do_branch) break;
+            b_valid = r_cnt < (uint32_t)F32_PTS_PER_WG ? r_cnt : (uint32_t)F32_PTS_PER_WG;
+            if (has_tile) {
+                cx.wrap_at = do_branch ? (uint32_t)STREAM_FLOATS : (uint32_t)Ly[L_D0B].stream_off;
+            } else {
+                cx.off = (uint32_t)Ly[L_D0B].stream_off;
+                cx.wrap_at = (uint32_t)STREAM_FLOATS;
+                cx.begin_chunk(CHF(L_D0B));
+#pragma unroll
+                for (int pc = 0; pc < (CHF(L_D0B) + PIECE_FLOATS - 1) / PIECE_FLOATS; ++pc) cx.issue_piece(pc);
+                cx.end_chunk();
+            }
+        }
         cx.refresh();
         int q_tile = cx.q;
-        if constexpr (TRUNK) { asm volatile("" : "+s"(cx.off)); asm volatile("" : "+v"(q_tile)); }
+        if constexpr (TRUNK || FUSED) { asm volatile("" : "+s"(cx.off)); asm volatile("" : "+v"(q_tile)); }
         const int q = q_tile;
         const long p_raw = tile * F32_PTS_PER_WG + cx.wave * F32_PTS_PER_WAVE + (cx.lane & 15);
         const long p = p_raw < P ? p_raw : P - 1;
@@ -205,13 +247,15 @@
             smp = __float_as_int(a[3]);
             if (q == 0) { stash[0] = a[0]; stash[1] = a[1]; stash[2] = a[2]; }
         } else if constexpr (!XW_IN) {
+            if (!FUSED || has_tile) {
             const float *rp = rays + (p / S) * ray_stride;
             const float z = zvals[p];
 #pragma unroll
             for (int i = 0; i < 3; ++i) x[i] = rp[i] + rp[3 + i] * z;
+            }
         } else if constexpr (XW_AHEAD) {
-            if (q == 0) {
-                if (tile == (long)blockIdx.x) {
+            if (q == 0 && (!FUSED || has_tile)) {
+                if (FUSED ? r_it == 0u : tile == (long)blockIdx.x) {
                     const float *row = xw + ((p / S) * (long)xw_row + src[p]) * 8;
                     nx_a = *reinterpret_cast<const f32x4 *>(row);
                     nx_w1 = row[4];
@@ -224,13 +268,23 @@
             stash[0] = a[0]; stash[1] = a[1]; stash[2] = a[2]; stash[3] = a[3]; stash[4] = row[4];
             if (sv_on) { float *d = SVP(act::XW, 16); d[0] = a[0]; d[1] = a[1]; d[2] = a[2]; }
         }
-        const bool has_next = XW_AHEAD && tile + gridDim.x < ntiles;
-        const long pn_raw = p_raw + (long)gridDim.x * F32_PTS_PER_WG;
+        const bool has_next = XW_AHEAD && (FUSED ? r_it + 1u < r_tiles : tile + gridDim.x < ntiles);
+        const long pn_raw = FUSED ? fused_tile(r_it + 1u) * F32_PTS_PER_WG + cx.wave * F32_PTS_PER_WAVE + (cx.lane & 15) : p_raw + (long)gridDim.x * F32_PTS_PER_WG;
         const long p_next = pn_raw < P ? pn_raw : P - 1;
         if constexpr (XW_AHEAD) {
             if (has_next && q == 0) nx_src = src[p_next];
         }
+        f32x4 b_hdr = f32x4{0.0f, 0.0f, 0.0f, 0.0f};
+        uint32_t b_slot = 0u;
+        if constexpr (FUSED) {
+            if (do_branch) {
+                const uint32_t j = (uint32_t)(cx.wave * F32_PTS_PER_WAVE + (cx.lane & 15));
+                b_slot = r_base + r_head + (j < b_valid ? j : b_valid - 1u);
+                if (!has_tile) b_hdr = sp.hdr[b_slot];
+            }
+        }
         if constexpr (!XW_IN && !BRANCH) {
+        if (!FUSED || has_tile) {
 #if SAHS_MODEL == 2
         if (q == 0) {
             stash[0] = x[0]; stash[1] = x[1]; stash[2] = x[2]; stash[3] = 0.0f; stash[4] = 0.0f;
@@ -307,6 +361,7 @@
             row[4] = stash[4];
         }
         }
+        }
         if constexpr (MODE == FIELD_DEFORM) continue;
         __builtin_amdgcn_wave_barrier();
         if (dump) { dsl[0] = stash[0] - x[0]; dsl[1] = stash[1] - x[1]; dsl[2] = stash[2] - x[2]; dsl[3] = stash[3]; dsl[4] = stash[4]; }
@@ -322,10 +377,10 @@
             const f32x4 *rec = sp.feat + (p >> 4) * (16 * 64) + q * 16 + (p & 15);
 #pragma unroll
             for (int b = 0; b < 16; ++b) feat[b] = rec[b * 64];
-        } else {
+        } else if (!FUSED || has_tile) {
             f32x4 h[16];
-            if constexpr (TRUNK) {
-                constexpr bool ENC_ONCE = MODE == FIELD_RADIANCE_TRUNK && !DIAG_ENC2;
+            if constexpr (TRUNK || FUSED) {
+                constexpr bool ENC_ONCE = (MODE == FIELD_RADIANCE_TRUNK && !DIAG_ENC2) || MODE == FIELD_RADIANCE_FUSED;
                 f32x4 in_tr[KB_XYZ + KB_AMB];
                 auto build_enc = [&]() {
                     const float xw[3] = {stash[0], stash[1], stash[2]}, amb[2] = {stash[3], stash[4]};
@@ -343,6 +398,9 @@
                 };
                 build_enc();
                 dense<KB_XYZ, KB_AMB, 16, CHF(L_T1)>(cx, in_tr, in_tr + KB_XYZ, h, Ly[L_T0].bias_off, false, 0.01f);
+                if constexpr (FUSED) {
+                    if (do_branch) b_hdr = sp.hdr[b_slot];
+                }
                 dense<16, 0, 16, CHF(L_T2)>(cx, h, nullptr, feat, Ly[L_T1].bias_off, false, 0.01f);
 #pragma unroll
                 for (int i = 0; i < 16; ++i) h[i] = feat[i];
@@ -416,7 +474,60 @@
             dense_sv<SAVE, 16, 0, 16, CHF(L_ALPHA)>(cx, h, nullptr, feat, Ly[L_FEAT].bias_off, false, 1.0f, SV(act::FEAT, 256));
             if (dump) dsl[13] = feat[0][0];
         }
-        if constexpr (!BRANCH) dense<16, 0, 1, (TRUNK ? CHF(L_START) : CHF(L_D0B))>(cx, feat, nullptr, fin, Ly[L_ALPHA].bias_off, false, 1.0f);
+        if constexpr (FUSED) {
+            if (has_tile) {
+                if (do_branch) dense<16, 0, 1, CHF(L_D0B)>(cx, feat, nullptr, fin, Ly[L_ALPHA].bias_off, false, 1.0f);
+                else dense<16, 0, 1, CHF(L_START)>(cx, feat, nullptr, fin, Ly[L_ALPHA].bias_off, false, 1.0f);
+            }
+        } else if constexpr (!BRANCH) dense<16, 0, 1, (TRUNK ? CHF(L_START) : CHF(L_D0B))>(cx, feat, nullptr, fin, Ly[L_ALPHA].bias_off, false, 1.0f);
+        if constexpr (FUSED) {
+            if (has_tile) {
+                if (p_raw < P) *reinterpret_cast<f32x4 *>(raw + p * D_RAW + 4 * q) = fin[0];
+                const long ray = p / S;
+                const bool last = (p - ray * S) == S - 1;
+                const float sg = fin[0][3] + (sp.noise != nullptr ? sp.noise[p] : 0.0f);
+                const bool live = q == 3 && p_raw < P && (last ? sp.has_bg == 0 : sg > 0.0f);
+                const uint32_t mask = (uint32_t)(__ballot(live) >> 48);
+                uint32_t *cnts = reinterpret_cast<uint32_t *>(lds + LDS_TOTAL_FLOATS);
+                if (cx.lane == 0) cnts[cx.wave] = (uint32_t)__popc(mask);
+                __syncthreads();
+                uint32_t before = 0u, all = 0u;
+#pragma unroll
+                for (int w = 0; w < F32_THREADS / WAVE; ++w) {
+                    const uint32_t c = cnts[w];
+                    all += c;
+                    before += w < cx.wave ? c : 0u;
+                }
+                before = (uint32_t)__builtin_amdgcn_readfirstlane((int)before);
+                all = (uint32_t)__builtin_amdgcn_readfirstlane((int)all);
+                uint32_t tail = r_head + r_cnt;
+                if (tail >= r_cap) tail -= r_cap;
+                const int j = cx.lane & 15;
+                if ((mask >> j) & 1u) {
+                    uint32_t idx = tail + before + (uint32_t)__popc(mask & ((1u << j) - 1u));
+                    if (idx >= r_cap) idx -= r_cap;
+                    const uint32_t slot = r_base + idx;
+                    f32x4 *rec = sp.feat + (long)(slot >> 4) * (16 * 64) + q * 16 + (slot & 15u);
+#pragma unroll
+                    for (int b = 0; b < 16; ++b) rec[b * 64] = feat[b];
+                    if (q == 0) sp.hdr[slot] = f32x4{stash[0], stash[1], stash[2], __int_as_float((int)p)};
+                }
+                r_cnt += all;
+                r_total += all;
+            }
+            if (!do_branch) continue;
+            smp = __float_as_int(b_hdr[3]);
+            __builtin_amdgcn_wave_barrier();
+            if (q == 0) { stash[0] = b_hdr[0]; stash[1] = b_hdr[1]; stash[2] = b_hdr[2]; }
+            __builtin_amdgcn_wave_barrier();
+            fin[0] = *reinterpret_cast<const f32x4 *>(raw + smp * D_RAW + 4 * q);
+            const f32x4 *rec = sp.feat + (long)(b_slot >> 4) * (16 * 64) + q * 16 + (b_slot & 15u);
+#pragma unroll
+            for (int b = 0; b < 16; ++b) feat[b] = rec[b * 64];
+            r_cnt -= b_valid;
+            r_head += (uint32_t)F32_PTS_PER_WG;
+            if (r_head >= r_cap) r_head -= r_cap;
+        }
         if constexpr (TRUNK) {
             if (p_raw < P) *reinterpret_cast<f32x4 *>(raw + p * D_RAW + 4 * q) = fin[0];
             const long ray = p / S;
@@ -496,7 +607,14 @@
             if (dump) dsl[17] = sn[0][0];
             dense<8, 0, 1, CHF(L_START)>(cx, sn, nullptr, fin, 0, true, 1.0f);
         }
-        if (p_raw < P) *reinterpret_cast<f32x4 *>(raw + smp * D_RAW + 4 * q) = fin[0];
+        if (FUSED ? (uint32_t)(cx.wave * F32_PTS_PER_WAVE + (cx.lane & 15)) < b_valid : p_raw < P)
+            *reinterpret_cast<f32x4 *>(raw + smp * D_RAW + 4 * q) = fin[0];
+    }
+    if constexpr (FUSED) {
+        if (threadIdx.x == 0) {
+            if (r_total != 0u) atomicAdd(sp.count, r_total);
+            if (blockIdx.x == 0) sp.count[1] = 1u;
+        }
     }
 }
 
@@ -511,7 +629,7 @@
 {
     const long ntiles = (P + F32_PTS_PER_WG - 1) / F32_PTS_PER_WG;
     const int grid = (int)(ntiles < num_cu ? ntiles : num_cu);
-    const size_t lds_bytes = (size_t)LDS_TOTAL_FLOATS * sizeof(float);
+    const size_t lds_bytes = (size_t)(LDS_TOTAL_FLOATS + ((MODE == FIELD_ALL_FUSED || MODE == FIELD_RADIANCE_FUSED) ? LDS_RING_FLOATS : 0)) * sizeof(float);
     static sahs_once::Flags attr_set;
     hipError_t ae = sahs_once::per_device(attr_set, [&]() {
         return hipFuncSetAttribute(reinterpret_cast<const void *>(field_forward_f32_kernel<SAVE, MODE>), hipFuncAttributeMaxDynamicSharedMemorySize,
@@ -569,13 +687,21 @@
 }
 
 extern "C" long SAHS_SYM(sahs_field_f32_sparse_ws_bytes)(long cap) { return SPARSE_HEAD_BYTES + cap * SPARSE_RECORD_BYTES; }
+extern "C" long SAHS_SYM(sahs_field_f32_sparse_ring_slots)(long P, int num_cu)
+{
+    if (P <= 0 || num_cu < 1) return 0;
+    const long ntiles = (P + F32_PTS_PER_WG - 1) / F32_PTS_PER_WG, grid = ntiles < num_cu ? ntiles : num_cu;
+    return sparse_ring_base(ntiles, grid, grid);
+}
 extern "C" int SAHS_SYM(sahs_field_forward_f32_sparse_launch)(const float *packed, const float *frame, int level, int stage, long P, int S,
                                                     const float *rays, int ray_stride, const float *zvals, float *raw, float *xw, int xw_row,
                                                     int xw_col0, const int *src, const float *noise, int has_bg, void *ws, long cap, int num_cu,
                                                     hipStream_t stream)
 {
     if (P <= 0) return 0;
-    if (ws == nullptr || cap < P || cap % F32_PTS_PER_WG != 0 || cap > (1L << 30)) return -4;
+    const bool fused = stage == 3 || stage == 4;
+    if (ws == nullptr || cap % F32_PTS_PER_WG != 0 || cap > (1L << 30)) return -4;
+    if (cap < (fused ? SAHS_SYM(sahs_field_f32_sparse_ring_slots)(P, num_cu) : P)) return -4;
     char *base = static_cast<char *>(ws);
     SparseArgs sp{noise, reinterpret_cast<unsigned int *>(base), reinterpret_cast<f32x4 *>(base + SPARSE_HEAD_BYTES),
                   reinterpret_cast<f32x4 *>(base + SPARSE_HEAD_BYTES + cap * 16), (unsigned int)cap, has_bg};
@@ -583,9 +709,13 @@
         return launch_field<false, FIELD_ALL_TRUNK>(packed, frame, level, P, S, rays, ray_stride, zvals, raw, nullptr, nullptr, xw, xw_row, xw_col0, nullptr, num_cu, stream, nullptr, sp);
     if (stage == 2)
         return launch_field<false, FIELD_BRANCH>(packed, frame, level, P, S, rays, ray_stride, nullptr, raw, nullptr, nullptr, nullptr, 0, 0, nullptr, num_cu, stream, nullptr, sp);
+    if (stage == 3)
+        return launch_field<false, FIELD_ALL_FUSED>(packed, frame, level, P, S, rays, ray_stride, zvals, raw, nullptr, nullptr, xw, xw_row, xw_col0, nullptr, num_cu, stream, nullptr, sp);
 #if SAHS_MODEL != 2
     if (stage == 1)
         return launch_field<false, FIELD_RADIANCE_TRUNK>(packed, frame, level, P, S, rays, ray_stride, nullptr, raw, nullptr, nullptr, xw, xw_row, 0, src, num_cu, stream, nullptr, sp);
+    if (stage == 4)
+        return launch_field<false, FIELD_RADIANCE_FUSED>(packed, frame, level, P, S, rays, ray_stride, nullptr, raw, nullptr, nullptr, xw, xw_row, 0, src, num_cu, stream, nullptr, sp);
 #endif
     return -2;
 }
diff --git a/sahs-deformable-nerf_amd/csrc/sahs_launchers.hpp b/sahs-deformable-nerf_amd/csrc/sahs_launchers.hpp
--- a/sahs-deformable-nerf_amd/csrc/sahs_launchers.hpp
+++ b/sahs-deformable-nerf_amd/csrc/sahs_launchers.hpp
@@ -59,6 +59,7 @@
                                                       int xw_row, int xw_col0, const int *src, float *actbuf, uint32_t *bits,           \
                                                       int num_cu, hipStream_t stream);                                                  \
     long sahs_field_f32_sparse_ws_bytes##sfx(long cap);                                                                                 \
+    long sahs_field_f32_sparse_ring_slots##sfx(long P, int num_cu);                                                                     \
     int sahs_field_forward_f32_sparse_launch##sfx(const float *packed, const float *frame, int level, int stage, long P, int S,        \
                                                   const float *rays, int ray_stride, const float *zvals, float *raw, float *xw,         \
                                                   int xw_row, int xw_col0, const int *src, const float *noise, int has_bg, void *ws,    \
diff --git a/sahs-deformable-nerf_amd/ops.py b/sahs-deformable-nerf_amd/ops.py
--- a/sahs-deformable-nerf_amd/ops.py
+++ b/sahs-deformable-nerf_amd/ops.py
@@ -236,7 +236,7 @@
     return rgb_c, disp_c, acc_c, None, None, None, w_bg, depth_f
 
 
-_SPARSE_WORKSPACE_BYTES = 4 << 30
+_SPARSE_WORKSPACE_BYTES = None
 _SPARSE_BRANCHES = True
 
 
@@ -254,6 +254,8 @@
 
 
 def sparse_workspace_bytes():
+    if _SPARSE_WORKSPACE_BYTES is None:
+        return int(_lib.lib().sahs_model_render_sparse_fused_workspace_bytes(0, 1 << 30))
     return _SPARSE_WORKSPACE_BYTES
 
 
@@ -262,6 +264,13 @@
     if rec is None:
         raise _lib.SahsError("sparse_last_count: this workspace has not been through a sparse render")
     return int(rec[:4].view(torch.int32).item())
+
+
+def sparse_last_path(workspace):
+    rec = workspace.get("sparse") if workspace else None
+    if rec is None:
+        raise _lib.SahsError("sparse_last_path: this workspace has not been through a sparse render")
+    return int(rec[4:8].view(torch.int32).item())
 
 
 ROW_COLUMNS = 36
@@ -300,7 +309,7 @@
         src = _workspace_buffer(ws, dev, "src", (N, Sf), torch.int32)
     extra = []
     if _SPARSE_BRANCHES and precision == SAHS_F32 and N > 0:
-        want = min(int(_fn("render_sparse_workspace_bytes", arch)[0](min(N * Sf, 1 << 30))), _SPARSE_WORKSPACE_BYTES)
+        want = min(int(_fn("render_sparse_workspace_bytes", arch)[0](min(N * Sf, 1 << 30))), sparse_workspace_bytes())
         extra = [_p(_workspace_buffer(ws, dev, "sparse", (want,), torch.uint8)), want]
     f, name = _fn("render_rays_rows_sparse" if extra else "render_rays_rows", arch)
     check(f(_p(packed), _p(frame), precision, N, _p(rays), int(rays.shape[1]), int(num_coarse), int(num_fine),
```
